# Glaciohound/Chimera-ST

Measured on AMD Instinct MI355X. Metric: train utterances/sec, MuST-C EN-DE s2t_transformer_m, 1/2/4/8 MI355X, higher is better.
Workload: dtype bf16

## Files before the change

### chimera-st_amd/csrc/gemm.hip

```cpp
#include "gemm_common.h"
#include <vector>
#include <stdlib.h>
#include <string.h>
#include <type_traits>

namespace {
using namespace cstg;

template <int BM_, int BN_, int WM_, int WN_, int KV_ = 8>
struct Cfg {
  static constexpr int BM = BM_, BN = BN_, WM = WM_, WN = WN_, NT = 64 * WM_ * WN_, TM = BM_ / WM_ / 32, TN = BN_ / WN_ / 32;
  static constexpr int KV = KV_;
  static_assert(BM_ <= GEMM_MAX_BM && GEMM_MAX_BM % BM_ == 0, "conv0.hip (cst_conv_row_limits) sizes live frames from GEMM_MAX_BM");
};
using CfgSmall = Cfg<128, 128, 2, 2>;
using CfgSkinny = Cfg<64, 64, 2, 2>;
using CfgNarrowN = Cfg<128, 64, 2, 2>;
using CfgNarrowM = Cfg<64, 128, 2, 2>;
using CfgLarge = Cfg<256, 256, 4, 4>;

template <typename T, bool A_KMAJOR, bool B_KMAJOR, bool SEG, typename C, bool CS = false>
__global__ __launch_bounds__(C::NT) void gemm_kernel(GemmParams p) {
  constexpr int BM = C::BM, BN = C::BN, NTHREADS = C::NT, TM = C::TM, TN = C::TN;
  constexpr int VEC = DT<T>::VEC;
  constexpr int KV = C::KV, BK = KV * VEC;
  constexpr int LDK = BK + VEC;
  constexpr int LDMA = sizeof(T) == 2 ? BM + 32 : BM + VEC;
  constexpr int LDMB = sizeof(T) == 2 ? BN + 32 : BN + VEC;
  constexpr int A_ELEMS = A_KMAJOR ? BM * LDK : BK * LDMA;
  constexpr int B_ELEMS = B_KMAJOR ? BN * LDK : BK * LDMB;
  constexpr int MVA = BM / VEC, MVB = BN / VEC;
  constexpr int NVA = BM * KV / NTHREADS, NVB = BN * KV / NTHREADS;
  extern __shared__ __attribute__((aligned(16))) char smem_raw[];
  T* smem = reinterpret_cast<T*>(smem_raw);
  constexpr int STAGE = A_ELEMS + B_ELEMS;

  const int tid = threadIdx.x, lane = tid & 63, wave = tid >> 6;
  const int wm = wave / C::WN, wn = wave % C::WN;

  const int ntiles = p.tiles_m * p.tiles_n;
  int tm, tn, z;
  if (p.split_order) {
    const int total = ntiles * p.splits, L = (int)blockIdx.x + (int)gridDim.x * (int)blockIdx.z;
    const int q = total / 8, r = total % 8, xcd = L % 8, loc = L / 8;
    const int item = (xcd < r ? xcd * (q + 1) : r * (q + 1) + (xcd - r) * q) + loc;
    z = item / ntiles;
    const int t = item % ntiles;
    tm = t / p.tiles_n;
    tn = t % p.tiles_n;
  } else {
    int id = blockIdx.x;
    {
      const int q = ntiles / 8, r = ntiles % 8, xcd = id % 8, loc = id / 8;
      id = (xcd < r ? xcd * (q + 1) : r * (q + 1) + (xcd - r) * q) + loc;
    }
    constexpr int GROUP_M = 8;
    const int per_group = GROUP_M * p.tiles_n;
    const int grp = id / per_group, rem = id % per_group;
    const int gm0 = grp * GROUP_M;
    const int gsz = (p.tiles_m - gm0 < GROUP_M) ? (p.tiles_m - gm0) : GROUP_M;
    tm = gm0 + rem % gsz;
    tn = rem / gsz;
    z = blockIdx.z;
  }
  const int64_t m0 = (int64_t)tm * BM, n0 = (int64_t)tn * BN;

  const int split = z % p.splits;
  const int64_t bidx = z / p.splits;
  const int64_t b0 = bidx / p.batch1, b1 = bidx % p.batch1;
  const T* A = (const T*)p.A + b0 * p.sa0 + b1 * p.sa1;
  const T* B = (const T*)p.B + b0 * p.sb0 + b1 * p.sb1;
  const int64_t cofs = b0 * p.sc0 + b1 * p.sc1;
  const int64_t bofs = b0 * p.sbias0 + b1 * p.sbias1;

  int ktiles = (int)((p.K + BK - 1) / BK);
  const int kfull = (int)(p.K / BK);
  if (p.k_len) {
    typedef const __attribute__((address_space(4))) int32_t* cptr_t;
    const int kl = ((cptr_t)p.k_len)[b0];
    const int live = kl <= 0 ? 0 : (kl + BK - 1) / BK;
    ktiles = live < ktiles ? live : ktiles;
  }
  const int per = (ktiles + p.splits - 1) / p.splits;
  const int kt0 = split * per;
  const int kt1 = (kt0 + per < ktiles) ? kt0 + per : ktiles;

  u32x4 ra[NVA], rb[NVB];
  const T* pa[NVA];
  const T* pb[NVB];
  int ka[NVA], kb[NVB];
  int aq[NVA], ar[NVA], bq[NVB], br[NVB];
#pragma unroll
  for (int i = 0; i < NVA; ++i) {
    const int v = tid + NTHREADS * i;
    if (A_KMAJOR) {
      int64_t row = m0 + v / KV;
      row = row < p.M ? row : p.M - 1;
      ka[i] = kt0 * BK + (v % KV) * VEC;
      if (SEG && p.a_seg) { aq[i] = ka[i] / (int)p.a_seg; ar[i] = ka[i] % (int)p.a_seg; pa[i] = A + row * p.lda; }
      else { aq[i] = 0; ar[i] = 0; pa[i] = A + row * p.lda + ka[i]; }
    } else {
      int64_t m = m0 + (int64_t)(v % MVA) * VEC;
      m = m < p.M ? m : p.M - VEC;
      ka[i] = kt0 * BK + v / MVA;
      aq[i] = 0; ar[i] = 0;
      pa[i] = A + (int64_t)ka[i] * p.lda + segaddr(m, p.a_seg, p.a_seg_stride);
    }
  }
#pragma unroll
  for (int i = 0; i < NVB; ++i) {
    const int v = tid + NTHREADS * i;
    if (B_KMAJOR) {
      int64_t row = n0 + v / KV;
      row = row < p.N ? row : p.N - 1;
      kb[i] = kt0 * BK + (v % KV) * VEC;
      if (SEG && p.b_seg) { bq[i] = kb[i] / (int)p.b_seg; br[i] = kb[i] % (int)p.b_seg; pb[i] = B + row * p.ldb; }
      else { bq[i] = 0; br[i] = 0; pb[i] = B + row * p.ldb + kb[i]; }
    } else {
      int64_t n = n0 + (int64_t)(v % MVB) * VEC;
      n = n < p.N ? n : p.N - VEC;
      kb[i] = kt0 * BK + v / MVB;
      bq[i] = 0; br[i] = 0;
      pb[i] = B + (int64_t)kb[i] * p.ldb + segaddr(n, p.b_seg, p.b_seg_stride);
    }
  }
  const int64_t step_a = A_KMAJOR ? (int64_t)BK : (int64_t)BK * p.lda;
  const int64_t step_b = B_KMAJOR ? (int64_t)BK : (int64_t)BK * p.ldb;

  auto load_tile = [&](auto tail_tag) {
    constexpr bool TAIL = decltype(tail_tag)::value;
    const u32x4 zero = {0, 0, 0, 0};
#pragma unroll
    for (int i = 0; i < NVA; ++i) {
      const T* qa = pa[i];
      if (SEG && A_KMAJOR && p.a_seg) qa = pa[i] + (int64_t)aq[i] * p.a_seg_stride + ar[i];
      if (TAIL) {
        const bool oka = ka[i] < p.K;
        const u32x4 va = *reinterpret_cast<const u32x4*>(oka ? qa : A);
        ra[i] = oka ? va : zero;
      } else {
        ra[i] = *reinterpret_cast<const u32x4*>(qa);
      }
      ka[i] += BK;
      if (SEG && A_KMAJOR && p.a_seg) { ar[i] += BK; while (ar[i] >= (int)p.a_seg) { ar[i] -= (int)p.a_seg; ++aq[i]; } }
      else pa[i] += step_a;
    }
#pragma unroll
    for (int i = 0; i < NVB; ++i) {
      const T* qb = pb[i];
      if (SEG && B_KMAJOR && p.b_seg) qb = pb[i] + (int64_t)bq[i] * p.b_seg_stride + br[i];
      if (TAIL) {
        const bool okb = kb[i] < p.K;
        const u32x4 vb = *reinterpret_cast<const u32x4*>(okb ? qb : B);
        rb[i] = okb ? vb : zero;
      } else {
        rb[i] = *reinterpret_cast<const u32x4*>(qb);
      }
      kb[i] += BK;
      if (SEG && B_KMAJOR && p.b_seg) { br[i] += BK; while (br[i] >= (int)p.b_seg) { br[i] -= (int)p.b_seg; ++bq[i]; } }
      else pb[i] += step_b;
    }
  };
  auto load_any = [&](int kt) {
    if (kt < kfull) load_tile(std::false_type{});
    else load_tile(std::true_type{});
  };
  static_assert(!CS || (!A_KMAJOR && NTHREADS % MVA == 0), "a thread must stage the same columns of an mn-major A in every vector");
  const bool do_cs = CS && tn == 0;
  float cs[VEC];
#pragma unroll
  for (int e = 0; e < VEC; ++e) cs[e] = 0.0f;
  auto store_tile = [&](int buf) {
#pragma unroll
    for (int i = 0; i < NVA; ++i) {
      const int v = tid + NTHREADS * i;
      T* da = smem + buf * STAGE + (A_KMAJOR ? (v / KV) * LDK + (v % KV) * VEC : (v / MVA) * LDMA + (v % MVA) * VEC);
      *reinterpret_cast<u32x4*>(da) = ra[i];
      if (CS && do_cs) {
        if (sizeof(T) == 2) {
#pragma unroll
          for (int e = 0; e < 4; ++e) {
            cs[2 * e] += __uint_as_float(ra[i][e] << 16);
            cs[2 * e + 1] += __uint_as_float(ra[i][e] & 0xffff0000u);
          }
        } else {
#pragma unroll
          for (int e = 0; e < 4; ++e) cs[e] += __uint_as_float(ra[i][e]);
        }
      }
    }
#pragma unroll
    for (int i = 0; i < NVB; ++i) {
      const int v = tid + NTHREADS * i;
      T* db = smem + buf * STAGE + A_ELEMS + (B_KMAJOR ? (v / KV) * LDK + (v % KV) * VEC : (v / MVB) * LDMB + (v % MVB) * VEC);
      *reinterpret_cast<u32x4*>(db) = rb[i];
    }
  };

  f32x16 acc[TM][TN];
#pragma unroll
  for (int i = 0; i < TM; ++i)
#pragma unroll
    for (int j = 0; j < TN; ++j)
#pragma unroll
      for (int r = 0; r < 16; ++r) acc[i][j][r] = 0.0f;

  constexpr int KLIST_MAX = 1000;
  __shared__ int klist[KLIST_MAX];
  __shared__ int klist_n;
  const bool kskip = !SEG && BK == 64 && p.k_live != nullptr && per <= KLIST_MAX;
  int nk = kt1 > kt0 ? kt1 - kt0 : 0;
  if (kskip) {
    if (wave == 0) {
      int total = 0;
      for (int base = 0; base < ktiles; base += 64) {
        const int kt = base + lane;
        total += __builtin_popcountll(__builtin_amdgcn_ballot_w64(kt < ktiles && p.k_live[kt] == p.k_epoch));
      }
      const int lo = (int)(((int64_t)total * split) / p.splits), hi = (int)(((int64_t)total * (split + 1)) / p.splits);
      int seen = 0, n = 0;
      for (int base = 0; base < ktiles && seen < hi; base += 64) {
        const int kt = base + lane;
        const bool live = kt < ktiles && p.k_live[kt] == p.k_epoch;
        const uint64_t m = __builtin_amdgcn_ballot_w64(live);
        const int idx = seen + __builtin_popcountll(m & ((1ull << lane) - 1ull));
        if (live && idx >= lo && idx < hi) klist[idx - lo] = kt;
        seen += __builtin_popcountll(m);
      }
      n = hi - lo;
      if (lane == 0) klist_n = n;
    }
    __syncthreads();
    nk = klist_n;
  }
  if (p.m_live) {
    typedef const __attribute__((address_space(4))) uint32_t* cptr_t;
    cptr_t ml = (cptr_t)p.m_live;
    const int t0 = (int)(m0 >> 6), t1 = (int)((((m0 + BM < p.M) ? m0 + BM : p.M) + 63) >> 6);
    bool live = false;
    for (int t = t0; t < t1; ++t) live |= ml[t] == p.m_epoch;
    if (!live) nk = 0;
  }
  if (p.m_len) {
    typedef const __attribute__((address_space(4))) int32_t* cptr_t;
    if (m0 >= (int64_t)((cptr_t)p.m_len)[b0]) nk = 0;
  }
  int pos = kt0;
  auto fetch = [&](int kt) {
    const int d = kt - pos;
    if (d) {
#pragma unroll
      for (int i = 0; i < NVA; ++i) { pa[i] += (int64_t)d * step_a; ka[i] += d * BK; }
#pragma unroll
      for (int i = 0; i < NVB; ++i) { pb[i] += (int64_t)d * step_b; kb[i] += d * BK; }
    }
    load_any(kt);
    pos = kt + 1;
  };
  auto tile_at = [&](int it) { return kskip ? klist[it] : kt0 + it; };

  if (nk > 0) {
    fetch(tile_at(0));
    store_tile(0);
  }
  __syncthreads();
  int cur = 0;
  const int lrow = lane & 31, lk = 8 * (lane >> 5);
  constexpr int WROWS = TM * 32, WCOLS = TN * 32;
  for (int it = 0; it < nk; ++it) {
    const bool more = it + 1 < nk;
    if (more) fetch(tile_at(it + 1));
    const T* sa = smem + cur * STAGE;
    const T* sb = sa + A_ELEMS;
#pragma unroll
    for (int kk = 0; kk < BK; kk += 16) {
      Frag<T> fa[TM], fb[TN];
#pragma unroll
      for (int i = 0; i < TM; ++i) {
        if (A_KMAJOR) frag_load_contig(fa[i], sa + (wm * WROWS + i * 32 + lrow) * LDK + kk + lk);
        else frag_load_tr(fa[i], sa, LDMA, wm * WROWS + i * 32, kk + lk, kk + lk + 4, lane);
      }
#pragma unroll
      for (int j = 0; j < TN; ++j) {
        if (B_KMAJOR) frag_load_contig(fb[j], sb + (wn * WCOLS + j * 32 + lrow) * LDK + kk + lk);
        else frag_load_tr(fb[j], sb, LDMB, wn * WCOLS + j * 32, kk + lk, kk + lk + 4, lane);
      }
#pragma unroll
      for (int i = 0; i < TM; ++i)
#pragma unroll
        for (int j = 0; j < TN; ++j) mma16(acc[i][j], fa[i], fb[j]);
    }
    if (more) store_tile(cur ^ 1);
    __syncthreads();
    cur ^= 1;
  }

  if (CS && do_cs) {
    float* red = reinterpret_cast<float*>(smem_raw);
#pragma unroll
    for (int e = 0; e < VEC; ++e) red[(tid / MVA) * BM + (tid % MVA) * VEC + e] = cs[e];
    __syncthreads();
    if (tid < BM && m0 + tid < p.M) {
      float tot = 0.0f;
      for (int r = 0; r < NTHREADS / MVA; ++r) tot += red[r * BM + tid];
      if (p.splits > 1) p.colsum_ws[((int64_t)bidx * p.splits + split) * p.M + m0 + tid] = tot;
      else DT<T>::st((T*)p.colsum + bidx * p.M + m0 + tid, tot);
    }
  }

  constexpr int LDC = BN + 4;
  constexpr int VPR = BN / 8;
  constexpr int NPASS = BM / 64;
  constexpr int ITERS = 64 * VPR / NTHREADS;
  float* stage = reinterpret_cast<float*>(smem_raw);
  float* wsp = p.splits > 1 ? p.ws + ((int64_t)z) * p.M * p.N : nullptr;
  const bool ws_vec = (p.N % 4) == 0;
#pragma unroll
  for (int ps = 0; ps < NPASS; ++ps) {
    __syncthreads();
#pragma unroll
    for (int i = 0; i < TM; ++i) {
      const int trow = wm * WROWS + i * 32;
      if (trow / 64 == ps) {
#pragma unroll
        for (int j = 0; j < TN; ++j)
#pragma unroll
          for (int r = 0; r < 16; ++r)
            stage[(trow - 64 * ps + acc_row(r, lane)) * LDC + wn * WCOLS + j * 32 + lrow] = acc[i][j][r];
      }
    }
    __syncthreads();
#pragma unroll 2
    for (int it = 0; it < ITERS; ++it) {
      const int v = tid + NTHREADS * it;
      const int rl = v / VPR, cl = (v % VPR) * 8;
      const int64_t row = m0 + 64 * ps + rl, col = n0 + cl;
      if (row >= p.M || col >= p.N) continue;
      float x[8];
      {
        const f32x4 a = *reinterpret_cast<const f32x4*>(stage + rl * LDC + cl);
        const f32x4 b = *reinterpret_cast<const f32x4*>(stage + rl * LDC + cl + 4);
        x[0] = a[0]; x[1] = a[1]; x[2] = a[2]; x[3] = a[3]; x[4] = b[0]; x[5] = b[1]; x[6] = b[2]; x[7] = b[3];
      }
      const bool full = col + 8 <= p.N;
      if (wsp) {
        if (full && ws_vec) store8(wsp + row * p.N + col, x);
        else
          for (int e = 0; e < 8 && col + e < p.N; ++e) wsp[row * p.N + col + e] = x[e];
      } else if (full && p.vec_epi) {
        epilogue_store8<T>(p, cofs, bofs, row, col, x);
      } else {
        for (int e = 0; e < 8 && col + e < p.N; ++e) epilogue_store<T>(p, cofs, bofs, row, col + e, x[e]);
      }
    }
  }
}

template <int N>
__device__ __forceinline__ void wait_vmcnt() { asm volatile("s_waitcnt vmcnt(%0)" ::"n"(N) : "memory"); }

template <typename T, bool A_KMAJOR, bool B_KMAJOR, typename C, int NS>
__global__ __launch_bounds__(C::NT) void gemm_glds_kernel(GemmParams p) {
  constexpr int BM = C::BM, BN = C::BN, NTHREADS = C::NT, TM = C::TM, TN = C::TN, NWAVES = C::NT / 64;
  constexpr int ES = sizeof(T), VEC = DT<T>::VEC, BK = 128 / ES;
  constexpr int A_BYTES = A_KMAJOR ? BM * 128 : BK * BM * ES;
  constexpr int B_BYTES = B_KMAJOR ? BN * 128 : BK * BN * ES;
  constexpr int STAGE_BYTES = A_BYTES + B_BYTES;
  constexpr int GA = A_BYTES / 1024 / NWAVES, GB = B_BYTES / 1024 / NWAVES;
  extern __shared__ __attribute__((aligned(16))) char smem_raw[];

  const int tid = threadIdx.x, lane = tid & 63, wave = tid >> 6;
  const int wm = wave / C::WN, wn = wave % C::WN;
  const int ntiles = p.tiles_m * p.tiles_n;
  int id = blockIdx.x;
  {
    const int q = ntiles / 8, r = ntiles % 8, xcd = id % 8, loc = id / 8;
    id = (xcd < r ? xcd * (q + 1) : r * (q + 1) + (xcd - r) * q) + loc;
  }
  constexpr int GROUP_M = 8;
  int tm, tn;
  {
    const int per_group = GROUP_M * p.tiles_n;
    const int grp = id / per_group, rem = id % per_group;
    const int gm0 = grp * GROUP_M;
    const int gsz = (p.tiles_m - gm0 < GROUP_M) ? (p.tiles_m - gm0) : GROUP_M;
    tm = gm0 + rem % gsz;
    tn = rem / gsz;
  }
  const int64_t m0 = (int64_t)tm * BM, n0 = (int64_t)tn * BN;
  const int z = blockIdx.z;
  const int split = z % p.splits;
  const int64_t bidx = z / p.splits;
  const int64_t b0 = bidx / p.batch1, b1 = bidx % p.batch1;
  const T* A = (const T*)p.A + b0 * p.sa0 + b1 * p.sa1;
  const T* B = (const T*)p.B + b0 * p.sb0 + b1 * p.sb1;
  const int64_t cofs = b0 * p.sc0 + b1 * p.sc1;
  const int64_t bofs = b0 * p.sbias0 + b1 * p.sbias1;
  const int ktiles = (int)((p.K + BK - 1) / BK);
  const int kfull = (int)(p.K / BK);
  const int per = (ktiles + p.splits - 1) / p.splits;
  const int kt0 = split * per;
  const int kt1 = (kt0 + per < ktiles) ? kt0 + per : ktiles;
  int nt = kt1 - kt0;
  if (p.m_len) {
    typedef const __attribute__((address_space(4))) int32_t* cptr_t;
    if (m0 >= (int64_t)((cptr_t)p.m_len)[b0]) nt = 0;
  }

  const T* pa[GA];
  const T* pb[GB];
  int ka[GA], kb[GB];
#pragma unroll
  for (int i = 0; i < GA; ++i) {
    const int g = wave + NWAVES * i;
    if (A_KMAJOR) {
      const int r = 8 * g + (lane >> 3), c = (lane & 7) ^ ((r >> 1) & 7);
      int64_t row = m0 + r;
      row = row < p.M ? row : p.M - 1;
      ka[i] = kt0 * BK + c * VEC;
      pa[i] = A + row * p.lda + ka[i];
    } else {
      constexpr int RB = BM * ES, RPG = 1024 / RB > 0 ? 1024 / RB : 1, CPR = RB / 16;
      const int kl = g * RPG + (lane * 16) / RB, pc = ((lane * 16) % RB) / 16;
      const int c = ES == 2 ? (pc ^ (4 * (kl & 3))) : pc;
      int64_t m = m0 + (int64_t)c * VEC;
      m = m < p.M ? m : p.M - VEC;
      ka[i] = kt0 * BK + kl;
      pa[i] = A + (int64_t)ka[i] * p.lda + segaddr(m, p.a_seg, p.a_seg_stride);
      (void)CPR;
    }
  }
#pragma unroll
  for (int i = 0; i < GB; ++i) {
    const int g = wave + NWAVES * i;
    if (B_KMAJOR) {
      const int r = 8 * g + (lane >> 3), c = (lane & 7) ^ ((r >> 1) & 7);
      int64_t row = n0 + r;
      row = row < p.N ? row : p.N - 1;
      kb[i] = kt0 * BK + c * VEC;
      pb[i] = B + row * p.ldb + kb[i];
    } else {
      constexpr int RB = BN * ES, RPG = 1024 / RB > 0 ? 1024 / RB : 1;
      const int kl = g * RPG + (lane * 16) / RB, pc = ((lane * 16) % RB) / 16;
      const int c = ES == 2 ? (pc ^ (4 * (kl & 3))) : pc;
      int64_t n = n0 + (int64_t)c * VEC;
      n = n < p.N ? n : p.N - VEC;
      kb[i] = kt0 * BK + kl;
      pb[i] = B + (int64_t)kb[i] * p.ldb + segaddr(n, p.b_seg, p.b_seg_stride);
    }
  }
  const int64_t step_a = A_KMAJOR ? (int64_t)BK : (int64_t)BK * p.lda;
  const int64_t step_b = B_KMAJOR ? (int64_t)BK : (int64_t)BK * p.ldb;

  auto issue = [&](int kt, int stage) {
    char* sbase = smem_raw + stage * STAGE_BYTES;
    if (kt < kfull) {
#pragma unroll
      for (int i = 0; i < GA; ++i) {
        __builtin_amdgcn_global_load_lds((const __attribute__((address_space(1))) void*)pa[i],
                                         (__attribute__((address_space(3))) void*)(sbase + (wave + NWAVES * i) * 1024), 16, 0, 0);
        pa[i] += step_a;
        ka[i] += BK;
      }
#pragma unroll
      for (int i = 0; i < GB; ++i) {
        __builtin_amdgcn_global_load_lds((const __attribute__((address_space(1))) void*)pb[i],
                                         (__attribute__((address_space(3))) void*)(sbase + A_BYTES + (wave + NWAVES * i) * 1024), 16, 0, 0);
        pb[i] += step_b;
        kb[i] += BK;
      }
    } else {
      const u32x4 zero = {0, 0, 0, 0};
#pragma unroll
      for (int i = 0; i < GA; ++i) {
        const bool ok = ka[i] < p.K;
        const u32x4 v = *reinterpret_cast<const u32x4*>(ok ? pa[i] : A);
        *reinterpret_cast<u32x4*>(sbase + (wave + NWAVES * i) * 1024 + lane * 16) = ok ? v : zero;
        pa[i] += step_a;
        ka[i] += BK;
      }
#pragma unroll
      for (int i = 0; i < GB; ++i) {
        const bool ok = kb[i] < p.K;
        const u32x4 v = *reinterpret_cast<const u32x4*>(ok ? pb[i] : B);
        *reinterpret_cast<u32x4*>(sbase + A_BYTES + (wave + NWAVES * i) * 1024 + lane * 16) = ok ? v : zero;
        pb[i] += step_b;
        kb[i] += BK;
      }
    }
  };

  f32x16 acc[TM][TN];
#pragma unroll
  for (int i = 0; i < TM; ++i)
#pragma unroll
    for (int j = 0; j < TN; ++j)
#pragma unroll
      for (int r = 0; r < 16; ++r) acc[i][j][r] = 0.0f;

  const int lrow = lane & 31, hi = lane >> 5;
  constexpr int WROWS = TM * 32, WCOLS = TN * 32;
  constexpr int G = GA + GB;

#pragma unroll
  for (int s = 0; s < NS - 1; ++s)
    if (s < nt) issue(kt0 + s, s);

  constexpr bool PIN = NTHREADS == 256 && TM == 4 && NS == 2 && A_KMAJOR && B_KMAJOR && sizeof(T) == 2;
  if constexpr (PIN) {
    auto issue_one = [&](int d, char* sbase) {
      if (d < GA) {
        __builtin_amdgcn_global_load_lds((const __attribute__((address_space(1))) void*)pa[d],
                                         (__attribute__((address_space(3))) void*)(sbase + (wave + NWAVES * d) * 1024), 16, 0, 0);
        pa[d] += step_a;
        ka[d] += BK;
      } else {
        const int e = d - GA;
        __builtin_amdgcn_global_load_lds((const __attribute__((address_space(1))) void*)pb[e],
                                         (__attribute__((address_space(3))) void*)(sbase + A_BYTES + (wave + NWAVES * e) * 1024), 16, 0, 0);
        pb[e] += step_b;
        kb[e] += BK;
      }
    };
    constexpr int NSLOT = TM * TN / 2, NFR = TM + TN;
    for (int it = 0; it < nt; ++it) {
      wait_vmcnt<0>();
      __builtin_amdgcn_s_barrier();
      const bool more = it + 1 < nt;
      const bool dma_ok = more && (kt0 + it + 1) < kfull;
      if (more && !dma_ok) issue(kt0 + it + 1, (it + 1) & 1);
      const char* sbase = smem_raw + (it & 1) * STAGE_BYTES;
      char* nbase = smem_raw + ((it + 1) & 1) * STAGE_BYTES;
      const T* sa = reinterpret_cast<const T*>(sbase);
      const T* sb = reinterpret_cast<const T*>(sbase + A_BYTES);
      Frag<T> fa[2][TM], fb[2][TN];
      auto read_one = [&](int f, int kk, int buf) {
        if (f < TM) frag_load_kswz(fa[buf][f], sa, wm * WROWS + f * 32 + lrow, kk * 16 + 8 * hi);
        else frag_load_kswz(fb[buf][f - TM], sb, wn * WCOLS + (f - TM) * 32 + lrow, kk * 16 + 8 * hi);
      };
#pragma unroll
      for (int f = 0; f < NFR; ++f) read_one(f, 0, 0);
      __builtin_amdgcn_sched_barrier(0);
#pragma unroll
      for (int kk = 0; kk < 4; ++kk) {
#pragma unroll
        for (int sl = 0; sl < NSLOT; ++sl) {
#pragma unroll
          for (int u = 0; u < 2; ++u) {
            const int m = 2 * sl + u, i = m / TN, j = m % TN;
            mma16(acc[i][j], fb[kk & 1][j], fa[kk & 1][i]);
          }
          if (kk < 3) {
            if (sl < NFR) read_one(sl, kk + 1, (kk + 1) & 1);
            if (sl == 0 && NFR > NSLOT) {
#pragma unroll
              for (int f = NSLOT; f < NFR; ++f) read_one(f, kk + 1, (kk + 1) & 1);
            }
          }
          if (kk * NSLOT + sl < G && dma_ok) issue_one(kk * NSLOT + sl, nbase);
          __builtin_amdgcn_sched_barrier(0);
        }
      }
    }
  } else
  for (int it = 0; it < nt; ++it) {
    const int issued = (it + NS - 1 < nt) ? it + NS - 1 : nt;
    if (NS > 2 && issued - it - 1 == NS - 2) wait_vmcnt<(NS - 2) * G>();
    else wait_vmcnt<0>();
    __builtin_amdgcn_s_barrier();
    if (it + NS - 1 < nt) issue(kt0 + it + NS - 1, (it + NS - 1) % NS);
    const char* sbase = smem_raw + (it % NS) * STAGE_BYTES;
    const T* sa = reinterpret_cast<const T*>(sbase);
    const T* sb = reinterpret_cast<const T*>(sbase + A_BYTES);
#pragma unroll
    for (int kk = 0; kk < BK; kk += 16) {
      Frag<T> fa[TM], fb[TN];
#pragma unroll
      for (int i = 0; i < TM; ++i) {
        if (A_KMAJOR) {
          const int r = wm * WROWS + i * 32 + lrow;
          frag_load_kswz(fa[i], sa, r, kk + 8 * hi);
        } else {
          frag_load_tr_swz(fa[i], sa, BM, wm * WROWS + i * 32, kk + 8 * hi, lane);
        }
      }
#pragma unroll
      for (int j = 0; j < TN; ++j) {
        if (B_KMAJOR) {
          const int r = wn * WCOLS + j * 32 + lrow;
          frag_load_kswz(fb[j], sb, r, kk + 8 * hi);
        } else {
          frag_load_tr_swz(fb[j], sb, BN, wn * WCOLS + j * 32, kk + 8 * hi, lane);
        }
      }
#pragma unroll
      for (int i = 0; i < TM; ++i)
#pragma unroll
        for (int j = 0; j < TN; ++j) mma16(acc[i][j], fa[i], fb[j]);
    }
  }

  float* wsp = p.splits > 1 ? p.ws + ((int64_t)z) * p.M * p.N : nullptr;
  const bool ws_vec = (p.N % 4) == 0;
  if constexpr (PIN) {
    constexpr int LDW = WCOLS + 4, VPRW = WCOLS / 8, RITER = 32 * VPRW / 64;
    static_assert(4 * 32 * LDW * 4 <= NS * STAGE_BYTES && (32 * VPRW) % 64 == 0, "the four waves' images live in the stage buffers");
    __syncthreads();
    float* img = reinterpret_cast<float*>(smem_raw) + wave * (32 * LDW);
#pragma unroll
    for (int i = 0; i < TM; ++i) {
#pragma unroll
      for (int j = 0; j < TN; ++j)
#pragma unroll
        for (int q = 0; q < 4; ++q) {
          const f32x4 v = {acc[i][j][4 * q], acc[i][j][4 * q + 1], acc[i][j][4 * q + 2], acc[i][j][4 * q + 3]};
          *reinterpret_cast<f32x4*>(img + lrow * LDW + j * 32 + 8 * q + 4 * hi) = v;
        }
#pragma unroll 2
      for (int tv = 0; tv < RITER; ++tv) {
        const int v = tv * 64 + lane;
        const int rl = v / VPRW, cl = (v % VPRW) * 8;
        const int64_t row = m0 + wm * WROWS + i * 32 + rl, col = n0 + wn * WCOLS + cl;
        if (row >= p.M || col >= p.N) continue;
        float x[8];
        {
          const f32x4 a = *reinterpret_cast<const f32x4*>(img + rl * LDW + cl);
          const f32x4 b = *reinterpret_cast<const f32x4*>(img + rl * LDW + cl + 4);
          x[0] = a[0]; x[1] = a[1]; x[2] = a[2]; x[3] = a[3]; x[4] = b[0]; x[5] = b[1]; x[6] = b[2]; x[7] = b[3];
        }
        const bool full = col + 8 <= p.N;
        if (wsp) {
          if (full && ws_vec) store8(wsp + row * p.N + col, x);
          else
            for (int e = 0; e < 8 && col + e < p.N; ++e) wsp[row * p.N + col + e] = x[e];
        } else if (full && p.vec_epi) {
          epilogue_store8<T>(p, cofs, bofs, row, col, x);
        } else {
          for (int e = 0; e < 8 && col + e < p.N; ++e) epilogue_store<T>(p, cofs, bofs, row, col + e, x[e]);
        }
      }
    }
    return;
  }
  constexpr int LDC = BN + 4;
  constexpr int VPR = BN / 8;
  constexpr int NPASS = BM / 64;
  constexpr int ITERS = 64 * VPR / NTHREADS;
  float* stage = reinterpret_cast<float*>(smem_raw);
#pragma unroll
  for (int ps = 0; ps < NPASS; ++ps) {
    __syncthreads();
#pragma unroll
    for (int i = 0; i < TM; ++i) {
      const int trow = wm * WROWS + i * 32;
      if (trow / 64 == ps) {
#pragma unroll
        for (int j = 0; j < TN; ++j)
#pragma unroll
          for (int r = 0; r < 16; ++r)
            stage[(trow - 64 * ps + acc_row(r, lane)) * LDC + wn * WCOLS + j * 32 + lrow] = acc[i][j][r];
      }
    }
    __syncthreads();
#pragma unroll 2
    for (int itv = 0; itv < ITERS; ++itv) {
      const int v = tid + NTHREADS * itv;
      const int rl = v / VPR, cl = (v % VPR) * 8;
      const int64_t row = m0 + 64 * ps + rl, col = n0 + cl;
      if (row >= p.M || col >= p.N) continue;
      float x[8];
      {
        const f32x4 a = *reinterpret_cast<const f32x4*>(stage + rl * LDC + cl);
        const f32x4 b = *reinterpret_cast<const f32x4*>(stage + rl * LDC + cl + 4);
        x[0] = a[0]; x[1] = a[1]; x[2] = a[2]; x[3] = a[3]; x[4] = b[0]; x[5] = b[1]; x[6] = b[2]; x[7] = b[3];
      }
      const bool full = col + 8 <= p.N;
      if (wsp) {
        if (full && ws_vec) store8(wsp + row * p.N + col, x);
        else
          for (int e = 0; e < 8 && col + e < p.N; ++e) wsp[row * p.N + col + e] = x[e];
      } else if (full && p.vec_epi) {
        epilogue_store8<T>(p, cofs, bofs, row, col, x);
      } else {
        for (int e = 0; e < 8 && col + e < p.N; ++e) epilogue_store<T>(p, cofs, bofs, row, col + e, x[e]);
      }
    }
  }
}

template <typename T>
__global__ void splitk_reduce_kernel(GemmParams p) {
  const int64_t total = p.M * p.N;
  const int64_t bidx = blockIdx.y;
  const int64_t b0 = bidx / p.batch1, b1 = bidx % p.batch1;
  const int64_t cofs = b0 * p.sc0 + b1 * p.sc1;
  const int64_t bofs = b0 * p.sbias0 + b1 * p.sbias1;
  const float* ws = p.ws + bidx * p.splits * total;
  if (p.colsum) {
    for (int64_t m = (int64_t)blockIdx.x * blockDim.x + threadIdx.x; m < p.M; m += (int64_t)gridDim.x * blockDim.x) {
      float v = 0.0f;
      for (int s = 0; s < p.splits; ++s) v += p.colsum_ws[(bidx * p.splits + s) * p.M + m];
      DT<T>::st((T*)p.colsum + bidx * p.M + m, v);
    }
  }
  if (p.vec_epi && (p.N % 8) == 0) {
    const int64_t total8 = total >> 3;
    for (int64_t i8 = (int64_t)blockIdx.x * blockDim.x + threadIdx.x; i8 < total8; i8 += (int64_t)gridDim.x * blockDim.x) {
      const float* src = ws + i8 * 8;
      float v[8] = {0.0f, 0.0f, 0.0f, 0.0f, 0.0f, 0.0f, 0.0f, 0.0f};
      int sp = 0;
      for (; sp + 4 <= p.splits; sp += 4) {
        f32x4 a[4][2];
#pragma unroll
        for (int u = 0; u < 4; ++u) {
          a[u][0] = *reinterpret_cast<const f32x4*>(src + (int64_t)(sp + u) * total);
          a[u][1] = *reinterpret_cast<const f32x4*>(src + (int64_t)(sp + u) * total + 4);
        }
#pragma unroll
        for (int u = 0; u < 4; ++u)
#pragma unroll
          for (int e = 0; e < 4; ++e) { v[e] += a[u][0][e]; v[4 + e] += a[u][1][e]; }
      }
      for (; sp < p.splits; ++sp) {
        const f32x4 a0 = *reinterpret_cast<const f32x4*>(src + (int64_t)sp * total), a1 = *reinterpret_cast<const f32x4*>(src + (int64_t)sp * total + 4);
#pragma unroll
        for (int e = 0; e < 4; ++e) { v[e] += a0[e]; v[4 + e] += a1[e]; }
      }
      const int64_t i = i8 * 8, row = i / p.N;
      epilogue_store8<T>(p, cofs, bofs, row, i - row * p.N, v);
    }
    return;
  }
  for (int64_t i = (int64_t)blockIdx.x * blockDim.x + threadIdx.x; i < total; i += (int64_t)gridDim.x * blockDim.x) {
    float v = 0.0f;
    for (int s = 0; s < p.splits; ++s) v += ws[s * total + i];
    epilogue_store<T>(p, cofs, bofs, i / p.N, i % p.N, v);
  }
}

template <typename T, bool AK, bool BK_, bool SEG, typename C>
int launch(GemmParams p, int64_t M, int64_t N, int64_t nbatch, hipStream_t s) {
  constexpr int VEC = DT<T>::VEC;
  constexpr int BKc = C::KV * VEC, LDK = BKc + VEC;
  constexpr int LDMA = sizeof(T) == 2 ? C::BM + 32 : C::BM + VEC, LDMB = sizeof(T) == 2 ? C::BN + 32 : C::BN + VEC;
  constexpr int A_ELEMS = AK ? C::BM * LDK : BKc * LDMA;
  constexpr int B_ELEMS = BK_ ? C::BN * LDK : BKc * LDMB;
  size_t lds = 2 * (size_t)(A_ELEMS + B_ELEMS) * sizeof(T);
  const size_t stage_bytes = (size_t)64 * (C::BN + 4) * sizeof(float);
  if (lds < stage_bytes) lds = stage_bytes;
  static bool attr_set = false;
  if (!attr_set) {
    (void)hipFuncSetAttribute(reinterpret_cast<const void*>(&gemm_kernel<T, AK, BK_, SEG, C>), hipFuncAttributeMaxDynamicSharedMemorySize, 160 * 1024 - 4096);
    attr_set = true;
  }
  p.tiles_m = (int)cst_ceil_div(M, C::BM);
  p.tiles_n = (int)cst_ceil_div(N, C::BN);
  p.split_order = (p.splits > 1 && nbatch == 1) ? 1 : 0;
  dim3 grid(p.tiles_m * p.tiles_n, 1, (unsigned)(nbatch * p.splits));
  if constexpr (!AK && !BK_ && !SEG && C::NT <= 256) {
    if (p.colsum) {
      static bool attr_cs = false;
      if (!attr_cs) {
        (void)hipFuncSetAttribute(reinterpret_cast<const void*>(&gemm_kernel<T, AK, BK_, SEG, C, true>), hipFuncAttributeMaxDynamicSharedMemorySize, 160 * 1024 - 4096);
        attr_cs = true;
      }
      hipLaunchKernelGGL((gemm_kernel<T, AK, BK_, SEG, C, true>), grid, dim3(C::NT), lds, s, p);
      return cst_check_launch("cst_gemm");
    }
  }
  if (p.colsum) { cst_set_error("cst_gemm: internal: column sums requested from a configuration that does not build them"); return CST_ERR_UNSUPPORTED; }
  hipLaunchKernelGGL((gemm_kernel<T, AK, BK_, SEG, C>), grid, dim3(C::NT), lds, s, p);
  return cst_check_launch("cst_gemm");
}

template <typename T, bool AK, bool BK_, typename C, int NS>
int launch_glds(GemmParams p, int64_t M, int64_t N, int64_t nbatch, hipStream_t s) {
  constexpr int ES = sizeof(T), BKc = 128 / ES;
  constexpr int A_BYTES = AK ? C::BM * 128 : BKc * C::BM * ES, B_BYTES = BK_ ? C::BN * 128 : BKc * C::BN * ES;
  size_t lds = (size_t)NS * (A_BYTES + B_BYTES);
  const size_t stage_bytes = (size_t)64 * (C::BN + 4) * sizeof(float);
  if (lds < stage_bytes) lds = stage_bytes;
  static bool attr_set = false;
  if (!attr_set) {
    (void)hipFuncSetAttribute(reinterpret_cast<const void*>(&gemm_glds_kernel<T, AK, BK_, C, NS>), hipFuncAttributeMaxDynamicSharedMemorySize, 160 * 1024);
    attr_set = true;
  }
  p.tiles_m = (int)cst_ceil_div(M, C::BM);
  p.tiles_n = (int)cst_ceil_div(N, C::BN);
  dim3 grid(p.tiles_m * p.tiles_n, 1, (unsigned)(nbatch * p.splits));
  hipLaunchKernelGGL((gemm_glds_kernel<T, AK, BK_, C, NS>), grid, dim3(C::NT), lds, s, p);
  return cst_check_launch("cst_gemm");
}


struct GemmSwitches {
  bool no_klive;
  int group_m;
  bool no_narrow;
  bool no_4w;
  bool experiment;
  const char* force_cfg;
};

GemmSwitches gemm_switches() {
  static const GemmSwitches once = [] {
    GemmSwitches w;
    w.no_klive = getenv("CST_GEMM_NO_KLIVE") != nullptr;
    const char* gm = getenv("CST_GEMM8P_GROUP_M");
    w.group_m = gm && atoi(gm) > 0 ? atoi(gm) : 4;
    w.no_narrow = getenv("CST_GEMM_NO_NARROW") != nullptr;
    w.no_4w = getenv("CST_GEMM_NO_4W") != nullptr;
    w.experiment = getenv("CST_GEMM_EXPERIMENT") != nullptr;
    w.force_cfg = nullptr;
    return w;
  }();
  GemmSwitches w = once;
  if (w.experiment) {
    const char* f = getenv("CST_GEMM_FORCE_CFG");
    w.force_cfg = f && *f ? f : nullptr;
  }
  return w;
}

enum class Family { Reg, Dma, Persistent8, FourWave };
enum class Tile { Small, Large, Skinny, NarrowN, NarrowM, Big4, Big4N, Unknown };
enum class Colsum { None, Fused, Separate };
using CfgBig4 = Cfg<256, 256, 2, 2>;
using CfgBig4N = Cfg<256, 192, 2, 2>;

struct GemmRoute {
  Family family;
  Tile tile;
  bool bf16, ak, bk;
  bool seg;
  int stages;
  int splits;
  Colsum colsum;
};

struct TileDims { int bm, bn, nt; };
template <typename C> constexpr TileDims dims_of() { return {C::BM, C::BN, C::NT}; }
constexpr TileDims kTileDims[] = {dims_of<CfgSmall>(),   dims_of<CfgLarge>(), dims_of<CfgSkinny>(), dims_of<CfgNarrowN>(),
                                  dims_of<CfgNarrowM>(), dims_of<CfgBig4>(),  dims_of<CfgBig4N>(),  {0, 0, 0}};

bool use_large(const cst_gemm_desc* d, bool seg, int splits) {
  if (seg) return false;
  const int64_t tiles = cst_ceil_div(d->M, 256) * cst_ceil_div(d->N, 256) * d->batch0 * d->batch1 * splits;
  return d->M >= 256 && d->N >= 256 && tiles >= 200;
}

int choose_splits(const cst_gemm_desc* d) {
  if (d->split_k > 1) return d->split_k;
  if (d->split_k == 0 || d->split_k == 1) return 1;
  const int bk = d->dtype == CST_BF16 ? 64 : 32;
  const int64_t ktiles = cst_ceil_div(d->K, bk);
  const int64_t nb = d->batch0 * d->batch1;
  if (d->M >= 256 && d->N >= 256) {
    const int64_t tl = cst_ceil_div(d->M, 256) * cst_ceil_div(d->N, 256) * nb;
    if (tl >= 200) return 1;
    int64_t s = 256 / tl;
    if (s > ktiles / 16) s = ktiles / 16;
    if (s > 32) s = 32;
    if (s >= 1 && tl * s >= 200) return (int)s;
  }
  const int64_t tiles = cst_ceil_div(d->M, 128) * cst_ceil_div(d->N, 128) * nb;
  if (tiles >= 256 || ktiles < 16) return 1;
  const int64_t cap = ktiles / 8 < 32 ? ktiles / 8 : 32;
  int64_t s1 = 256 / tiles, s2 = 512 / tiles;
  if (s1 > cap) s1 = cap;
  if (s2 > cap) s2 = cap;
  if (s1 < 1) s1 = 1;
  if (s2 < 1) s2 = 1;
  const int64_t s = (2.0 / (double)s2 < 0.9 / (double)s1) ? s2 : s1;
  return (int)s;
}

struct Forced { const char* name; bool kk; Family family; Tile tile; int stages; };
const Forced kForced[] = {
    {"small", false, Family::Reg, Tile::Small, 0},     {"narrowm", false, Family::Reg, Tile::NarrowM, 0},
    {"narrown", false, Family::Reg, Tile::NarrowN, 0}, {"skinny", false, Family::Reg, Tile::Skinny, 0},
    {"large", false, Family::Reg, Tile::Large, 0},     {"big4r", false, Family::Reg, Tile::Big4, 0},
    {"skinny4", true, Family::Dma, Tile::Skinny, 4},   {"skinny2", true, Family::Dma, Tile::Skinny, 2},
    {"small2", true, Family::Dma, Tile::Small, 2},     {"small3", true, Family::Dma, Tile::Small, 3},
    {"big4", true, Family::Dma, Tile::Big4, 2},        {"big4n", true, Family::Dma, Tile::Big4N, 2},
    {"big4r", true, Family::Reg, Tile::Big4, 0},       {"large", true, Family::Reg, Tile::Large, 0},
    {"8p", true, Family::Persistent8, Tile::Large, 0}, {"4w", true, Family::FourWave, Tile::Big4N, 0},
};

GemmRoute gemm_route(const cst_gemm_desc* d, const GemmParams& p, const GemmSwitches& sw) {
  GemmRoute r;
  r.bf16 = d->dtype == CST_BF16;
  r.ak = d->a_kmajor != 0;
  r.bk = d->b_kmajor != 0;
  r.seg = (r.ak && d->a_seg) || (r.bk && d->b_seg);
  r.stages = 2;
  r.splits = choose_splits(d);
  const bool kk = r.ak && r.bk, mm = !r.ak && !r.bk;
  const bool large = use_large(d, r.seg, r.splits);
  const int64_t nbatch = d->batch0 * d->batch1;
  r.colsum = !d->colsum ? Colsum::None : (mm && !d->a_seg && !d->b_seg && !large) ? Colsum::Fused : Colsum::Separate;
  auto take = [&r](Family f, Tile t, int stages = 2) { r.family = f; r.tile = t; r.stages = stages; return r; };

  if (!sw.no_narrow && !r.seg && !large && kk && d->N <= 64 && d->M > 256) return take(Family::Dma, Tile::NarrowN);
  if (!sw.no_narrow && !r.seg && !large && mm && d->M <= 64 && d->N > 256) return take(Family::Reg, Tile::NarrowM);

  GemmParams q = p;
  q.splits = r.splits;
  const bool unsplit1 = !r.seg && nbatch == 1 && r.splits == 1;
  if (sw.force_cfg && r.bf16 && !r.seg && nbatch == 1 && (mm || (kk && r.splits == 1))) {
    for (const Forced& f : kForced) {
      if (f.kk != kk || strcmp(f.name, sw.force_cfg) != 0) continue;
      if (f.family == Family::Persistent8 && !cst_gemm8p_supported(q, r.ak, r.bk, nbatch)) break;
      if (f.family == Family::FourWave && !cst_gemm4w_supported(q, r.ak, r.bk, nbatch)) break;
      return take(f.family, f.tile, f.stages);
    }
    return take(Family::Reg, Tile::Unknown);
  }

  const bool mid8p = kk && unsplit1 && d->M >= 256 && d->N >= 256 && cst_ceil_div(d->M, 256) * cst_ceil_div(d->N, 256) >= 150;
  if (kk && unsplit1 && (d->M <= 256 || (!large && !mid8p && cst_ceil_div(d->M, 128) * cst_ceil_div(d->N, 128) < 256))) {
    const bool two_stage = d->M > 256 && cst_ceil_div(d->M, 64) * cst_ceil_div(d->N, 64) > 512;
    return take(Family::Dma, Tile::Skinny, two_stage ? 2 : 4);
  }
  if (r.bf16 && !r.seg && !d->colsum) {
    if (!sw.no_4w && cst_gemm4w_supported(q, r.ak, r.bk, nbatch)) return take(Family::FourWave, Tile::Big4N);
    if (r.ak && (!d->dact || (!d->resid && !d->aux_out)) && (large || mid8p) && cst_gemm8p_supported(q, r.ak, r.bk, nbatch))
      return take(Family::Persistent8, Tile::Large);
  }
  const Tile t = large ? Tile::Large : Tile::Small;
  if (r.seg) return take(Family::Reg, Tile::Small);
  return take(kk && !d->colsum ? Family::Dma : Family::Reg, t);
}

void route_text(const GemmRoute& r, char* out, int64_t n) {
  const TileDims t = kTileDims[(int)r.tile];
  const char* dt = r.bf16 ? "bf16" : "f32";
  const char a = r.ak ? 'k' : 'm', b = r.bk ? 'k' : 'm';
  switch (r.family) {
    case Family::Reg:
      snprintf(out, (size_t)n, "reg %s %c%c%s %dx%d nt%d%s split%d", dt, a, b, r.seg ? " seg" : "", t.bm, t.bn, t.nt,
               r.colsum == Colsum::Fused ? " colsum" : "", r.splits);
      break;
    case Family::Dma: snprintf(out, (size_t)n, "glds %s %c%c %dx%d nt%d ns%d split%d", dt, a, b, t.bm, t.bn, t.nt, r.stages, r.splits); break;
    case Family::Persistent8: snprintf(out, (size_t)n, "8p %c%c", a, b); break;
    case Family::FourWave: snprintf(out, (size_t)n, "4w"); break;
  }
}

}

extern "C" int64_t cst_colsum_workspace(int64_t rows, int64_t cols);
extern "C" int cst_colsum_typed(const void* x, int64_t ldx, void* out, void* workspace, int64_t rows, int64_t cols, int dtype, int out_dtype, cst_stream stream);
extern "C" int cst_colsum_typed_live(const void* x, int64_t ldx, void* out, void* workspace, int64_t rows, int64_t cols, int dtype, int out_dtype,
                                     const uint32_t* row_live, uint32_t epoch, cst_stream stream);

namespace {

int validate(const cst_gemm_desc* d) {
  CST_REQUIRE(d && d->A && d->B && d->C, "cst_gemm: null operand");
  CST_REQUIRE(d->dtype == CST_F32 || d->dtype == CST_BF16, "cst_gemm: bad dtype %d", d->dtype);
  CST_REQUIRE(d->c_dtype == d->dtype || d->c_dtype == CST_F32, "cst_gemm: c_dtype must be dtype or f32");
  CST_REQUIRE(d->M > 0 && d->N > 0 && d->K > 0, "cst_gemm: empty problem M=%lld N=%lld K=%lld", (long long)d->M,
              (long long)d->N, (long long)d->K);
  const int vec = d->dtype == CST_BF16 ? 8 : 4;
  if (d->a_kmajor) CST_REQUIRE(d->K % vec == 0 && d->lda % vec == 0, "cst_gemm: k-major A needs K,lda %% %d == 0 (K=%lld lda=%lld)", vec, (long long)d->K, (long long)d->lda);
  else CST_REQUIRE(d->M % vec == 0 && d->lda % vec == 0, "cst_gemm: mn-major A needs M,lda %% %d == 0 (M=%lld lda=%lld)", vec, (long long)d->M, (long long)d->lda);
  if (d->b_kmajor) CST_REQUIRE(d->K % vec == 0 && d->ldb % vec == 0, "cst_gemm: k-major B needs K,ldb %% %d == 0 (K=%lld ldb=%lld)", vec, (long long)d->K, (long long)d->ldb);
  else CST_REQUIRE(d->N % vec == 0 && d->ldb % vec == 0, "cst_gemm: mn-major B needs N,ldb %% %d == 0 (N=%lld ldb=%lld)", vec, (long long)d->N, (long long)d->ldb);
  CST_REQUIRE(d->a_seg % vec == 0 && d->b_seg % vec == 0 && d->a_seg_stride % vec == 0 && d->b_seg_stride % vec == 0,
              "cst_gemm: segment sizes must be multiples of %d", vec);
  CST_REQUIRE(((uintptr_t)d->A % 16 == 0) && ((uintptr_t)d->B % 16 == 0), "cst_gemm: A/B must be 16-byte aligned");
  CST_REQUIRE(d->sa0 % vec == 0 && d->sa1 % vec == 0 && d->sb0 % vec == 0 && d->sb1 % vec == 0, "cst_gemm: batch strides of A/B must be multiples of %d", vec);
  CST_REQUIRE(d->batch0 >= 1 && d->batch1 >= 1, "cst_gemm: batch counts must be >= 1");
  CST_REQUIRE(!d->dact || d->aux_in, "cst_gemm: dact needs aux_in");
  CST_REQUIRE(d->drop_p >= 0.0f && d->drop_p < 1.0f, "cst_gemm: drop_p must be in [0, 1)");
  CST_REQUIRE(d->drop_p == 0.0f || d->batch0 * d->batch1 == 1, "cst_gemm: fused dropout needs an unbatched problem");
  CST_REQUIRE(!d->colsum || (!d->a_kmajor && !d->a_seg), "cst_gemm: colsum needs an mn-major, unsegmented A");
  return CST_OK;
}

GemmParams fill_params(const cst_gemm_desc* d, const GemmSwitches& sw) {
  GemmParams p;
  p.M = d->M; p.N = d->N; p.K = d->K;
  p.A = d->A; p.lda = d->lda; p.a_seg = d->a_seg; p.a_seg_stride = d->a_seg_stride;
  p.B = d->B; p.ldb = d->ldb; p.b_seg = d->b_seg; p.b_seg_stride = d->b_seg_stride;
  p.C = d->C; p.ldc = d->ldc;
  p.bias = d->bias; p.bias_mode = d->bias ? d->bias_mode : CST_BIAS_NONE; p.sbias0 = d->sbias0; p.sbias1 = d->sbias1;
  p.act = d->act;
  p.aux_out = d->aux_out; p.ld_aux_out = d->ld_aux_out;
  p.dact = d->dact; p.aux_in = d->aux_in; p.ld_aux_in = d->ld_aux_in;
  p.resid = d->resid; p.ld_resid = d->ld_resid;
  p.alpha = d->alpha;
  p.drop_thr = d->drop_p > 0.0f ? cst_drop_thr16(d->drop_p) : 0u;
  p.drop_key = d->drop_key;
  p.drop_scale = d->drop_p > 0.0f ? 1.0f / (1.0f - d->drop_p) : 1.0f;
  p.drop_row0 = 0;
  p.batch1 = d->batch1;
  p.sa0 = d->sa0; p.sa1 = d->sa1; p.sb0 = d->sb0; p.sb1 = d->sb1; p.sc0 = d->sc0; p.sc1 = d->sc1;
  p.c_f32 = (d->c_dtype == CST_F32 && d->dtype != CST_F32) ? 1 : 0;
  {
    auto al16 = [](const void* q) { return q == nullptr || ((uintptr_t)q % 16) == 0; };
    bool ok = d->ldc % 8 == 0 && d->sc0 % 8 == 0 && d->sc1 % 8 == 0 && al16(d->C) && al16(d->bias) && al16(d->aux_out) && al16(d->aux_in) && al16(d->resid);
    if (d->bias && d->bias_mode == CST_BIAS_COL) ok = ok && d->sbias0 % 8 == 0 && d->sbias1 % 8 == 0;
    if (d->aux_out) ok = ok && d->ld_aux_out % 8 == 0;
    if (d->aux_in) ok = ok && d->ld_aux_in % 8 == 0;
    if (d->resid) ok = ok && d->ld_resid % 8 == 0;
    if (d->drop_p > 0.0f) ok = ok && (d->N % 2 == 0);
    p.vec_epi = ok ? 1 : 0;
  }
  p.tiles_m = p.tiles_n = 0;
  p.split_order = 0;
  p.sched = nullptr;
  p.gperm_full = 0;
  p.mrot = 0;
  p.k_live = sw.no_klive ? nullptr : d->k_live;
  p.k_epoch = d->k_epoch;
  p.m_live = sw.no_klive ? nullptr : d->m_live;
  p.m_epoch = d->m_epoch;
  p.k_len = sw.no_klive ? nullptr : d->k_len;
  p.m_len = sw.no_klive ? nullptr : d->m_len;
  p.group_m = sw.group_m;
  p.splits = 1;
  p.ws = nullptr;
  p.colsum = nullptr;
  p.colsum_ws = nullptr;
  return p;
}

int64_t route_workspace(const cst_gemm_desc* d, const GemmRoute& r) {
  const int64_t s = r.splits, nb = d->batch0 * d->batch1;
  int64_t bytes = s > 1 ? s * d->M * d->N * nb * (int64_t)sizeof(float) : 0;
  if (r.colsum == Colsum::Fused) bytes += s > 1 ? s * d->M * nb * (int64_t)sizeof(float) : 0;
  else if (r.colsum == Colsum::Separate) bytes += cst_colsum_workspace(d->K, d->M);
  return bytes;
}

int take_route(const cst_gemm_desc* d, const GemmSwitches& sw, GemmParams& p, GemmRoute& r) {
  r = gemm_route(d, p, sw);
  const int64_t nbatch = d->batch0 * d->batch1;
  CST_REQUIRE(r.colsum != Colsum::Separate || (nbatch == 1 && d->M % 8 == 0 && d->lda % 8 == 0),
              "cst_gemm: colsum of this configuration runs as a separate column sum: unbatched, M and lda multiples of 8");
  CST_REQUIRE(cst_ceil_div(d->M, 128) * cst_ceil_div(d->N, 128) < (1ll << 31) && nbatch * r.splits < 65536, "cst_gemm: grid too large");
  p.splits = r.splits;
  p.colsum = r.colsum == Colsum::Fused ? d->colsum : nullptr;
#ifdef CST_TRACE
  if (p.splits == 1 && d->workspace) p.ws = (float*)d->workspace;
#endif
  const int64_t need = route_workspace(d, r);
  if (need > 0 && (!d->workspace || d->workspace_bytes < need)) {
    if (r.splits > 1) cst_set_error("cst_gemm: split_k=%d needs %lld workspace bytes, got %lld", r.splits, (long long)need, (long long)d->workspace_bytes);
    else cst_set_error("cst_gemm: colsum needs %lld workspace bytes, got %lld", (long long)need, (long long)d->workspace_bytes);
    return CST_ERR_WORKSPACE;
  }
  if (r.splits > 1) {
    p.ws = (float*)d->workspace;
    p.colsum_ws = p.ws + (int64_t)r.splits * d->M * d->N * nbatch;
  }
  return CST_OK;
}

template <typename W>
bool read_back(hipStream_t s, const W* dev, int64_t n, std::vector<W>& host) {
  host.resize((size_t)n);
  return hipStreamSynchronize(s) == hipSuccess && hipMemcpy(host.data(), dev, sizeof(W) * n, hipMemcpyDeviceToHost) == hipSuccess;
}

struct Work { double flops, bytes; };
Work credited_work(const cst_gemm_desc* d, const GemmParams& p, hipStream_t s) {
  double frac = 1.0;
  if (cst_prof_is_on()) {
    std::vector<uint32_t> st;
    std::vector<int32_t> len;
    const int64_t mtiles = cst_ceil_div(d->M, 256);
    if (p.k_live && read_back(s, p.k_live, cst_ceil_div(d->K, 64), st)) {
      int64_t live = 0;
      for (uint32_t v : st) live += v == p.k_epoch;
      frac *= (double)live / (double)st.size();
    }
    if (p.k_len && read_back(s, p.k_len, d->batch0, len)) {
      double sum = 0.0;
      for (int32_t v : len) sum += (double)(v < 0 ? 0 : (v < d->K ? v : d->K));
      frac *= sum / ((double)d->batch0 * (double)d->K);
    }
    if (p.m_len && read_back(s, p.m_len, d->batch0, len)) {
      double live = 0.0;
      for (int32_t v : len) {
        const int64_t t = v <= 0 ? 0 : cst_ceil_div((int64_t)v, 256);
        live += (double)(t < mtiles ? t : mtiles);
      }
      frac *= live / ((double)d->batch0 * (double)mtiles);
    }
    if (p.m_live && read_back(s, p.m_live, cst_ceil_div(d->M, 64), st)) {
      const int64_t nt = (int64_t)st.size();
      int64_t live = 0;
      for (int64_t t = 0; t < mtiles; ++t) {
        bool l = false;
        for (int64_t i = 4 * t; i < 4 * t + 4 && i < nt; ++i) l |= st[i] == p.m_epoch;
        live += l;
      }
      frac *= (double)live / (double)mtiles;
    }
  }
  const double nbatch = (double)(d->batch0 * d->batch1), esz = (double)cst_dtype_size(d->dtype);
  return {2.0 * (double)d->M * (double)d->N * (double)d->K * nbatch * frac,
          ((double)d->M * d->K + (double)d->N * d->K) * esz * nbatch * frac + (double)d->M * d->N * cst_dtype_size(d->c_dtype) * nbatch};
}

int unlaunchable(const GemmRoute& r, const GemmSwitches& sw) {
  if (r.tile == Tile::Unknown) {
    cst_set_error("cst_gemm: unknown CST_GEMM_FORCE_CFG %s", sw.force_cfg ? sw.force_cfg : "");
    return CST_ERR_BAD_ARG;
  }
  if (r.family == Family::Reg && r.colsum == Colsum::Fused && kTileDims[(int)r.tile].nt > 256) {
    cst_set_error("cst_gemm: internal: column sums requested from a configuration that does not build them");
    return CST_ERR_UNSUPPORTED;
  }
  return CST_OK;
}

template <typename T, bool SEG, typename C>
int launch_reg(const GemmRoute& r, const GemmParams& p, int64_t nbatch, hipStream_t s) {
  return r.ak ? (r.bk ? launch<T, true, true, SEG, C>(p, p.M, p.N, nbatch, s) : launch<T, true, false, SEG, C>(p, p.M, p.N, nbatch, s))
              : (r.bk ? launch<T, false, true, SEG, C>(p, p.M, p.N, nbatch, s) : launch<T, false, false, SEG, C>(p, p.M, p.N, nbatch, s));
}

constexpr int arm(Family f, Tile t, int stages = 0) { return ((int)f << 8) | ((int)t << 4) | stages; }

template <typename T>
int launch_route(const GemmRoute& r, const GemmParams& p, int64_t nbatch, hipStream_t s, const GemmSwitches& sw) {
  constexpr bool HOOK = std::is_same<T, bf16_t>::value;
  const int64_t M = p.M, N = p.N;
  switch (arm(r.family, r.tile, r.family == Family::Dma ? r.stages : 0)) {
    case arm(Family::Persistent8, Tile::Large): return cst_gemm8p_launch(p, r.ak, r.bk, nbatch, s);
    case arm(Family::FourWave, Tile::Big4N): return cst_gemm4w_launch(p, s);
    case arm(Family::Reg, Tile::Small): return r.seg ? launch_reg<T, true, CfgSmall>(r, p, nbatch, s) : launch_reg<T, false, CfgSmall>(r, p, nbatch, s);
    case arm(Family::Reg, Tile::Large): return launch_reg<T, false, CfgLarge>(r, p, nbatch, s);
    case arm(Family::Reg, Tile::NarrowM): return launch<T, false, false, false, CfgNarrowM>(p, M, N, nbatch, s);
    case arm(Family::Dma, Tile::Small, 2): return launch_glds<T, true, true, CfgSmall, 2>(p, M, N, nbatch, s);
    case arm(Family::Dma, Tile::Large, 2): return launch_glds<T, true, true, CfgLarge, 2>(p, M, N, nbatch, s);
    case arm(Family::Dma, Tile::NarrowN, 2): return launch_glds<T, true, true, CfgNarrowN, 2>(p, M, N, nbatch, s);
    case arm(Family::Dma, Tile::Skinny, 2): return launch_glds<T, true, true, CfgSkinny, 2>(p, M, N, nbatch, s);
    case arm(Family::Dma, Tile::Skinny, 4): return launch_glds<T, true, true, CfgSkinny, 4>(p, M, N, nbatch, s);
    case arm(Family::Reg, Tile::NarrowN): if constexpr (HOOK) return launch<T, false, false, false, CfgNarrowN>(p, M, N, nbatch, s); break;
    case arm(Family::Reg, Tile::Skinny): if constexpr (HOOK) return launch<T, false, false, false, CfgSkinny>(p, M, N, nbatch, s); break;
    case arm(Family::Reg, Tile::Big4):
      if constexpr (HOOK) return r.ak ? launch<T, true, true, false, CfgBig4>(p, M, N, nbatch, s) : launch<T, false, false, false, CfgBig4>(p, M, N, nbatch, s);
      break;
    case arm(Family::Dma, Tile::Small, 3): if constexpr (HOOK) return launch_glds<T, true, true, CfgSmall, 3>(p, M, N, nbatch, s); break;
    case arm(Family::Dma, Tile::Big4, 2): if constexpr (HOOK) return launch_glds<T, true, true, CfgBig4, 2>(p, M, N, nbatch, s); break;
    case arm(Family::Dma, Tile::Big4N, 2): if constexpr (HOOK) return launch_glds<T, true, true, CfgBig4N, 2>(p, M, N, nbatch, s); break;
    default: break;
  }
  const int rc = unlaunchable(r, sw);
  if (rc == CST_OK) cst_set_error("cst_gemm: internal: a route without a launch arm");
  return rc == CST_OK ? CST_ERR_UNSUPPORTED : rc;
}

int finish(const cst_gemm_desc* d, const GemmRoute& r, const GemmParams& p, cst_stream stream) {
  const int64_t nbatch = d->batch0 * d->batch1;
  if (p.splits > 1 && d->defer_reduce) {
    CST_REQUIRE((nbatch == 1 || !d->colsum) && d->alpha == 1.0f && !d->bias && !d->act && !d->dact && !d->aux_out && !d->resid && d->drop_p == 0.0f && d->ldc == d->N &&
                    d->N % 8 == 0 && r.colsum != Colsum::Separate,
                "cst_gemm: defer_reduce needs a plain epilogue and a dense C (batched: no colsum; the slabs are [batch][split][M][N])");
    return CST_OK;
  }
  int rc = CST_OK;
  if (p.splits > 1) {
    const int64_t total = d->M * d->N;
    const int64_t work = (p.vec_epi && d->N % 8 == 0) ? total / 8 : total;
    int blocks = (int)(cst_ceil_div(work, 256) < 2048 ? cst_ceil_div(work, 256) : 2048);
    dim3 grid(blocks, (unsigned)nbatch);
    if (d->dtype == CST_BF16) hipLaunchKernelGGL(splitk_reduce_kernel<bf16_t>, grid, dim3(256), 0, (hipStream_t)stream, p);
    else hipLaunchKernelGGL(splitk_reduce_kernel<float>, grid, dim3(256), 0, (hipStream_t)stream, p);
    rc = cst_check_launch("cst_gemm split-k reduce");
  }
  if (rc == CST_OK && r.colsum == Colsum::Separate) {
    void* cws = (char*)d->workspace + (p.splits > 1 ? (int64_t)p.splits * d->M * d->N * (int64_t)sizeof(float) : 0);
    rc = p.k_live ? cst_colsum_typed_live(d->A, d->lda, d->colsum, cws, d->K, d->M, d->dtype, d->dtype, p.k_live, p.k_epoch, stream)
                  : cst_colsum_typed(d->A, d->lda, d->colsum, cws, d->K, d->M, d->dtype, d->dtype, stream);
  }
  return rc;
}

int gemm_one(const cst_gemm_desc* d, cst_stream stream) {
  int rc = validate(d);
  if (rc != CST_OK) return rc;
  const GemmSwitches sw = gemm_switches();
  GemmParams p = fill_params(d, sw);
  GemmRoute r;
  if ((rc = take_route(d, sw, p, r)) != CST_OK) return rc;
  hipStream_t s = (hipStream_t)stream;
  const int64_t nbatch = d->batch0 * d->batch1;
  const Work w = credited_work(d, p, s);
  CstProfScope prof(CST_K_GEMM, s, w.flops, w.bytes);
  rc = r.bf16 ? launch_route<bf16_t>(r, p, nbatch, s, sw) : launch_route<float>(r, p, nbatch, s, sw);
  if (cst_prof_is_on())
    prof.tag("M=%lld N=%lld K=%lld b=%lld a%c b%c split=%d%s%s%s%s%s%s%s", (long long)d->M, (long long)d->N, (long long)d->K, (long long)nbatch, r.ak ? 'k' : 'm',
             r.bk ? 'k' : 'm', p.splits, d->bias ? " bias" : "", d->act ? " act" : "", d->aux_out ? " aux_out" : "", d->dact ? " dact" : "",
             d->resid ? " resid" : "", d->drop_p > 0 ? " drop" : "", (d->k_live || d->m_live || d->k_len || d->m_len) ? " live" : "");
  return rc != CST_OK ? rc : finish(d, r, p, stream);
}

GemmRoute query_route(const cst_gemm_desc* d) {
  const GemmSwitches sw = gemm_switches();
  return gemm_route(d, fill_params(d, sw), sw);
}

}

extern "C" int cst_gemm_splits(const cst_gemm_desc* d) { return d ? query_route(d).splits : 0; }

extern "C" int cst_gemm_colsum_is_fused(const cst_gemm_desc* d) { return d && query_route(d).colsum == Colsum::Fused ? 1 : 0; }

extern "C" int64_t cst_gemm_workspace(const cst_gemm_desc* d) { return route_workspace(d, query_route(d)); }

extern "C" int cst_gemm_route(const cst_gemm_desc* d, char* out, int64_t out_bytes) {
  if (out && out_bytes > 0) out[0] = 0;
  int rc = validate(d);
  if (rc != CST_OK) return rc;
  CST_REQUIRE(out && out_bytes > 0, "cst_gemm_route: no room for the text");
  const GemmSwitches sw = gemm_switches();
  GemmParams p = fill_params(d, sw);
  GemmRoute r;
  if ((rc = take_route(d, sw, p, r)) != CST_OK) return rc;
  if ((rc = unlaunchable(r, sw)) != CST_OK) return rc;
  route_text(r, out, out_bytes);
  return CST_OK;
}

extern "C" int cst_gemm(const cst_gemm_desc* d, cst_stream stream) { return gemm_one(d, stream); }
```

### chimera-st_amd/csrc/gemm_common.h

```cpp
#pragma once
#include "cst_common.h"

namespace cstg {

constexpr int GEMM_MAX_BM = 256;

struct GemmParams {
  int64_t M, N, K;
  const void* A; int64_t lda, a_seg, a_seg_stride;
  const void* B; int64_t ldb, b_seg, b_seg_stride;
  void* C; int64_t ldc;
  const void* bias; int bias_mode; int64_t sbias0, sbias1;
  int act;
  void* aux_out; int64_t ld_aux_out;
  int dact;
  const void* aux_in; int64_t ld_aux_in;
  const void* resid; int64_t ld_resid;
  float alpha;
  uint32_t drop_thr, drop_key; float drop_scale;
  int64_t drop_row0;
  int64_t batch1;
  int64_t sa0, sa1, sb0, sb1, sc0, sc1;
  int splits;
  float* ws;
  int c_f32;
  int vec_epi;
  int tiles_m, tiles_n;
  int nz;
  int half_from, nitems;
  int group_m;
  unsigned long long magic_ntiles, magic_per_group;
  int per_group, group_shift;
  int gperm_full, gperm_q, gperm_r;
  int mrot;
  unsigned long long magic_gq, magic_gq1;
  int split_order;
  int* sched;
  const uint32_t* m_live; uint32_t m_epoch;
  const int32_t* k_len;
  const int32_t* m_len;
  const uint32_t* k_live; uint32_t k_epoch;
  void* colsum;
  float* colsum_ws;
};

__device__ __forceinline__ int64_t segaddr(int64_t c, int64_t seg, int64_t seg_stride) {
  return seg ? (c / seg) * seg_stride + (c % seg) : c;
}

template <typename T>
__device__ __forceinline__ void epilogue_store(const GemmParams& p, int64_t cofs, int64_t bofs, int64_t row, int64_t col, float v) {
  v *= p.alpha;
  if (p.bias_mode == CST_BIAS_COL) v += DT<T>::ld((const T*)p.bias + bofs + col);
  else if (p.bias_mode == CST_BIAS_ROW) v += DT<T>::ld((const T*)p.bias + bofs + row);
  if (p.aux_out) DT<T>::st((T*)p.aux_out + cofs + row * p.ld_aux_out + col, v);
  v = act_t<T>(v, p.act);
  if (p.drop_thr) v *= cst_drop1(p.drop_key, (uint64_t)((row + p.drop_row0) * p.N + col), p.drop_thr, p.drop_scale);
  if (p.dact) v *= dact_t<T>(DT<T>::ld((const T*)p.aux_in + cofs + row * p.ld_aux_in + col), p.dact);
  if (p.resid) v += DT<T>::ld((const T*)p.resid + cofs + row * p.ld_resid + col);
  if (p.c_f32) ((float*)p.C)[cofs + row * p.ldc + col] = v;
  else DT<T>::st((T*)p.C + cofs + row * p.ldc + col, v);
}

template <typename T>
__device__ __forceinline__ void epilogue_store8(const GemmParams& p, int64_t cofs, int64_t bofs, int64_t row, int64_t col, float (&v)[8]) {
#pragma unroll
  for (int e = 0; e < 8; ++e) v[e] *= p.alpha;
  if (p.bias_mode == CST_BIAS_COL) {
    float b[8];
    load8((const T*)p.bias + bofs + col, b);
#pragma unroll
    for (int e = 0; e < 8; ++e) v[e] += b[e];
  } else if (p.bias_mode == CST_BIAS_ROW) {
    const float b = DT<T>::ld((const T*)p.bias + bofs + row);
#pragma unroll
    for (int e = 0; e < 8; ++e) v[e] += b;
  }
  if (p.aux_out) store8((T*)p.aux_out + cofs + row * p.ld_aux_out + col, v);
  if (p.act == CST_ACT_RELU) {
#pragma unroll
    for (int e = 0; e < 8; ++e) v[e] = fmaxf(v[e], 0.0f);
  } else if (p.act == CST_ACT_GELU) {
#pragma unroll
    for (int e = 0; e < 8; ++e) v[e] = gelu_t<T>(v[e]);
  }
  if (p.drop_thr) cst_drop8(v, p.drop_key, (uint64_t)((row + p.drop_row0) * p.N + col), p.drop_thr, p.drop_scale);
  if (p.dact) {
    float z[8];
    load8((const T*)p.aux_in + cofs + row * p.ld_aux_in + col, z);
#pragma unroll
    for (int e = 0; e < 8; ++e) v[e] *= dact_t<T>(z[e], p.dact);
  }
  if (p.resid) {
    float r[8];
    load8((const T*)p.resid + cofs + row * p.ld_resid + col, r);
#pragma unroll
    for (int e = 0; e < 8; ++e) v[e] += r[e];
  }
  if (p.c_f32) store8((float*)p.C + cofs + row * p.ldc + col, v);
  else store8((T*)p.C + cofs + row * p.ldc + col, v);
}

}

int cst_gemm8p_launch(cstg::GemmParams p, bool a_kmajor, bool b_kmajor, int64_t nbatch, hipStream_t s);
bool cst_gemm8p_supported(const cstg::GemmParams& p, bool a_kmajor, bool b_kmajor, int64_t nbatch);
int cst_gemm4w_launch(cstg::GemmParams p, hipStream_t s);
bool cst_gemm4w_supported(const cstg::GemmParams& p, bool a_kmajor, bool b_kmajor, int64_t nbatch);
```

### chimera-st_amd/functional.py

```python
import os as _os
import weakref as _weakref

import torch

from . import kernels as K
from . import lib as L

_ACT = {None: L.ACT_NONE, "none": L.ACT_NONE, "relu": L.ACT_RELU, "gelu": L.ACT_GELU}


def _flat2d(x):
    return x.reshape(-1, x.shape[-1]).contiguous()


def _vec(dtype):
    return 8 if dtype == torch.bfloat16 else 4


def _with_tiles(t, tiles):
    if t.is_contiguous():
        t._cst_live_tiles = (tiles[0], tiles[1], t.data_ptr(), t.numel(), t.shape[-1], t._version)
        if t._base is not None:
            t._base._cst_live_tiles = t._cst_live_tiles
    return t
# ... 500 lines not shown
        B, T = qkv.shape[0], qkv.shape[1]
        o = torch.empty(B, T, C, dtype=qkv.dtype, device=qkv.device)
        lse = torch.empty((seq[0].numel() - 1) if seq is not None else B, H, int(seq[1]) if seq is not None else T, dtype=torch.float32, device=qkv.device)
        d = K.attn_desc(q, k, v, o, lse, H, D, kpm, causal, scale, "bt", "bt", drop_p, drop_key, kvl, seq)
        K.attn_fwd_desc(d)
        ctx.save_for_backward(qkv, o, lse, kpm, kvl, seq[0] if seq is not None else None)
        ctx.cfg = (H, D, C, causal, scale, drop_p, drop_key, int(seq[1]) if seq is not None else None)
        return o

    @staticmethod
    def backward(ctx, do):
        qkv, o, lse, kpm, kvl, seq_off = ctx.saved_tensors
        H, D, C, causal, scale, drop_p, drop_key, seq_max = ctx.cfg
        seq = (seq_off, seq_max) if seq_off is not None else None
        live = _tiles_of(do, qkv.shape[0] * qkv.shape[1]) if ctx.pad_tiles is not None else None
        if not do.is_contiguous():
            do = do.contiguous()
        dqkv = torch.empty_like(qkv)
        K.attn_bwd(do, qkv[..., :C], qkv[..., C:2 * C], qkv[..., 2 * C:], o, lse, H, D, kpm, causal, scale, "bt", "bt", drop_p, drop_key, kvl, seq,
                   grads=(dqkv[..., :C], dqkv[..., C:2 * C], dqkv[..., 2 * C:]))
        if live is not None:
            stamps = torch.where(ctx.pad_tiles, live[0], torch.full_like(live[0], live[1] if live[1] < 2 ** 31 else live[1] - 2 ** 32))
            dqkv = _with_tiles(dqkv, (stamps, live[1]))
        return dqkv, None, None, None, None, None, None, None, None, None


def attention_packed(qkv, num_heads, key_padding_mask=None, causal=False, scale=None, dropout_p=0.0, seq=None):
    C = qkv.shape[-1] // 3
    if scale is None:
        scale = (C // num_heads) ** -0.5
    assert qkv.is_contiguous()
    if seq is not None:
        assert key_padding_mask is None and qkv.shape[0] == 1 and qkv.shape[1] == seq.rows
        return _AttnPackedFn.apply(qkv, None, seq.kv_len, num_heads, bool(causal), float(scale), *_drop_args(dropout_p), None, (seq.offsets, seq.longest))
    key_padding_mask, kv_len = _mask_and_len(key_padding_mask)
    pad_tiles = _pad_tiles(key_padding_mask) if (key_padding_mask is not None and qkv.requires_grad) else None
    return _AttnPackedFn.apply(qkv, key_padding_mask, kv_len, num_heads, bool(causal), float(scale), *_drop_args(dropout_p), pad_tiles)


class _StackedRowsFn(torch.autograd.Function):

    @staticmethod
    def forward(ctx, *ts):
        a = ts[0]
        ctx.rows, ctx.n = a.shape[0], len(ts)
        return torch.as_strided(a, (len(ts) * a.shape[0],) + tuple(a.shape[1:]), a.stride(), a.storage_offset())

    @staticmethod
    def backward(ctx, g):
        r = ctx.rows
        return tuple(g[i * r:(i + 1) * r] for i in range(ctx.n))


def stacked_rows(*ts):
    a = ts[0]
    n = a.numel() * a.element_size()
    if (not _os.environ.get("CST_NO_QKV_VIEW") and all(t.shape == a.shape and t.is_contiguous() for t in ts)
            and all(ts[i].data_ptr() + n == ts[i + 1].data_ptr() for i in range(len(ts) - 1))
            and a.untyped_storage().data_ptr() == ts[-1].untyped_storage().data_ptr()):
        K.STATS["qkv_view"] = K.STATS.get("qkv_view", 0) + 1
        out = _StackedRowsFn.apply(*ts)
        out._cst_parts = tuple(t.detach() for t in ts)
        out._cst_parts_params = tuple(ts)
        return out
    return torch.cat(ts, 0)


class PackedRows:

    def __init__(self, offsets, kv_len, rows, longest, B, T, host_lens=None):
        self.offsets, self.kv_len, self.rows, self.longest, self.B, self.T = offsets, kv_len, rows, longest, B, T
        self.host_lens = host_lens
        self.kept_host = None


def plan_packed_rows(padding_mask, margin):
    B, T = padding_mask.shape
    lens = (~padding_mask).sum(dim=1).to(torch.int32)
    n = torch.clamp(lens + (margin + 1), max=T)
    off = torch.zeros(B + 1, dtype=torch.int32, device=padding_mask.device)
    off[1:] = torch.cumsum(n, 0)
    host = torch.cat((off[-1:], n.max().view(1), lens)).tolist()
    plan = PackedRows(off.contiguous(), lens.contiguous(), int(host[0]), int(host[1]), B, T, [int(v) for v in host[2:]])
    plan.kept_host = [min(T, v + margin + 1) for v in plan.host_lens]
    return plan


def plan_from_lengths(lens_dev, host_lens, T):
    B = lens_dev.numel()
    n = torch.clamp(lens_dev.to(torch.int32), max=T)
    off = torch.zeros(B + 1, dtype=torch.int32, device=lens_dev.device)
    off[1:] = torch.cumsum(n, 0)
    hl = [min(int(v), T) for v in host_lens]
    return PackedRows(off.contiguous(), n.contiguous(), sum(hl), max(hl), B, T, hl)


class _PackRowsFn(torch.autograd.Function):

    @staticmethod
    def forward(ctx, x, seq):
        ctx.seq = seq
        return K.rows_pack(x.contiguous(), seq.offsets, seq.rows, tail_sum=False).unsqueeze(0)

    @staticmethod
    def backward(ctx, dy):
        s = ctx.seq
        dy2 = dy.reshape(s.rows, dy.shape[-1])
        return K.rows_unpack(dy2.contiguous(), s.offsets, s.B, s.T, tail_broadcast=False), None


class _UnpackRowsFn(torch.autograd.Function):

    @staticmethod
    def forward(ctx, y, seq, broadcast):
        ctx.seq, ctx.broadcast = seq, broadcast
        y2 = y.reshape(seq.rows, y.shape[-1])
        return K.rows_unpack(y2.contiguous(), seq.offsets, seq.B, seq.T, tail_broadcast=broadcast)

    @staticmethod
    def backward(ctx, dx):
        s = ctx.seq
        return K.rows_pack(dx.contiguous(), s.offsets, s.rows, tail_sum=ctx.broadcast).unsqueeze(0), None, None


def pack_rows(x, seq):
    return _PackRowsFn.apply(x, seq)


def unpack_rows(y, seq, broadcast=True):
    return _UnpackRowsFn.apply(y, seq, bool(broadcast))


def _conv0_args(wav, w, write_limit, grad_limit):
    C, _, k = w.shape
    if _os.environ.get("CST_NO_MLEN") or _os.environ.get("CST_GEMM_NO_KLIVE"):
        write_limit = grad_limit = None
    return wav.float().contiguous(), w.reshape(C, k).contiguous(), k, write_limit, grad_limit


class _Conv0Fn(torch.autograd.Function):
    @staticmethod
    def forward(ctx, wav, w, gamma, beta, stride, eps, write_limit, grad_limit):
        wav, w2, k, write_limit, grad_limit = _conv0_args(wav, w, write_limit, grad_limit)
        y, mean, rstd, gram = K.conv0_fwd(wav, w2, gamma, beta, k, stride, eps, frame_limit=write_limit)
        ctx.save_for_backward(wav, w2, gamma, beta, mean, rstd, gram)
        ctx.k, ctx.stride, ctx.grad_limit = k, stride, grad_limit
        return y

    @staticmethod
    def backward(ctx, dy):
        wav, w2, gamma, beta, mean, rstd, gram = ctx.saved_tensors
        dw, dg, db = K.conv0_bwd(dy.contiguous(), wav, w2, gamma, beta, mean, rstd, gram, ctx.k, ctx.stride, frame_limit=ctx.grad_limit)
        return None, dw.view(w2.shape[0], 1, ctx.k).to(w2.dtype), dg.to(gamma.dtype), db.to(gamma.dtype), None, None, None, None


def conv0_gn_gelu(wav, weight, gn_weight, gn_bias, stride, eps=1e-5, write_limit=None, grad_limit=None):
    return _Conv0Fn.apply(wav, weight, gn_weight, gn_bias, stride, eps, write_limit, grad_limit)


class _Conv0LnFn(torch.autograd.Function):
    @staticmethod
    def forward(ctx, wav, w, bias, gamma, beta, stride, eps, write_limit, grad_limit):
        wav, w2, k, write_limit, grad_limit = _conv0_args(wav, w, write_limit, grad_limit)
        y, mean, rstd = K.conv0_ln_fwd(wav, w2, bias, gamma, beta, k, stride, eps, frame_limit=write_limit)
        ctx.save_for_backward(wav, w2, bias, gamma, beta, mean, rstd)
        ctx.k, ctx.stride, ctx.grad_limit = k, stride, grad_limit
        return y

    @staticmethod
    def backward(ctx, dy):
        wav, w2, bias, gamma, beta, mean, rstd = ctx.saved_tensors
        dw, dbi, dg, db = K.conv0_ln_bwd(dy.contiguous(), wav, w2, bias, gamma, beta, mean, rstd, ctx.k, ctx.stride, frame_limit=ctx.grad_limit)
        return (None, dw.view(w2.shape[0], 1, ctx.k).to(w2.dtype), dbi.to(bias.dtype), dg.to(gamma.dtype), db.to(gamma.dtype),
                None, None, None, None)


def conv0_ln_gelu(wav, weight, bias, ln_weight, ln_bias, stride, eps=1e-5, write_limit=None, grad_limit=None):
    return _Conv0LnFn.apply(wav, weight, bias, ln_weight, ln_bias, stride, eps, write_limit, grad_limit)


class _LnGeluFn(torch.autograd.Function):

    @staticmethod
    def forward(ctx, u, gamma, beta, conv_bias, eps, row_limit):
        if _os.environ.get("CST_NO_MLEN"):
            row_limit = None
        u = u.contiguous()
        y, mean, rstd = K.ln_gelu_fwd(u, gamma, beta, eps, row_limit)
        ctx.save_for_backward(u, gamma, beta, mean, rstd)
        ctx.row_limit = row_limit
        ctx.bias_dtype = conv_bias.dtype if conv_bias is not None else None
        return y

    @staticmethod
    def backward(ctx, dy):
        u, gamma, beta, mean, rstd = ctx.saved_tensors
        want_bias = ctx.bias_dtype is not None and ctx.needs_input_grad[3]
        du, dg, db, dc = K.ln_gelu_bwd(dy.contiguous(), u, gamma, beta, mean, rstd, ctx.row_limit,
                                       want_colsum=want_bias, padded=True)
        return du, dg.to(gamma.dtype), db.to(gamma.dtype), (dc.to(ctx.bias_dtype) if want_bias else None), None, None


def ln_gelu(u, ln_weight, ln_bias, conv_bias=None, eps=1e-5, row_limit=None):
    return _LnGeluFn.apply(u, ln_weight, ln_bias, conv_bias, eps, row_limit)


def _padded_base(t, L, C):
    if t.dim() == 3 and t.stride(2) == 1 and t.stride(1) == C and t.stride(0) == (L + 2) * C and t.storage_offset() >= C:
        return torch.as_strided(t, (t.shape[0], L + 2, C), t.stride(), t.storage_offset() - C)
    return None


class _Conv1dCLFn(torch.autograd.Function):

    @staticmethod
    def forward(ctx, x, w_cl, bias, k, stride, pad, act, prev_z, grad_is_dz, nz_out=None, nz_in=None, unread_ok=False):
        if _os.environ.get("CST_NO_MLEN"):
            nz_in = None
            fwd_len = None
        else:
            fwd_len = nz_out if (bias is None or unread_ok) else None
        ctx.nz_out = nz_out
        ctx.nz_in = nz_in
        B, Lin, Cin = x.shape
        Cout = w_cl.shape[0]
        if pad:
            xp = torch.empty(B, Lin + 2 * pad, Cin, dtype=x.dtype, device=x.device)
            xp[:, :pad].zero_()
            xp[:, pad + Lin:].zero_()
            xp[:, pad:pad + Lin] = x
        elif x.stride(2) == 1 and x.stride(1) == Cin:
            xp = x
        else:
            xp = x.contiguous()
        Lp = Lin + 2 * pad
        Lout = (Lp - k) // stride + 1
        padded_out = bool(grad_is_dz) and act != L.ACT_NONE
        rows = Lout + 2 if padded_out else Lout
        y_full = torch.empty(B, rows, Cout, dtype=x.dtype, device=x.device)
        z_full = torch.empty_like(y_full) if act != L.ACT_NONE else None
        coff = Cout if padded_out else 0
        K.gemm(xp, w_cl, y_full, Lout, Cout, k * Cin, a_kmajor=1, b_kmajor=1, lda=stride * Cin, ldb=k * Cin, ldc=Cout, bias=bias,
               act=act, aux_out=z_full, ld_aux_out=Cout, batch0=B, sa=(xp.stride(0), 0), sc=(rows * Cout, 0), split_k=1,
               a_off=0, c_off=coff, m_len=fwd_len)
        y = y_full[:, 1:1 + Lout] if padded_out else y_full
        z = (z_full[:, 1:1 + Lout] if padded_out else z_full) if z_full is not None else None
        ctx.save_for_backward(xp, w_cl, z, prev_z)
        ctx.cfg = (B, Lin, Cin, Cout, k, stride, pad, Lout, act, bias is not None, grad_is_dz)
        ctx.set_materialize_grads(False)
        if act != L.ACT_NONE:
            ctx.mark_non_differentiable(z)
            return y, z
        return y, None

    @staticmethod
    def backward(ctx, dy, _dz_unused):
        xp, w_cl, z, prev_z = ctx.saved_tensors
        B, Lin, Cin, Cout, k, stride, pad, Lout, act, has_bias, grad_is_dz = ctx.cfg
        fast = pad == 0 and k <= stride + 1
        dzp = _padded_base(dy, Lout, Cout) if (act == L.ACT_NONE or grad_is_dz) else None
        if dzp is None:
            dyc = dy.contiguous()
            dzc = K.act_bwd(dyc, z.contiguous(), act) if (act != L.ACT_NONE and not grad_is_dz) else dyc
            if fast:
                dzp = torch.empty(B, Lout + 2, Cout, dtype=dy.dtype, device=dy.device)
                dzp[:, 0].zero_()
                dzp[:, Lout + 1].zero_()
                dzp[:, 1:1 + Lout] = dzc
            dz_rows, dz_bs, dz_off = dzc, Lout * Cout, 0
        else:
            dz_rows, dz_bs, dz_off = dzp, (Lout + 2) * Cout, Cout
        dx = dw = db = None
        if ctx.needs_input_grad[0]:
            if fast:
                dx_padded = prev_z is not None and _padded_base(prev_z, Lin, Cin) is not None
                rows = Lin + 2 if dx_padded else Lin
                dx_full = torch.empty(B, rows, Cin, dtype=dy.dtype, device=dy.device)
                if dx_padded:
                    dx_full[:, 0].zero_()
                    dx_full[:, Lin + 1].zero_()
                pz = prev_z if prev_z is None or dx_padded else prev_z.contiguous()
                pz_base = _padded_base(prev_z, Lin, Cin) if dx_padded else pz
                w3 = w_cl.view(Cout, k, Cin)
                for r in range(stride):
                    taps = list(range(r, k, stride))
                    n = len(taps)
                    U = (Lin - r + stride - 1) // stride
                    if n == 0 or U <= 0:
                        continue
                    wr = w3[:, r::stride, :].flip(1).permute(2, 1, 0).reshape(Cin, n * Cout).contiguous()
                    ml = ctx.nz_in[r] if ctx.nz_in is not None else None
                    K.gemm(dzp, wr, dx_full, U, Cin, n * Cout, a_kmajor=1, b_kmajor=1, lda=Cout, ldb=n * Cout, ldc=stride * Cin,
                           batch0=B, sa=((Lout + 2) * Cout, 0), sc=(rows * Cin, 0), a_off=(2 - n) * Cout,
                           c_off=(Cin if dx_padded else 0) + r * Cin, dact=L.ACT_GELU if prev_z is not None else L.ACT_NONE,
                           aux_in=pz_base, ld_aux_in=stride * Cin, split_k=1, m_len=ml)
                dx = dx_full[:, 1:1 + Lin] if dx_padded else dx_full
            else:
                dz2 = dz_rows.reshape(B * Lout, Cout) if dzp is None else dzp[:, 1:1 + Lout].reshape(B * Lout, Cout)
                dcol = torch.empty(B * Lout, k * Cin, dtype=dy.dtype, device=dy.device)
                K.gemm(dz2, w_cl, dcol, B * Lout, k * Cin, Cout, a_kmajor=1, b_kmajor=0, lda=Cout, ldb=k * Cin, ldc=k * Cin, split_k=1)
                pzc = prev_z if prev_z is None else prev_z.contiguous()
                dx = K.col2im1d(dcol, pzc, B, Lin, Lout, Cin, k, stride, pad, L.ACT_GELU if prev_z is not None else 0)
        if ctx.needs_input_grad[1]:
            part = torch.empty(B, Cout, k * Cin, dtype=torch.float32, device=dy.device)
            wgs = B * ((Cout + 255) // 256) * ((k * Cin + 255) // 256)
            rem = wgs % 256
            sk = 2 if (wgs >= 256 and 0 < rem < 192 and Lout >= 2048) else 1
            dw = torch.empty(Cout, k * Cin, dtype=w_cl.dtype, device=dy.device)
            K.gemm(dz_rows, xp, part, Cout, k * Cin, Lout, a_kmajor=0, b_kmajor=0, lda=Cout, ldb=stride * Cin, ldc=k * Cin, batch0=B,
                   sa=(dz_bs, 0), sb=(xp.stride(0), 0), sc=(Cout * k * Cin, 0), a_off=dz_off, split_k=sk, k_len=ctx.nz_out, reduce_to=dw)
        if has_bias and ctx.needs_input_grad[2]:
            db = K.colsum(dz_rows.reshape(B * Lout, Cout) if dzp is None else dzp[:, 1:1 + Lout].reshape(B * Lout, Cout), w_cl.dtype)
        return dx, dw, db, None, None, None, None, None, None, None, None, None


def conv1d_cl(x, weight, bias, stride, pad=0, act=None, prev_z=None, grad_is_dz=False, nz_out=None, nz_in=None, unread_ok=False):
    Cout, Cin, k = weight.shape
    w_cl = weight.permute(0, 2, 1).reshape(Cout, k * Cin)
    if not w_cl.is_contiguous():
        w_cl = w_cl.contiguous()
    return _Conv1dCLFn.apply(x, w_cl, bias, k, stride, pad, _ACT[act], prev_z, bool(grad_is_dz), nz_out, nz_in, bool(unread_ok))


_POSCONV_DW_SPLIT = int(_os.environ.get("CST_POSCONV_DW_SPLIT", 1))
_POSCONV_WINDOW_CG, _POSCONV_WINDOW_KMAX = 48, 128


class _PosConvFn(torch.autograd.Function):

    @staticmethod
    def forward(ctx, x, weight, bias, groups, lens=None, grad_rows=None, grad_rows_host=None):
        B, T, C = x.shape
        k = weight.shape[2]
        cg = C // groups
        padl = k // 2
        Tp = T + k - 1 + (1 if k % 2 == 0 else 0)
        ml = None if lens is None else torch.clamp(lens.to(torch.int32) + padl, max=T).contiguous()
        window = (x.dtype == torch.bfloat16 and weight.dtype == x.dtype and cg == _POSCONV_WINDOW_CG and k <= _POSCONV_WINDOW_KMAX
                  and (bias is None or bias.dtype == x.dtype) and not _os.environ.get("CST_POSCONV_GEMM"))
        ctx.window = window
        if window:
            xc = x.contiguous()
            wg = weight.view(groups, cg, cg, k).permute(0, 1, 3, 2).contiguous()
            y, z = K.posconv_fwd(xc, wg, bias, groups, ml)
            ctx.save_for_backward(xc, weight, z)
            ctx.cfg = (B, T, C, k, groups, cg, padl, Tp)
            ctx.grad_rows, ctx.grad_rows_host = grad_rows, grad_rows_host
            return y
        xg = torch.empty(groups, B, Tp, cg, dtype=x.dtype, device=x.device)
        xg[:, :, :padl].zero_()
        xg[:, :, padl + T:].zero_()
        xg[:, :, padl:padl + T] = x.view(B, T, groups, cg).permute(2, 0, 1, 3)
        wg = weight.view(groups, cg, cg, k).permute(0, 1, 3, 2).contiguous()
        y = torch.empty(B, T, C, dtype=x.dtype, device=x.device)
        z = torch.empty_like(y)
        xc = x.contiguous()
        K.gemm(xg, wg, y, T, cg, k * cg, a_kmajor=1, b_kmajor=1, lda=cg, ldb=k * cg, ldc=C, batch0=B, batch1=groups,
               sa=(Tp * cg, B * Tp * cg), sb=(0, cg * k * cg), sc=(T * C, cg), bias=bias, sbias=(0, cg), act=L.ACT_GELU,
               aux_out=z, ld_aux_out=C, resid=xc, ld_resid=C, split_k=1, m_len=ml)
        ctx.save_for_backward(xg, weight, z)
        ctx.cfg = (B, T, C, k, groups, cg, padl, Tp)
        ctx.grad_rows, ctx.grad_rows_host = grad_rows, grad_rows_host
        return y

    @staticmethod
    def backward(ctx, dy):
        xg, weight, z = ctx.saved_tensors
        B, T, C, k, groups, cg, padl, Tp = ctx.cfg
        dy = dy.contiguous()
        dz = K.act_bwd(dy, z, L.ACT_GELU)
        dx = dw = db = None
        window = ctx.window and (_POSCONV_DW_SPLIT == 1 or not ctx.needs_input_grad[1])
        if ctx.window and not window:
            xc = xg
            xg = torch.zeros(groups, B, Tp, cg, dtype=xc.dtype, device=xc.device)
            xg[:, :, padl:padl + T] = xc.view(B, T, groups, cg).permute(2, 0, 1, 3)
        lp = k - 1 - padl
        dzg = None
        if (ctx.needs_input_grad[0] or ctx.needs_input_grad[1]) and not window:
            dzg = torch.empty(groups, B, Tp, cg, dtype=dy.dtype, device=dy.device)
            dzg[:, :, :lp].zero_()
            dzg[:, :, lp + T:].zero_()
            dzg[:, :, lp:lp + T] = dz.view(B, T, groups, cg).permute(2, 0, 1, 3)
        if ctx.needs_input_grad[0]:
            wflip = weight.view(groups, cg, cg, k).flip(3).permute(0, 2, 3, 1).contiguous()
            gr = ctx.grad_rows
            ml = None if gr is None else torch.clamp(gr.to(torch.int32) + lp, max=T).contiguous()
            if window:
                dx = K.posconv_dx(dz, wflip, dy, groups, ml)
            else:
                dx = torch.empty(B, T, C, dtype=dy.dtype, device=dy.device)
                K.gemm(dzg, wflip, dx, T, cg, k * cg, a_kmajor=1, b_kmajor=1, lda=cg, ldb=k * cg, ldc=C, batch0=B, batch1=groups,
                       sa=(Tp * cg, B * Tp * cg), sb=(0, cg * k * cg), sc=(T * C, cg), resid=dy, ld_resid=C, split_k=1, m_len=ml)
        if ctx.needs_input_grad[1]:
            Kr = B * Tp - (k - 1)
            if ctx.needs_input_grad[2] and not _os.environ.get("CST_NO_GEMM_COLSUM"):
                db = torch.empty(C, dtype=dy.dtype, device=dy.device)
            live = None
            if ctx.grad_rows is not None and not _os.environ.get("CST_GEMM_NO_KLIVE"):
                if ctx.grad_rows_host is not None:
                    import numpy as np
                    n = np.asarray(ctx.grad_rows_host, dtype=np.int64)
                    ks = np.arange((Kr + 63) // 64, dtype=np.int64) * 64
                    b0 = ks // Tp
                    t0 = ks - b0 * Tp
                    nxt = np.minimum(b0 + 1, B - 1)
                    st = ((t0 < n[b0]) | ((t0 + 64 > Tp) & (b0 + 1 < B) & (n[nxt] > 0))).astype(np.int32)
                    stamps = torch.from_numpy(st).pin_memory().to(dy.device, non_blocking=True)
                else:
                    n = ctx.grad_rows.to(torch.int64)
                    ks = torch.arange((Kr + 63) // 64, device=dy.device, dtype=torch.int64) * 64
                    b0 = torch.div(ks, Tp, rounding_mode="floor")
                    t0 = ks - b0 * Tp
                    nxt = torch.clamp(b0 + 1, max=B - 1)
                    stamps = ((t0 < n[b0]) | ((t0 + 64 > Tp) & (b0 + 1 < B) & (n[nxt] > 0))).to(torch.int32)
                live = (stamps, 1)
            if window:
                dw = K.posconv_dw(dz, xg, groups, k, db, live)
            else:
                dwg = torch.empty(groups, cg, k * cg, dtype=torch.float32, device=dy.device)
                K.gemm(dzg, xg, dwg, cg, k * cg, Kr, a_kmajor=0, b_kmajor=0, lda=cg, ldb=cg, ldc=k * cg, batch0=1, batch1=groups,
                       sa=(0, B * Tp * cg), sb=(0, B * Tp * cg), sc=(0, cg * k * cg), a_off=lp * cg, split_k=_POSCONV_DW_SPLIT, colsum=db,
                       k_live=live)
                dw = dwg.view(groups, cg, k, cg).permute(0, 1, 3, 2).reshape(C, cg, k).to(weight.dtype)
                if db is not None:
                    db = db.to(weight.dtype)
        if ctx.needs_input_grad[2] and db is None:
            db = K.colsum(dz.view(B * T, C), weight.dtype)
        return dx, dw, db, None, None, None, None


class _WeightNormFn(torch.autograd.Function):

    @staticmethod
    def forward(ctx, v, g):
        vc, gc = v.contiguous(), g.reshape(-1).contiguous()
        w, norm = K.weight_norm_fwd(vc, gc)
        ctx.save_for_backward(vc, gc, norm)
        ctx.gshape = g.shape
        return w

    @staticmethod
    def backward(ctx, dw):
        vc, gc, norm = ctx.saved_tensors
        dv, dg = K.weight_norm_bwd(vc, gc, dw.contiguous(), norm)
        return dv, dg.view(ctx.gshape)


def weight_norm_last_dim(v, g):
    return _WeightNormFn.apply(v, g)


def pos_conv_gelu_residual(x, weight, bias, groups, lens=None, grad_rows=None, grad_rows_host=None):
    return _PosConvFn.apply(x, weight, bias, groups, lens, grad_rows, grad_rows_host)


class _GluFn(torch.autograd.Function):
    @staticmethod
    def forward(ctx, z):
        z2 = _flat2d(z)
        ctx.save_for_backward(z2)
        ctx.shape = z.shape
        return K.glu_fwd(z2).view(*z.shape[:-1], z.shape[-1] // 2)

    @staticmethod
    def backward(ctx, dy):
        (z2,) = ctx.saved_tensors
        return K.glu_bwd(_flat2d(dy), z2).view(ctx.shape)


def glu(z):
    return _GluFn.apply(z)


class _MaskRowsFn(torch.autograd.Function):
    @staticmethod
    def forward(ctx, x, mask):
        m = mask.reshape(-1).to(torch.uint8).contiguous()
        ctx.save_for_backward(m)
        ctx.shape = x.shape
        return K.mask_rows(_flat2d(x), m).view(x.shape)

    @staticmethod
    def backward(ctx, dy):
        (m,) = ctx.saved_tensors
        return K.mask_rows(_flat2d(dy), m).view(ctx.shape), None


def mask_rows(x, mask):
    return _MaskRowsFn.apply(x, mask)


class _DropoutFn(torch.autograd.Function):

    @staticmethod
    def forward(ctx, x, p, key):
        ctx.p, ctx.key = p, key
        xc = x.contiguous()
        return K.dropout(xc, p, key).view(x.shape)

    @staticmethod
    def backward(ctx, dy):
        dc = dy.contiguous()
        return K.dropout(dc, ctx.p, ctx.key).view(dy.shape), None, None


def dropout(x, p, key=None):
    if p <= 0.0:
        return x
    from . import rng
    return _DropoutFn.apply(x, float(p), rng.next_key() if key is None else key)


class _EmbedPosFn(torch.autograd.Function):

    @staticmethod
    def forward(ctx, tokens, pad_mask, embed, x, pos_table, scale, pad_idx, p, key):
        out = K.embed_pos_fwd(tokens, pad_mask, embed, x, pos_table, scale, pad_idx, p, key)
        ctx.save_for_backward(tokens)
        ctx.cfg = (scale, pad_idx, p, key, embed.shape[0] if embed is not None else 0, embed.dtype if embed is not None else None)
        return out

    @staticmethod
    def backward(ctx, dy):
        (tokens,) = ctx.saved_tensors
        scale, pad_idx, p, key, V, gdt = ctx.cfg
        dy = dy.contiguous()
        if V:
            dE = K.embed_bwd(dy, tokens, V, scale, pad_idx, p, key, gdt) if ctx.needs_input_grad[2] else None
            return None, None, dE, None, None, None, None, None, None
        dx = K.dropout_scale(dy, scale, p, key) if ctx.needs_input_grad[3] else None
        return None, None, None, dx, None, None, None, None, None


def embed_positions(tokens=None, pad_mask=None, embed=None, x=None, pos_table=None, scale=1.0, pad_idx=1, dropout_p=0.0):
    if pad_mask is not None:
        pad_mask = pad_mask.to(torch.uint8).contiguous()
    if tokens is not None:
        tokens = tokens.contiguous()
    if x is not None and not x.is_contiguous():
        x = x.contiguous()
    return _EmbedPosFn.apply(tokens, pad_mask, embed, x, pos_table, float(scale), int(pad_idx), *_drop_args(dropout_p))


class _LsCeFn(torch.autograd.Function):
    @staticmethod
    def forward(ctx, logits, target, eps, pad):
        l2 = _flat2d(logits)
        t = target.reshape(-1).contiguous()
        out2, lse = K.ls_ce_fwd(l2, t, eps, pad)
        ctx.save_for_backward(l2, t, lse)
        ctx.cfg = (eps, pad, logits.shape)
        ctx.mark_non_differentiable(out2)
        return out2[0].clone(), out2

    @staticmethod
    def backward(ctx, dloss, _):
        l2, t, lse = ctx.saved_tensors
        eps, pad, shape = ctx.cfg
        g = dloss.reshape(1).float().contiguous()
        return K.ls_ce_bwd(l2, t, lse, g, eps, pad).view(shape), None, None, None


def label_smoothed_nll_loss(logits, target, eps, pad):
    loss, out2 = _LsCeFn.apply(logits, target, float(eps), int(pad))
    return loss, out2[1]


class _CtcFn(torch.autograd.Function):
    @staticmethod
    def forward(ctx, logits, targets, target_len, input_len, blank, zero_infinity):
        loss, nll, saved = K.ctc_fwd(logits, targets, target_len, input_len, blank, zero_infinity, need_grad=ctx.needs_input_grad[0])
        ctx.save_for_backward(*[t for t in saved if t is not None])
        ctx.cfg = (blank, zero_infinity)
        ctx.mark_non_differentiable(nll)
        return loss[0].clone(), nll

    @staticmethod
    def backward(ctx, dloss, _):
        blank, zero_infinity = ctx.cfg
        g = dloss.reshape(1).float().contiguous()
        return K.ctc_bwd(ctx.saved_tensors, g, blank, zero_infinity), None, None, None, None, None


def ctc_loss(logits, targets, target_len, input_len, blank=0, zero_infinity=False):
    return _CtcFn.apply(logits, targets, target_len, input_len, int(blank), bool(zero_infinity))


def ctc_greedy(logits, input_len, blank=0):
    return K.ctc_greedy(logits, input_len, int(blank))


class _InfoNceFn(torch.autograd.Function):
    @staticmethod
    def forward(ctx, x, y, idx, inv_temp):
        loss, nll, counters, saved, _ = K.infonce_fwd(x, y, idx, inv_temp)
        ctx.save_for_backward(*saved)
        ctx.inv_temp = inv_temp
        ctx.mark_non_differentiable(nll, counters)
        return loss[0].clone(), nll, counters

    @staticmethod
    def backward(ctx, dloss, _nll, _counters):
        g = dloss.reshape(1).float().contiguous()
        dx, dy = K.infonce_bwd(ctx.saved_tensors, g, ctx.inv_temp, need_dy=ctx.needs_input_grad[1])
        return (dx if ctx.needs_input_grad[0] else None), dy, None, None


def infonce_loss(x, y, neg_idx, logit_temp):
    return _InfoNceFn.apply(x, y, neg_idx, 1.0 / float(logit_temp))


def sample_negatives(B, M, num_negatives, cross_sample_negatives=0, key=None, device="cuda"):
# ... 98 lines not shown
```

### chimera-st_amd/kernels.py

```python
import ctypes
import os

import torch

from . import lib as L

_ws = {}
STATS = {}


def workspace(nbytes: int, device) -> torch.Tensor:
    key = (device.index, L.stream_ptr().value)
    t = _ws.get(key)
    if t is None or t.numel() < nbytes:
        t = torch.empty(max(nbytes, 1 << 20), dtype=torch.uint8, device=device)
        _ws[key] = t
    return t


class _Deferred:

    MAX_BYTES = 32 << 20

    def __init__(self):
        self.on, self.items, self.keep, self.flushes = 0, [], [], 0
        self.main = None
        self.side = None
        self.side_used = False
        self.poison = False

    def push(self, src_ptr, dst, stride, Lr, P, keep, order=0):
        if self.poison:
            dst.fill_(float("nan"))
        if self.side_used and torch.is_tensor(keep) and torch.cuda.current_stream() != self.main:
            keep.record_stream(self.main)
        self.items.append((src_ptr, dst.data_ptr(), stride, Lr, P, L.dtype_code(dst.dtype), order))
        self.keep.append((keep, dst.detach()))

    def join(self):
        if self.side_used:
            torch.cuda.current_stream().wait_stream(self.side)
            self.side_used = False

    def flush(self):
        self.join()
        if self.items:
            reduce_multi(self.items)
            self.flushes += 1
            self.items, self.keep = [], []


DEFER = _Deferred()


def reduce_multi(items):
    lib = L.load()
    for at in range(0, len(items), 64):
        chunk = items[at:at + 64]
        arr = (L.ReduceItem * len(chunk))()
        for a, (src, dst, stride, Lr, P, dt, order) in zip(arr, chunk):
            a.src, a.dst, a.stride, a.L, a.P, a.dst_dtype, a.order = src, dst, stride, Lr, P, dt, order
        L.check(lib.cst_reduce_multi(arr, len(chunk), L.stream_ptr()), "cst_reduce_multi")


class deferred_reductions:

    def __init__(self, enabled=True):
        self.enabled = bool(enabled) and not os.environ.get("CST_NO_DEFER")

    def __enter__(self):
        if self.enabled:
            DEFER.on += 1
            DEFER.main = torch.cuda.current_stream()
            DEFER.poison = bool(os.environ.get("CST_DEFER_POISON"))
        return self

    def __exit__(self, *exc):
        if self.enabled:
            DEFER.on -= 1
            if DEFER.on == 0:
                DEFER.flush()
        return False


def side_gemm(big, reads, *args, **kw):
    if big or not DEFER.on or DEFER.main is None or not os.environ.get("CST_SIDE_STREAM") or torch.cuda.current_stream() != DEFER.main:
        return gemm(*args, **kw)
    if DEFER.side is None:
        DEFER.side = torch.cuda.Stream()
    side = DEFER.side
    side.wait_stream(DEFER.main)
    DEFER.side_used = True
    with torch.cuda.stream(side):
        out = gemm(*args, **kw)
    for t in reads:
        if t is not None:
            t.record_stream(side)
    STATS["side_gemm"] = STATS.get("side_gemm", 0) + 1
    return out


def _2d(t):
    assert t.dim() == 2 and t.stride(1) == 1, "expected a row-major 2-D tensor, got %s / %s" % (tuple(t.shape), t.stride())
    return t


def _stamps(live, extent, stat):
    if live is None:
        return None, 0
    assert live[0].numel() * 64 >= extent and live[0].dtype == torch.int32
    STATS[stat] = STATS.get(stat, 0) + 1
    return live[0].data_ptr(), live[1]


def _per_batch(v, batch0, stat):
    if v is None:
        return None
    assert v.dtype == torch.int32 and v.numel() == batch0 and v.is_contiguous()
    STATS[stat] = STATS.get(stat, 0) + 1
    return v.data_ptr()


def gemm(A, B, C, M, N, K, *, a_kmajor, b_kmajor, lda, ldb, ldc, bias=None, bias_mode=L.BIAS_COL, act=L.ACT_NONE,
         aux_out=None, ld_aux_out=0, dact=L.ACT_NONE, aux_in=None, ld_aux_in=0, resid=None, ld_resid=0, alpha=1.0,
         batch0=1, batch1=1, sa=(0, 0), sb=(0, 0), sc=(0, 0), sbias=(0, 0), a_seg=0, a_seg_stride=0, b_seg=0,
         b_seg_stride=0, split_k=-1, a_off=0, b_off=0, c_off=0, drop_p=0.0, drop_key=0, k_live=None, m_live=None, k_len=None, m_len=None,
         ws=None, colsum=None, defer=False, reduce_to=None):
    lib = L.load()
    d = L.GemmDesc()
    d.dtype = L.dtype_code(A.dtype)
    assert B.dtype == A.dtype, "A/B dtype mismatch"
    d.c_dtype = L.dtype_code(C.dtype)
    d.a_kmajor, d.b_kmajor = int(a_kmajor), int(b_kmajor)
    d.M, d.N, d.K = M, N, K
    es = A.element_size()
    d.A = A.data_ptr() + a_off * es
    d.lda, d.a_seg, d.a_seg_stride = lda, a_seg, a_seg_stride
    d.B = B.data_ptr() + b_off * es
    d.ldb, d.b_seg, d.b_seg_stride = ldb, b_seg, b_seg_stride
    d.C = C.data_ptr() + c_off * C.element_size()
    d.ldc = ldc
    if bias is not None:
        assert bias.dtype == A.dtype
        d.bias, d.bias_mode = bias.data_ptr(), bias_mode
    else:
        d.bias, d.bias_mode = None, L.BIAS_NONE
    d.sbias0, d.sbias1 = sbias
    d.act = act
    d.aux_out = None if aux_out is None else aux_out.data_ptr() + c_off * es
    d.ld_aux_out = ld_aux_out
    d.dact = dact
    d.aux_in = None if aux_in is None else aux_in.data_ptr() + c_off * es
    d.ld_aux_in = ld_aux_in
    d.resid = None if resid is None else resid.data_ptr() + c_off * es
    d.ld_resid = ld_resid
    d.alpha = alpha
    d.drop_p, d.drop_key = float(drop_p), int(drop_key) & 0xFFFFFFFF
    d.batch0, d.batch1 = batch0, batch1
    d.sa0, d.sa1 = sa
    d.sb0, d.sb1 = sb
    d.sc0, d.sc1 = sc
    d.split_k = split_k
    d.k_live, d.k_epoch = _stamps(k_live, K, "gemm_k_live")
    d.m_live, d.m_epoch = _stamps(m_live, M, "gemm_m_live")
    d.k_len = _per_batch(k_len, batch0, "gemm_k_len")
    d.m_len = _per_batch(m_len, batch0, "gemm_m_len")
    if colsum is not None:
        assert not a_kmajor and colsum.dtype == A.dtype and colsum.is_contiguous() and colsum.numel() == M * batch0 * batch1
        d.colsum = colsum.data_ptr()
    else:
        d.colsum = None
    d.defer_reduce = 0
    splits = 1
    need = lib.cst_gemm_workspace(ctypes.byref(d))
    nb = batch0 * batch1
    deferred = False
    if need > 0 and (reduce_to is not None or (defer and DEFER.on and nb == 1 and need <= DEFER.MAX_BYTES and ldc == N and N % 8 == 0)):
        splits = lib.cst_gemm_splits(ctypes.byref(d))
        if splits > 1:
            assert ws is None and bias is None and act == L.ACT_NONE and dact == L.ACT_NONE and resid is None and aux_out is None and alpha == 1.0
            ws = torch.empty(need, dtype=torch.uint8, device=A.device)
            d.defer_reduce = 1
            deferred = True
    if need > 0:
        if ws is None:
            ws = workspace(need, A.device)
        assert ws.dtype == torch.uint8 and ws.numel() >= need, "split-K scratch too small: %d < %d" % (ws.numel(), need)
        d.workspace, d.workspace_bytes = ws.data_ptr(), ws.numel()
    else:
        d.workspace, d.workspace_bytes = None, 0
    L.check(lib.cst_gemm(ctypes.byref(d), L.stream_ptr()), "cst_gemm")
    if reduce_to is not None:
        assert C.dtype == torch.float32 and sc == (M * N, 0) and ldc == N and reduce_to.numel() == M * N and reduce_to.is_contiguous() and colsum is None
        item = ((ws.data_ptr(), reduce_to, M * N, M * N, nb * splits, ws) if deferred else (C.data_ptr(), reduce_to, M * N, M * N, nb, C))
        if defer and DEFER.on:
            DEFER.push(*item)
        else:
            reduce_multi([(item[0], item[1].data_ptr(), item[2], item[3], item[4], L.dtype_code(reduce_to.dtype), 0)])
    elif deferred:
        DEFER.push(ws.data_ptr(), C, M * N, M * N, splits, ws)
        if colsum is not None:
            DEFER.push(ws.data_ptr() + 4 * splits * M * N, colsum, M, M, splits, ws)
    return C


_DW_FUSED = {}


def dw_colsum_is_fused(n_out, k_in, tokens, dtype):
    key = (n_out, k_in, tokens, dtype)
    r = _DW_FUSED.get(key)
    if r is None:
        d = L.GemmDesc()
        d.dtype = d.c_dtype = L.dtype_code(dtype)
        d.a_kmajor = d.b_kmajor = 0
        d.M, d.N, d.K = n_out, k_in, tokens
        d.batch0 = d.batch1 = 1
        d.split_k = -1
        d.colsum = 1
        r = _DW_FUSED[key] = bool(L.load().cst_gemm_colsum_is_fused(ctypes.byref(d)))
        if len(_DW_FUSED) > 4096:
            _DW_FUSED.clear()
    return r


def layernorm_fwd(x, res, gamma, beta, eps, want_sum=False):
    x = _2d(x)
    rows, cols = x.shape
    y = torch.empty_like(x)
    s = torch.empty_like(x) if (want_sum and res is not None) else None
    mean = torch.empty(rows, dtype=torch.float32, device=x.device)
    rstd = torch.empty(rows, dtype=torch.float32, device=x.device)
    L.check(L.load().cst_layernorm_fwd(L.ptr(x), L.ptr(res), L.ptr(gamma), L.ptr(beta), L.ptr(y), L.ptr(s), L.ptr(mean),
                                       L.ptr(rstd), rows, cols, eps, L.dtype_code(x.dtype), L.stream_ptr()), "cst_layernorm_fwd")
    return y, s, mean, rstd


_EPOCH = [0x3C6EF372]


def next_epoch():
    _EPOCH[0] = (_EPOCH[0] % 0xFFFFFFFE) + 1
    return _EPOCH[0]


def _two_stage(wbytes, outs, defer, launch):
    deferred = bool(defer) and DEFER.on > 0
    dev = outs[0].device
    ws = torch.empty(wbytes, dtype=torch.uint8, device=dev) if deferred else workspace(wbytes, dev)
    launch(ws, *[None if deferred else L.ptr(o) for o in outs])
    if deferred:
        n, cols = len(outs), outs[0].numel()
        for i, o in enumerate(outs):
            DEFER.push(ws.data_ptr() + 4 * cols * i, o, n * cols, cols, wbytes // (4 * n * cols), ws, order=1)


def layernorm_bwd(dy, s, gamma, mean, rstd, dres=None, grad_dtype=torch.float32, want_tiles=False, defer=False):
    dy, s = _2d(dy), _2d(s)
    rows, cols = s.shape
    lib = L.load()
    dx = torch.empty_like(s)
    dg = torch.empty(cols, dtype=grad_dtype, device=s.device)
    db = torch.empty(cols, dtype=grad_dtype, device=s.device)
    stamps, epoch = (torch.empty((rows + 63) // 64, dtype=torch.int32, device=s.device), next_epoch()) if want_tiles else (None, 0)

    def launch(ws, pg, pb):
        if want_tiles:
            L.check(lib.cst_layernorm_bwd_tiles(L.ptr(dy), L.ptr(s), L.ptr(gamma), L.ptr(mean), L.ptr(rstd), L.ptr(dres), L.ptr(dx), pg,
                                                pb, L.ptr(ws), rows, cols, L.dtype_code(s.dtype), L.dtype_code(grad_dtype),
                                                L.ptr(stamps), epoch, L.stream_ptr()), "cst_layernorm_bwd_tiles")
        else:
            L.check(lib.cst_layernorm_bwd(L.ptr(dy), L.ptr(s), L.ptr(gamma), L.ptr(mean), L.ptr(rstd), L.ptr(dres), L.ptr(dx), pg,
                                          pb, L.ptr(ws), rows, cols, L.dtype_code(s.dtype), L.dtype_code(grad_dtype), L.stream_ptr()),
                    "cst_layernorm_bwd")

    _two_stage(lib.cst_layernorm_bwd_workspace(rows, cols), (dg, db), defer, launch)
    return (dx, dg, db, (stamps, epoch)) if want_tiles else (dx, dg, db)


def _bhtd_strides(t, layout):
    assert t.stride(-1) == 1
    if layout == "bt":
        return t.stride(0), None, t.stride(1)
    return t.stride(1), None, t.stride(0)


def attn_desc(q, k, v, o, lse, H, D, kpm, causal, scale, layout_q="bt", layout_kv="bt", drop_p=0.0, drop_key=0, kv_len=None, seq=None):
    d = L.AttnDesc()
    d.dtype = L.dtype_code(q.dtype)
    if layout_q == "bt":
        B, Tq = q.shape[0], q.shape[1]
    else:
        Tq, B = q.shape[0], q.shape[1]
    Tk = k.shape[1] if layout_kv == "bt" else k.shape[0]
    if seq is not None:
        assert layout_q == "bt" and layout_kv == "bt" and B == 1 and kpm is None
        assert seq[0].dtype == torch.int32 and seq[0].is_contiguous()
        B, Tq, Tk = seq[0].numel() - 1, int(seq[1]), int(seq[1])
        d.seq_offsets = seq[0].data_ptr()
        STATS["attn_packed"] = STATS.get("attn_packed", 0) + 1
    else:
        d.seq_offsets = None
    d.B, d.H, d.Tq, d.Tk, d.D = B, H, Tq, Tk, D

    def st(t, lay):
        sb, _, stt = _bhtd_strides(t, lay)
        return sb, D, stt

    d.Q = q.data_ptr(); d.q_sb, d.q_sh, d.q_st = st(q, layout_q)
    d.K = k.data_ptr(); d.k_sb, d.k_sh, d.k_st = st(k, layout_kv)
    d.V = v.data_ptr(); d.v_sb, d.v_sh, d.v_st = st(v, layout_kv)
    d.O = o.data_ptr(); d.o_sb, d.o_sh, d.o_st = st(o, layout_q)
    d.lse = lse.data_ptr()
    if kpm is not None:
        assert kpm.dtype == torch.uint8 and kpm.stride(1) == 1 and kpm.shape == (B, Tk)
        d.key_padding_mask, d.kpm_stride = kpm.data_ptr(), kpm.stride(0)
        bits = kpm_bits(kpm)
        d.kpm_bits = bits.data_ptr()
        d._kpm_bits_owner = bits
    else:
        d.key_padding_mask, d.kpm_stride = None, 0
        d.kpm_bits = None
    d.bwd_ws = None
    d.causal, d.scale = int(causal), scale
    if q.dtype == torch.bfloat16 and D == 64 and not causal and not os.environ.get("CST_ATTN_GENERIC"):
        STATS["attn_fast"] = STATS.get("attn_fast", 0) + 1
    d.drop_p, d.drop_key = float(drop_p), int(drop_key) & 0xFFFFFFFF
    if kv_len is not None:
        assert (kpm is not None or seq is not None) and kv_len.dtype == torch.int32 and kv_len.numel() == B and kv_len.is_contiguous()
        d.kv_len = kv_len.data_ptr()
        STATS["attn_kv_len"] = STATS.get("attn_kv_len", 0) + 1
    else:
        d.kv_len = None
    return d


_KPM_BITS = []
_BIT_WEIGHTS = {}


def kpm_bits(kpm):
    key = (kpm.data_ptr(), tuple(kpm.shape), kpm._version)
    for ptr, shape, ver, _, bits in _KPM_BITS:
        if (ptr, shape, ver) == key:
            return bits
    B, Tk = kpm.shape
    nw = (Tk + 63) // 64
    m = kpm != 0
    if nw * 64 != Tk:
        m = torch.cat([m, torch.ones(B, nw * 64 - Tk, dtype=torch.bool, device=kpm.device)], 1)
    w = _BIT_WEIGHTS.get(kpm.device)
    if w is None:
        w = _BIT_WEIGHTS[kpm.device] = torch.ones(64, dtype=torch.int64, device=kpm.device) << torch.arange(64, dtype=torch.int64, device=kpm.device)
    bits = (m.view(B, nw, 64).to(torch.int64) * w).sum(-1).contiguous()
    _KPM_BITS.append(key + (kpm, bits))
    if len(_KPM_BITS) > 8:
        _KPM_BITS.pop(0)
    return bits


def attn_fwd(q, k, v, H, D, kpm, causal, scale, layout_q="bt", layout_kv="bt", drop_p=0.0, drop_key=0, kv_len=None):
    o = torch.empty_like(q)
    if layout_q == "bt":
        B, Tq = q.shape[0], q.shape[1]
    else:
        Tq, B = q.shape[0], q.shape[1]
    lse = torch.empty(B, H, Tq, dtype=torch.float32, device=q.device)
    d = attn_desc(q, k, v, o, lse, H, D, kpm, causal, scale, layout_q, layout_kv, drop_p, drop_key, kv_len)
    L.check(L.load().cst_attn_fwd(ctypes.byref(d), L.stream_ptr()), "cst_attn_fwd")
    return o, lse


def attn_fwd_desc(d):
    L.check(L.load().cst_attn_fwd(ctypes.byref(d), L.stream_ptr()), "cst_attn_fwd")


def attn_bwd_desc(d):
    L.check(L.load().cst_attn_bwd(ctypes.byref(d), L.stream_ptr()), "cst_attn_bwd")


def attn_bwd_fill(d, do, dq, dk, dv, delta, D, layout_q="bt", layout_kv="bt"):
    def st(t, lay):
        sb, _, stt = _bhtd_strides(t, lay)
        return sb, D, stt

    d.dO = do.data_ptr(); d.do_sb, d.do_sh, d.do_st = st(do, layout_q)
    d.dQ = dq.data_ptr(); d.dq_sb, d.dq_sh, d.dq_st = st(dq, layout_q)
    d.dK = dk.data_ptr(); d.dk_sb, d.dk_sh, d.dk_st = st(dk, layout_kv)
    d.dV = dv.data_ptr(); d.dv_sb, d.dv_sh, d.dv_st = st(dv, layout_kv)
    d.delta = delta.data_ptr()
    flags = torch.empty(int(d.B) * int(d.H) * ((int(d.Tq) + 63) // 64), dtype=torch.uint8, device=do.device)
    d.q_flags = flags.data_ptr()
    STATS["attn_q_flags"] = STATS.get("attn_q_flags", 0) + 1
    d._q_flags_owner = flags
    ws = torch.empty(int(L.load().cst_attn_bwd_workspace(ctypes.byref(d))) // 4, dtype=torch.float32, device=do.device)
    d.bwd_ws = ws.data_ptr()
    d._bwd_ws_owner = ws


def attn_bwd(do, q, k, v, o, lse, H, D, kpm, causal, scale, layout_q="bt", layout_kv="bt", drop_p=0.0, drop_key=0, kv_len=None, seq=None,
             grads=None):
    dq, dk, dv = grads if grads is not None else (torch.empty_like(q), torch.empty_like(k), torch.empty_like(v))
    delta = torch.empty_like(lse)
    d = attn_desc(q, k, v, o, lse, H, D, kpm, causal, scale, layout_q, layout_kv, drop_p, drop_key, kv_len, seq)
    attn_bwd_fill(d, do, dq, dk, dv, delta, D, layout_q, layout_kv)
    attn_bwd_desc(d)
    return dq, dk, dv


def conv0_fwd(wav, w, gamma, beta, k, stride, eps=1e-5, frame_limit=None):
    assert wav.dtype == torch.float32 and wav.is_contiguous()
    B, S = wav.shape
    C = w.shape[0]
    Lo = (S - k) // stride + 1
    y = torch.empty(B, Lo, C, dtype=w.dtype, device=wav.device)
    mean = torch.empty(B, C, dtype=torch.float32, device=wav.device)
    rstd = torch.empty(B, C, dtype=torch.float32, device=wav.device)
    gram = torch.empty(B, k * k + k, dtype=torch.float32, device=wav.device)
    lib = L.load()
    ws = workspace(lib.cst_conv0_fwd_workspace(B, S, k, stride), wav.device)
    L.check(lib.cst_conv0_gn_gelu_fwd(L.ptr(wav), L.ptr(w), L.ptr(gamma), L.ptr(beta), L.ptr(y), L.ptr(mean), L.ptr(rstd),
                                      L.ptr(gram), L.ptr(ws), _lim(frame_limit, B), B, S, C, k, stride, eps, L.dtype_code(w.dtype),
                                      L.stream_ptr()), "cst_conv0_gn_gelu_fwd")
    return y, mean, rstd, gram


def _lim(frame_limit, B):
    if frame_limit is None:
        return None
    assert frame_limit.dtype == torch.int32 and frame_limit.numel() == B and frame_limit.is_contiguous()
    STATS["conv0_frame_limit"] = STATS.get("conv0_frame_limit", 0) + 1
    return L.ptr(frame_limit)


def conv0_bwd(dy, wav, w, gamma, beta, mean, rstd, gram, k, stride, frame_limit=None):
    B, S = wav.shape
    C = w.shape[0]
    lib = L.load()
    dw = torch.empty(C, k, dtype=torch.float32, device=wav.device)
    dg = torch.empty(C, dtype=torch.float32, device=wav.device)
    db = torch.empty(C, dtype=torch.float32, device=wav.device)
    ws = workspace(lib.cst_conv0_bwd_workspace(B, S, C, k, stride), wav.device)
    L.check(lib.cst_conv0_gn_gelu_bwd(L.ptr(dy), L.ptr(wav), L.ptr(w), L.ptr(gamma), L.ptr(beta), L.ptr(mean), L.ptr(rstd),
                                      L.ptr(gram), L.ptr(dw), L.ptr(dg), L.ptr(db), L.ptr(ws), _lim(frame_limit, B), B, S, C, k, stride,
                                      L.dtype_code(w.dtype), L.stream_ptr()), "cst_conv0_gn_gelu_bwd")
    return dw, dg, db


def conv0_ln_fwd(wav, w, bias, gamma, beta, k, stride, eps=1e-5, frame_limit=None):
    assert wav.dtype == torch.float32 and wav.is_contiguous()
    B, S = wav.shape
    C = w.shape[0]
    Lo = (S - k) // stride + 1
    y = torch.empty(B, Lo, C, dtype=w.dtype, device=wav.device)
    mean = torch.empty(B, Lo, dtype=torch.float32, device=wav.device)
    rstd = torch.empty(B, Lo, dtype=torch.float32, device=wav.device)
    L.check(L.load().cst_conv0_ln_gelu_fwd(L.ptr(wav), L.ptr(w), L.ptr(bias), L.ptr(gamma), L.ptr(beta), L.ptr(y), L.ptr(mean),
                                           L.ptr(rstd), _lim(frame_limit, B), B, S, C, k, stride, eps, L.dtype_code(w.dtype),
                                           L.stream_ptr()), "cst_conv0_ln_gelu_fwd")
    return y, mean, rstd


def conv0_ln_bwd(dy, wav, w, bias, gamma, beta, mean, rstd, k, stride, frame_limit=None):
    B, S = wav.shape
    C = w.shape[0]
    lib = L.load()
    dw = torch.empty(C, k, dtype=torch.float32, device=wav.device)
    dbi, dg, db = (torch.empty(C, dtype=torch.float32, device=wav.device) for _ in range(3))
    ws = workspace(lib.cst_conv0_ln_bwd_workspace(B, S, C, k, stride), wav.device)
    L.check(lib.cst_conv0_ln_gelu_bwd(L.ptr(dy), L.ptr(wav), L.ptr(w), L.ptr(bias), L.ptr(gamma), L.ptr(beta), L.ptr(mean),
                                      L.ptr(rstd), L.ptr(dw), L.ptr(dbi), L.ptr(dg), L.ptr(db), L.ptr(ws), _lim(frame_limit, B), B, S,
                                      C, k, stride, L.dtype_code(w.dtype), L.stream_ptr()), "cst_conv0_ln_gelu_bwd")
    return dw, dbi, dg, db


def _row_lim(row_limit, B):
    if row_limit is None:
        return None
    assert row_limit.dtype == torch.int32 and row_limit.numel() == B and row_limit.is_contiguous()
    return L.ptr(row_limit)


def ln_gelu_fwd(u, gamma, beta, eps=1e-5, row_limit=None):
    assert u.dim() == 3 and u.is_contiguous()
    B, Lr, C = u.shape
    y = torch.empty_like(u)
    mean = torch.empty(B, Lr, dtype=torch.float32, device=u.device)
    rstd = torch.empty(B, Lr, dtype=torch.float32, device=u.device)
    L.check(L.load().cst_ln_gelu_fwd(L.ptr(u), L.ptr(gamma), L.ptr(beta), L.ptr(y), L.ptr(mean), L.ptr(rstd), _row_lim(row_limit, B),
                                     B, Lr, C, eps, L.dtype_code(u.dtype), L.stream_ptr()), "cst_ln_gelu_fwd")
    return y, mean, rstd


def ln_gelu_bwd(dy, u, gamma, beta, mean, rstd, row_limit=None, want_colsum=False, padded=False):
    assert dy.is_contiguous() and u.is_contiguous()
    B, Lr, C = u.shape
    lib = L.load()
    if padded:
        full = torch.empty(B, Lr + 2, C, dtype=u.dtype, device=u.device)
        full[:, 0].zero_()
        full[:, Lr + 1].zero_()
# ... 567 lines not shown
```

### chimera-st_amd/lib.py

```python
import ctypes
import os

import torch

_HERE = os.path.dirname(os.path.abspath(__file__))
LIB_PATH = os.path.join(_HERE, "libcst_hip.so")
ABI_VERSION = 13

F32, BF16 = 0, 1
ACT_NONE, ACT_RELU, ACT_GELU = 0, 1, 2
BIAS_NONE, BIAS_COL, BIAS_ROW = 0, 1, 2
K_GEMM, K_ATTN_FWD, K_ATTN_BWD, K_LAYERNORM, K_CONV0, K_ELEMENTWISE, K_LOSS, K_OPTIM = range(8)
KERNEL_CLASSES = ["gemm", "attn_fwd", "attn_bwd", "layernorm", "conv0", "elementwise", "loss", "optim"]

c_i64, c_int, c_f, c_p = ctypes.c_int64, ctypes.c_int, ctypes.c_float, ctypes.c_void_p


class GemmDesc(ctypes.Structure):
    _fields_ = [
        ("dtype", c_int), ("c_dtype", c_int), ("a_kmajor", c_int), ("b_kmajor", c_int),
        ("M", c_i64), ("N", c_i64), ("K", c_i64),
        ("A", c_p), ("lda", c_i64), ("a_seg", c_i64), ("a_seg_stride", c_i64),
        ("B", c_p), ("ldb", c_i64), ("b_seg", c_i64), ("b_seg_stride", c_i64),
        ("C", c_p), ("ldc", c_i64),
        ("bias", c_p), ("bias_mode", c_int), ("sbias0", c_i64), ("sbias1", c_i64),
        ("act", c_int),
        ("aux_out", c_p), ("ld_aux_out", c_i64),
        ("dact", c_int),
        ("aux_in", c_p), ("ld_aux_in", c_i64),
        ("resid", c_p), ("ld_resid", c_i64),
        ("alpha", c_f),
        ("drop_p", c_f), ("drop_key", ctypes.c_uint32),
        ("batch0", c_i64), ("batch1", c_i64),
        ("sa0", c_i64), ("sa1", c_i64), ("sb0", c_i64), ("sb1", c_i64), ("sc0", c_i64), ("sc1", c_i64),
        ("split_k", c_int),
        ("workspace", c_p), ("workspace_bytes", c_i64),
        ("k_live", c_p), ("k_epoch", ctypes.c_uint32),
        ("m_live", c_p), ("m_epoch", ctypes.c_uint32),
        ("k_len", c_p),
        ("m_len", c_p),
        ("colsum", c_p),
        ("defer_reduce", c_int),
    ]


class ReduceItem(ctypes.Structure):
    _fields_ = [("src", c_p), ("dst", c_p), ("stride", c_i64), ("L", c_i64), ("P", ctypes.c_int32), ("dst_dtype", ctypes.c_int32),
                ("block0", ctypes.c_int32), ("order", ctypes.c_int32)]


class AttnDesc(ctypes.Structure):
    _fields_ = [
        ("dtype", c_int),
        ("B", c_i64), ("H", c_i64), ("Tq", c_i64), ("Tk", c_i64), ("D", c_i64),
        ("Q", c_p), ("q_sb", c_i64), ("q_sh", c_i64), ("q_st", c_i64),
        ("K", c_p), ("k_sb", c_i64), ("k_sh", c_i64), ("k_st", c_i64),
        ("V", c_p), ("v_sb", c_i64), ("v_sh", c_i64), ("v_st", c_i64),
        ("O", c_p), ("o_sb", c_i64), ("o_sh", c_i64), ("o_st", c_i64),
        ("lse", c_p),
        ("key_padding_mask", c_p), ("kpm_stride", c_i64),
        ("causal", c_int), ("scale", c_f),
        ("drop_p", c_f), ("drop_key", ctypes.c_uint32),
        ("dO", c_p), ("do_sb", c_i64), ("do_sh", c_i64), ("do_st", c_i64),
        ("dQ", c_p), ("dq_sb", c_i64), ("dq_sh", c_i64), ("dq_st", c_i64),
        ("dK", c_p), ("dk_sb", c_i64), ("dk_sh", c_i64), ("dk_st", c_i64),
        ("dV", c_p), ("dv_sb", c_i64), ("dv_sh", c_i64), ("dv_st", c_i64),
        ("delta", c_p),
        ("kv_len", c_p),
        ("q_flags", c_p),
        ("seq_offsets", c_p),
        ("kpm_bits", c_p),
        ("bwd_ws", c_p),
    ]


class BeamDesc(ctypes.Structure):
    _fields_ = [
        ("dtype", c_int),
        ("bsz", c_i64), ("beam", c_i64), ("vocab", c_i64), ("max_len", c_i64),
        ("pad", c_i64), ("unk", c_i64), ("eos", c_i64), ("min_len", c_i64),
        ("unk_penalty", c_f), ("len_penalty", c_f), ("temperature", c_f),
        ("normalize_scores", c_int),
        ("logits", c_p), ("ld_logits", c_i64),
        ("step", c_p),
        ("tokens", c_p), ("scores", c_p), ("anc", c_p),
        ("cands_to_ignore", c_p), ("finished", c_p), ("nfinal", c_p), ("num_remaining", c_p),
        ("fin_tokens", c_p), ("fin_pos", c_p), ("fin_score", c_p), ("fin_len", c_p),
        ("workspace", c_p),
        ("members", c_i64), ("logits_n", c_p * 7), ("lprobs_out", c_p),
        ("no_repeat_ngram", c_i64), ("prefix_tokens", c_p), ("prefix_len", c_i64),
        ("sampling", c_i64), ("sample_topk", c_i64), ("sample_topp", c_f), ("sample_key", c_p),
        ("diverse_groups", c_i64), ("diverse_strength", c_f), ("diverse_siblings", c_i64), ("sibling_rate", c_f),
        ("fin_anc", c_p),
    ]


class LmFusionDesc(ctypes.Structure):
    _fields_ = [("lm_logits", c_p), ("lm_weight", c_f), ("lprobs_out", c_p)]


class LexDesc(ctypes.Structure):
    _fields_ = [("representation", c_i64), ("constraints", c_p), ("width", c_i64), ("workspace", c_p)]


LEX_TBL_W, LEX_SW, LEX_NEXT_MAX, LEX_WIDTH_MAX = 136, 44, 16, 65


def lex_states(workspace, bsz, beam):
    words = workspace.view(torch.int32)
    return words[bsz * LEX_TBL_W:bsz * LEX_TBL_W + 2 * bsz * beam * LEX_SW].view(2, bsz * beam, LEX_SW)


class FbankDesc(ctypes.Structure):
    _fields_ = [
        ("B", c_i64), ("S", c_i64), ("T", c_i64),
        ("wave", c_p), ("n_samples", c_p), ("out", c_p), ("n_frames", c_p),
        ("utterance_cmvn", c_int), ("norm_means", c_int), ("norm_vars", c_int),
        ("global_mean", c_p), ("global_std", c_p),
        ("global_first", c_int),
        ("specaugment", c_int),
        ("n_fmask", c_int), ("n_tmask", c_int),
        ("fmask", c_p), ("tmask", c_p),
        ("mask_mean", c_int), ("mask_value", c_f),
        ("workspace", c_p), ("workspace_bytes", c_i64),
    ]


SYMBOLS = [
    ("cst_last_error", ctypes.c_char_p, []),
    ("cst_version", c_int, []),
    ("cst_device_arch_ok", c_int, []),
    ("cst_prof_enable", None, [c_int]),
    ("cst_prof_query", c_i64, [c_int, ctypes.POINTER(ctypes.c_double), ctypes.POINTER(ctypes.c_double), ctypes.POINTER(ctypes.c_double)]),
    ("cst_layernorm_fwd", c_int, [c_p, c_p, c_p, c_p, c_p, c_p, c_p, c_p, c_i64, c_i64, c_f, c_int, c_p]),
    ("cst_layernorm_bwd_workspace", c_i64, [c_i64, c_i64]),
    ("cst_layernorm_bwd", c_int, [c_p, c_p, c_p, c_p, c_p, c_p, c_p, c_p, c_p, c_p, c_i64, c_i64, c_int, c_int, c_p]),
    ("cst_layernorm_bwd_tiles", c_int, [c_p, c_p, c_p, c_p, c_p, c_p, c_p, c_p, c_p, c_p, c_i64, c_i64, c_int, c_int, c_p, ctypes.c_uint32, c_p]),
    ("cst_gemm_workspace", c_i64, [ctypes.POINTER(GemmDesc)]),
    ("cst_gemm_colsum_is_fused", c_int, [ctypes.POINTER(GemmDesc)]),
    ("cst_gemm_splits", c_int, [ctypes.POINTER(GemmDesc)]),
    ("cst_gemm_route", c_int, [ctypes.POINTER(GemmDesc), ctypes.c_char_p, c_i64]),
    ("cst_reduce_multi", c_int, [ctypes.POINTER(ReduceItem), c_int, c_p]),
    ("cst_gemm", c_int, [ctypes.POINTER(GemmDesc), c_p]),
    ("cst_posconv_fwd", c_int, [c_p, c_p, c_p, c_p, c_p, c_p, c_i64, c_i64, c_i64, c_i64, c_i64, c_p]),
    ("cst_posconv_dx", c_int, [c_p, c_p, c_p, c_p, c_p, c_i64, c_i64, c_i64, c_i64, c_i64, c_p]),
    ("cst_posconv_dw", c_int, [c_p, c_p, c_p, c_p, c_p, ctypes.c_uint32, c_i64, c_i64, c_i64, c_i64, c_i64, c_p]),
    ("cst_prof_dump", c_i64, [c_int, ctypes.c_char_p, c_i64]),
    ("cst_gemm_reserve_cus", c_int, [c_int]),
    ("cst_transpose2d", c_int, [c_p, c_p, c_i64, c_i64, c_int, c_p]),
    ("cst_transpose2d_multi", c_int, [c_p, c_int, c_i64, c_int, c_p]),
    ("cst_weight_norm_workspace", c_i64, [c_i64, c_i64]),
    ("cst_weight_norm_fwd", c_int, [c_p, c_p, c_p, c_p, c_p, c_i64, c_i64, c_int, c_p]),
    ("cst_weight_norm_bwd", c_int, [c_p, c_p, c_p, c_p, c_p, c_p, c_p, c_i64, c_i64, c_int, c_p]),
    ("cst_attn_bwd_workspace", c_i64, [ctypes.POINTER(AttnDesc)]),
    ("cst_attn_fwd", c_int, [ctypes.POINTER(AttnDesc), c_p]),
    ("cst_attn_bwd", c_int, [ctypes.POINTER(AttnDesc), c_p]),
    ("cst_conv0_fwd_workspace", c_i64, [c_i64, c_i64, c_int, c_int]),
    ("cst_conv0_gn_gelu_fwd", c_int, [c_p, c_p, c_p, c_p, c_p, c_p, c_p, c_p, c_p, c_p, c_i64, c_i64, c_i64, c_int, c_int, c_f, c_int, c_p]),
    ("cst_conv0_bwd_workspace", c_i64, [c_i64, c_i64, c_i64, c_int, c_int]),
    ("cst_conv0_gn_gelu_bwd", c_int, [c_p, c_p, c_p, c_p, c_p, c_p, c_p, c_p, c_p, c_p, c_p, c_p, c_p, c_i64, c_i64, c_i64, c_int, c_int, c_int, c_p]),
    ("cst_conv0_ln_gelu_fwd", c_int, [c_p, c_p, c_p, c_p, c_p, c_p, c_p, c_p, c_p, c_i64, c_i64, c_i64, c_int, c_int, c_f, c_int, c_p]),
    ("cst_conv0_ln_bwd_workspace", c_i64, [c_i64, c_i64, c_i64, c_int, c_int]),
    ("cst_conv0_ln_gelu_bwd", c_int, [c_p, c_p, c_p, c_p, c_p, c_p, c_p, c_p, c_p, c_p, c_p, c_p, c_p, c_p, c_i64, c_i64, c_i64, c_int, c_int, c_int, c_p]),
    ("cst_ln_gelu_fwd", c_int, [c_p, c_p, c_p, c_p, c_p, c_p, c_p, c_i64, c_i64, c_i64, c_f, c_int, c_p]),
    ("cst_ln_gelu_bwd_workspace", c_i64, [c_i64, c_i64]),
    ("cst_ln_gelu_bwd", c_int, [c_p, c_p, c_p, c_p, c_p, c_p, c_p, c_i64, c_p, c_p, c_p, c_p, c_p, c_i64, c_i64, c_i64, c_int, c_p]),
    ("cst_glu_fwd", c_int, [c_p, c_p, c_i64, c_i64, c_int, c_p]),
    ("cst_glu_bwd", c_int, [c_p, c_p, c_p, c_i64, c_i64, c_int, c_p]),
    ("cst_act_bwd", c_int, [c_p, c_p, c_p, c_i64, c_int, c_int, c_p]),
    ("cst_act_fwd", c_int, [c_p, c_p, c_i64, c_int, c_int, c_p]),
    ("cst_colsum", c_int, [c_p, c_i64, c_p, c_i64, c_i64, c_int, c_p]),
    ("cst_colsum_workspace", c_i64, [c_i64, c_i64]),
    ("cst_colsum_typed", c_int, [c_p, c_i64, c_p, c_p, c_i64, c_i64, c_int, c_int, c_p]),
    ("cst_colsum_typed_live", c_int, [c_p, c_i64, c_p, c_p, c_i64, c_i64, c_int, c_int, c_p, ctypes.c_uint32, c_p]),
    ("cst_col2im1d", c_int, [c_p, c_p, c_p, c_i64, c_i64, c_i64, c_i64, c_int, c_int, c_int, c_int, c_int, c_p]),
    ("cst_mask_rows", c_int, [c_p, c_p, c_p, c_i64, c_i64, c_int, c_p]),
    ("cst_dropout", c_int, [c_p, c_p, c_i64, c_f, ctypes.c_uint32, c_int, c_p]),
    ("cst_rows_pack", c_int, [c_p, c_p, c_p, c_i64, c_i64, c_i64, c_int, c_int, c_p]),
    ("cst_rows_unpack", c_int, [c_p, c_p, c_p, c_i64, c_i64, c_i64, c_int, c_int, c_p]),
    ("cst_dec_linear", c_int, [c_p, c_p, c_p, c_p, c_p, c_i64, c_i64, c_i64, c_i64, c_i64, c_i64, c_int, c_p, c_i64, c_int, c_p]),
    ("cst_dec_ln_linear", c_int, [c_p, c_p, c_p, c_p, c_f, c_p, c_p, c_i64, c_i64, c_i64, c_i64, c_i64, c_i64, c_int, c_p, c_i64, c_int, c_p]),
    ("cst_dropout_colsum", c_int, [c_p, c_p, c_p, c_p, c_i64, c_i64, c_int, c_int, c_f, ctypes.c_uint32, c_p, ctypes.c_uint32, c_p]),
    ("cst_conv_row_limits", c_int, [c_p, c_p, c_p, c_int, c_i64, c_p, c_i64, c_int, c_p]),
    ("cst_dropout_scale", c_int, [c_p, c_p, c_i64, c_f, c_f, ctypes.c_uint32, c_int, c_p]),
    ("cst_embed_pos_fwd", c_int, [c_p, c_p, c_p, c_p, c_p, c_f, c_i64, c_p, c_i64, c_i64, c_i64, c_i64, c_i64, c_f, ctypes.c_uint32, c_int, c_p]),
    ("cst_embed_bwd", c_int, [c_p, c_p, c_p, c_f, c_i64, c_i64, c_i64, c_i64, c_f, ctypes.c_uint32, c_int, c_int, c_p]),
    ("cst_ls_ce_fwd", c_int, [c_p, c_p, c_p, c_p, c_p, c_i64, c_i64, c_f, c_i64, c_int, c_p]),
    ("cst_ls_ce_bwd", c_int, [c_p, c_p, c_p, c_p, c_p, c_i64, c_i64, c_f, c_i64, c_int, c_p]),
    ("cst_score_tokens", c_int, [c_p, ctypes.POINTER(c_p), c_i64, c_i64, c_p, c_i64, c_p, c_p, c_p, c_i64, c_i64, c_i64, c_int, c_p]),
    ("cst_ctc_fwd", c_int, [c_p, c_i64, c_i64, c_p, c_i64, c_p, c_p, c_i64, c_int, c_p, c_p, c_p, c_p, c_p, c_p, c_i64, c_i64, c_i64, c_int, c_p]),
    ("cst_ctc_bwd", c_int, [c_p, c_i64, c_i64, c_p, c_i64, c_p, c_p, c_i64, c_int, c_p, c_p, c_p, c_p, c_p, c_p, c_i64, c_i64, c_i64, c_i64, c_i64,
                            c_int, c_p]),
    ("cst_ctc_greedy", c_int, [c_p, c_i64, c_i64, c_p, c_i64, c_p, c_p, c_p, c_i64, c_i64, c_i64, c_int, c_p]),
    ("cst_w2v_negatives", c_int, [ctypes.c_uint32, c_i64, c_i64, c_i64, c_i64, c_p, c_p]),
    ("cst_infonce_fwd", c_int, [c_p, c_p, c_p, c_f, c_p, c_p, c_p, c_p, c_p, c_p, c_p, c_p, c_i64, c_i64, c_i64, c_int, c_p]),
    ("cst_infonce_bwd_x", c_int, [c_p, c_p, c_p, c_f, c_p, c_p, c_p, c_p, c_p, c_p, c_i64, c_i64, c_i64, c_int, c_p]),
    ("cst_infonce_bwd_y", c_int, [c_p, c_p, c_p, c_p, c_p, c_p, c_p, c_p, c_i64, c_i64, c_i64, c_int, c_p]),
    ("cst_gumbel_vq_workspace", c_i64, [c_i64, c_i64, c_i64]),
    ("cst_gumbel_vq_fwd", c_int, [c_p, c_p, c_p, ctypes.c_uint32, c_int, c_p, c_p, c_p, c_p, c_p, c_p, c_p, c_i64, c_i64, c_i64, c_i64, c_int, c_p]),
    ("cst_gumbel_vq_bwd", c_int, [c_p, c_p, ctypes.c_uint32, c_f, c_p, c_p, c_p, c_p, c_p, c_i64, c_i64, c_i64, c_int, c_p]),
    ("cst_contrastive_fwd", c_int, [c_p, c_p, c_p, c_p, c_p, c_p, c_p, c_i64, c_i64, c_i64, c_f, c_int, c_p]),
    ("cst_contrastive_bwd", c_int, [c_p, c_p, c_p, c_p, c_p, c_p, c_p, c_p, c_i64, c_i64, c_i64, c_f, c_int, c_p]),
    ("cst_sumsq_workspace", c_i64, []),
    ("cst_sumsq", c_int, [c_p, c_i64, c_p, c_p, c_int, c_p]),
    ("cst_adam_step", c_int, [c_p, c_p, c_p, c_p, c_p, c_i64, c_f, c_f, c_f, c_f, c_f, c_i64, c_p, c_int, c_int, c_p]),
    ("cst_beam_workspace", c_i64, [c_i64, c_i64]),
    ("cst_beam_init", c_int, [ctypes.POINTER(BeamDesc), c_p]),
    ("cst_beam_step", c_int, [ctypes.POINTER(BeamDesc), c_p]),
    ("cst_beam_step_lm", c_int, [ctypes.POINTER(BeamDesc), ctypes.POINTER(LmFusionDesc), c_p]),
    ("cst_lex_workspace", c_i64, [c_i64, c_i64, c_i64]),
    ("cst_lex_init", c_int, [ctypes.POINTER(BeamDesc), ctypes.POINTER(LexDesc), c_p]),
    ("cst_beam_step_lex", c_int, [ctypes.POINTER(BeamDesc), ctypes.POINTER(LmFusionDesc), ctypes.POINTER(LexDesc), c_p]),
    ("cst_dec_embed", c_int, [c_p, c_p, c_p, c_p, c_f, c_i64, c_p, c_i64, c_i64, c_i64, c_i64, c_int, c_p]),
    ("cst_dec_self_attn", c_int, [c_p, c_p, c_p, c_p, c_p, c_p, c_i64, c_i64, c_i64, c_i64, c_f, c_int, c_p]),
    ("cst_batch_by_size", c_i64, [c_p, c_i64, c_i64, c_i64, ctypes.c_int32, c_p]),
    ("cst_wav_info", c_int, [ctypes.c_char_p, c_p, c_p, c_p, c_p]),
    ("cst_wav_read_f32", c_i64, [ctypes.c_char_p, c_i64, c_i64, c_p, c_i64]),
    ("cst_edit_distance", c_i64, [c_p, c_i64, c_p, c_i64]),
    ("cst_dec_cross_attn", c_int, [c_p, c_p, c_p, c_p, c_p, c_p, c_i64, c_i64, c_i64, c_i64, c_i64, c_i64, c_f, c_int, c_p]),
    ("cst_fbank_workspace_bytes", c_i64, [c_i64, c_i64]),
    ("cst_fbank", c_int, [ctypes.POINTER(FbankDesc), c_p]),
    ("cst_dec_ln_q_cross_attn", c_int, [c_p, c_i64, c_p, c_p, c_p, c_f, c_p, c_p, c_p, c_p, c_p, c_i64, c_i64, c_i64, c_i64, c_i64, c_i64, c_f, c_int, c_p]),
    ("cst_attn_avg_probs", c_int, [c_p, c_i64, c_p, c_i64, c_i64, c_i64, c_p, c_p, c_i64, c_p, c_i64, c_i64, c_i64, c_i64, c_i64, c_i64, c_f, c_f,
                                   c_int, c_int, c_p]),
    ("cst_collate_pairs", c_int, [c_p, c_p, c_int, c_p, c_p, c_i64, c_p, c_i64, c_i64, c_i64, c_i64, c_i64, c_int, c_int, c_p, c_p]),
    ("cst_token_block_slices", c_i64, [c_p, c_i64, c_int, c_i64, c_i64, c_p, c_i64]),
    ("cst_token_block_index", c_int, [c_p, c_i64, c_p, c_i64, c_p]),
    ("cst_collate_blocks", c_int, [c_p, c_int, c_p, c_i64, c_p, c_i64, c_i64, c_i64, c_i64, c_p, c_p]),
]

_lib = None


def load():
    global _lib
    if _lib is not None:
        return _lib
    if not os.path.exists(LIB_PATH):
        raise RuntimeError(
            "chimera-st_amd: %s is missing — the HIP extension is the product path and there is no fallback. "
            "Build it with `python -c 'import __graft_entry__ as g; g.build()'` or `make -C chimera-st_amd/csrc`." % LIB_PATH)
    lib = ctypes.CDLL(LIB_PATH)
    for name, res, args in SYMBOLS:
        fn = getattr(lib, name)
        fn.restype = res
        fn.argtypes = args
    built = lib.cst_version()
    if built != ABI_VERSION:
        raise RuntimeError("chimera-st_amd: %s was built for ABI version %d, this package binds version %d (include/cst.h "
                           "CST_ABI_VERSION) — rebuild it with `make -C chimera-st_amd/csrc`." % (LIB_PATH, built, ABI_VERSION))
    _lib = lib
    return lib


def check(rc, what=""):
    if rc != 0:
        msg = load().cst_last_error()
        raise RuntimeError("libcst_hip %s failed (%d): %s" % (what, rc, msg.decode() if msg else "?"))


def dtype_code(t: torch.dtype) -> int:
    if t == torch.float32:
        return F32
    if t == torch.bfloat16:
        return BF16
    raise TypeError("chimera-st_amd kernels compute in float32 or bfloat16 storage, got %s" % t)


_DEV_INDEX = None


def stream_ptr():
    global _DEV_INDEX
    if _DEV_INDEX is None:
        _DEV_INDEX = torch.cuda.current_device()
    return ctypes.c_void_p(torch._C._cuda_getCurrentRawStream(_DEV_INDEX))


def ptr(t):
    if t is None:
        return None
    if not t.is_cuda:
        raise RuntimeError("chimera-st_amd: tensor is not on the GPU — the HIP path has no CPU fallback")
    return ctypes.c_void_p(t.data_ptr())


def prof_enable(on: bool):
    load().cst_prof_enable(1 if on else 0)


def prof_query():
    lib = load()
    out = {}
    for i, name in enumerate(KERNEL_CLASSES):
        ms, fl, by = ctypes.c_double(), ctypes.c_double(), ctypes.c_double()
        n = lib.cst_prof_query(i, ctypes.byref(ms), ctypes.byref(fl), ctypes.byref(by))
        out[name] = dict(launches=int(n), ms=ms.value, flops=fl.value, bytes=by.value)
    return out


def prof_dump(cls):
    lib = load()
    n = lib.cst_prof_dump(cls, None, 0)
    buf = ctypes.create_string_buffer(int(n) + 16)
    lib.cst_prof_dump(cls, buf, len(buf))
    out = []
    for line in buf.value.decode().splitlines():
        ms, fl, by, *tag = line.split(" ", 3)
        out.append((float(ms), float(fl), float(by), tag[0] if tag else ""))
    return out
```

### chimera-st_amd/s2t_transformer.py

```python
import math
from typing import Dict, List, Optional

import os

import torch
import torch.nn as nn

from . import functional as CF
from .fairseq_model import (EncoderOut, FairseqEncoder, FairseqEncoderDecoderModel, FairseqIncrementalDecoder,
                            lengths_to_padding_mask)
from .modules import (Embedding, FairseqDropout, LayerNorm, Linear, PositionalEmbedding, TransformerDecoderLayer,
                      TransformerEncoderLayer, causal_mask, to_batch_major, to_time_major_view)
from .registry import register_model, register_model_architecture


class Conv1dSubsampler(nn.Module):

    def __init__(self, in_channels, mid_channels, out_channels, kernel_sizes=(3, 3)):
        super().__init__()
        self.n_layers = len(kernel_sizes)
        self.conv_layers = nn.ModuleList()
        for i, k in enumerate(kernel_sizes):
            cin = in_channels if i == 0 else mid_channels // 2
            cout = mid_channels if i < self.n_layers - 1 else out_channels * 2
            conv = nn.Module()
            ref = nn.Conv1d(cin, cout, k, stride=2, padding=k // 2)
            conv.weight = nn.Parameter(ref.weight.detach().clone())
            conv.bias = nn.Parameter(ref.bias.detach().clone())
            conv.kernel_size = k
            self.conv_layers.append(conv)

    def input_reach(self):
        r = 0
        for conv in reversed(self.conv_layers):
            r = 2 * r + (conv.kernel_size - 1 - conv.kernel_size // 2)
        return r

    def get_out_seq_lens_tensor(self, in_seq_lens_tensor):
        out = in_seq_lens_tensor.clone()
        for _ in range(self.n_layers):
            out = ((out.float() - 1) / 2 + 1).floor().long()
        return out

    def forward(self, src_tokens, src_lengths, padding_unread=False):
        x = src_tokens
        lens = [src_lengths]
        for _ in range(self.n_layers):
            lens.append(((lens[-1].float() - 1) / 2 + 1).floor().long())
        limits = [None] * self.n_layers
        if padding_unread and not os.environ.get("CST_NO_MLEN"):
            need = lens[-1]
            for i in reversed(range(self.n_layers)):
                limits[i] = need.to(torch.int32).contiguous()
                k = self.conv_layers[i].kernel_size
                need = (need - 1) * 2 + (k - k // 2)
        for i, conv in enumerate(self.conv_layers):
            z, _ = CF.conv1d_cl(x, conv.weight, conv.bias, 2, pad=conv.kernel_size // 2, nz_out=limits[i], unread_ok=limits[i] is not None)
            x = CF.glu(z)
        return to_time_major_view(x), lens[-1]


class TransformerDecoder(FairseqIncrementalDecoder):

    def __init__(self, args, dictionary, embed_tokens, no_encoder_attn=False):
        self.args = args
        super().__init__(dictionary)
        self.register_buffer("version", torch.Tensor([3]))
        self._future_mask = None
        self.dropout_module = FairseqDropout(args.dropout, module_name=self.__class__.__name__)
        self.decoder_layerdrop = getattr(args, "decoder_layerdrop", 0.0)
        assert self.decoder_layerdrop == 0.0
        self.share_input_output_embed = args.share_decoder_input_output_embed
        input_embed_dim = embed_tokens.embedding_dim
        embed_dim = args.decoder_embed_dim
        self.embed_dim = embed_dim
        self.output_embed_dim = getattr(args, "decoder_output_dim", embed_dim)
        assert input_embed_dim == embed_dim and self.output_embed_dim == embed_dim
        self.padding_idx = embed_tokens.padding_idx
        self.max_target_positions = args.max_target_positions
        self.embed_tokens = embed_tokens
        self.embed_scale = 1.0 if getattr(args, "no_scale_embedding", False) else math.sqrt(embed_dim)
        self.project_in_dim = None
        self.embed_positions = (PositionalEmbedding(args.max_target_positions, embed_dim, self.padding_idx,
                                                    learned=getattr(args, "decoder_learned_pos", False))
                                if not getattr(args, "no_token_positional_embeddings", False) else None)
        self.layernorm_embedding = None
        self.cross_self_attention = False
        self.layers = nn.ModuleList([TransformerDecoderLayer(args, no_encoder_attn) for _ in range(args.decoder_layers)])
        self.num_layers = len(self.layers)
        if args.decoder_normalize_before and not getattr(args, "no_decoder_final_norm", False):
            self.layer_norm = LayerNorm(embed_dim)
        else:
            self.layer_norm = None
        self.project_out_dim = None
        self.adaptive_softmax = None
        if self.share_input_output_embed:
            self.output_projection = Linear(self.embed_tokens.weight.shape[1], self.embed_tokens.weight.shape[0], bias=False)
            self.output_projection.weight = self.embed_tokens.weight
        else:
            self.output_projection = Linear(self.output_embed_dim, len(dictionary), bias=False)
            nn.init.normal_(self.output_projection.weight, mean=0, std=self.output_embed_dim ** -0.5)

    def forward(self, prev_output_tokens, encoder_out=None, incremental_state=None, features_only=False,
                full_context_alignment=False, alignment_layer=None, alignment_heads=None, src_lengths=None,
                return_all_hiddens=False, **unused):
        x, extra = self.extract_features(prev_output_tokens, encoder_out=encoder_out, incremental_state=incremental_state,
                                         full_context_alignment=full_context_alignment, alignment_layer=alignment_layer,
                                         alignment_heads=alignment_heads)
        if not features_only:
            x = self.output_layer(x)
        return x, extra

    def extract_features(self, prev_output_tokens, encoder_out=None, incremental_state=None, full_context_alignment=False,
                         alignment_layer=None, alignment_heads=None):
        return self.extract_features_scriptable(prev_output_tokens, encoder_out, incremental_state, full_context_alignment,
                                                alignment_layer, alignment_heads)

    def extract_features_scriptable(self, prev_output_tokens, encoder_out=None, incremental_state=None,
                                    full_context_alignment=False, alignment_layer=None, alignment_heads=None):
        if alignment_heads is not None:
            raise NotImplementedError("alignment_heads: per-head attention weights never leave the fused kernel")
        if alignment_layer is not None and not 0 <= alignment_layer < self.num_layers:
            raise ValueError("alignment_layer %r outside the decoder's %d layers" % (alignment_layer, self.num_layers))
        attn = None
        if incremental_state is None and prev_output_tokens.is_cuda:
            x = CF.embed_positions(tokens=prev_output_tokens, embed=self.embed_tokens.weight,
                                   pos_table=(self.embed_positions.table(prev_output_tokens.size(1), prev_output_tokens.device)
                                              if self.embed_positions is not None else None),
                                   scale=self.embed_scale, pad_idx=self.padding_idx,
                                   dropout_p=self.dropout_module.p if self.training else 0.0)
        else:
            positions = (self.embed_positions(prev_output_tokens, incremental_state=incremental_state)
                         if self.embed_positions is not None else None)
            if incremental_state is not None:
                prev_output_tokens = prev_output_tokens[:, -1:]
                if positions is not None:
                    positions = positions[:, -1:]
            x = self.embed_scale * self.embed_tokens(prev_output_tokens)
            if positions is not None:
                x = x + positions.to(x.dtype)
            x = self.dropout_module(x)
        x = to_time_major_view(x.contiguous())
        if incremental_state is None:
            self_attn_padding_mask = prev_output_tokens.eq(self.padding_idx)
        else:
            self_attn_padding_mask = prev_output_tokens.eq(self.padding_idx) if prev_output_tokens.eq(self.padding_idx).any() else None
        inner_states = [x]
        for idx, layer in enumerate(self.layers):
            if incremental_state is None and not full_context_alignment:
                self_attn_mask = self.buffered_future_mask(x)
            else:
                self_attn_mask = None
            x, layer_attn, _ = layer(x, encoder_out.encoder_out if encoder_out is not None else None,
                                     encoder_out.encoder_padding_mask if encoder_out is not None else None, incremental_state,
                                     self_attn_mask=self_attn_mask, self_attn_padding_mask=self_attn_padding_mask,
                                     need_attn=idx == alignment_layer)
            inner_states.append(x)
            if idx == alignment_layer:
                attn = layer_attn
        if self.layer_norm is not None:
            x = self.layer_norm(x)
        x = x.transpose(0, 1)
        return x, {"attn": [attn], "inner_states": inner_states}

    def output_layer(self, features):
        return self.output_projection(features)

    def max_positions(self):
        if self.embed_positions is None:
            return self.max_target_positions
        return min(self.max_target_positions, self.embed_positions.max_positions)

    def buffered_future_mask(self, tensor):
        dim = tensor.size(0)
        if self._future_mask is None or self._future_mask.device != tensor.device or self._future_mask.size(0) < dim:
            self._future_mask = causal_mask(max(dim, 256), tensor.device)
        m = self._future_mask[:dim, :dim]
        m.cst_kind = "causal"
        return m


class TransformerDecoderScriptable(TransformerDecoder):

    def extract_features(self, prev_output_tokens, encoder_out=None, incremental_state=None, full_context_alignment=False,
                         alignment_layer=None, alignment_heads=None):
        x, extra = self.extract_features_scriptable(prev_output_tokens, encoder_out, incremental_state, full_context_alignment,
                                                    alignment_layer, alignment_heads)
        return x, (None if alignment_layer is None else extra)


def build_embedding(dictionary, embed_dim):
    return Embedding(len(dictionary), embed_dim, dictionary.pad())


def reorder_encoder_out(encoder_out: EncoderOut, new_order):
    return EncoderOut(
        encoder_out=None if encoder_out.encoder_out is None else encoder_out.encoder_out.index_select(1, new_order),
        encoder_padding_mask=None if encoder_out.encoder_padding_mask is None
        else encoder_out.encoder_padding_mask.index_select(0, new_order),
        encoder_embedding=None if encoder_out.encoder_embedding is None
        else encoder_out.encoder_embedding.index_select(0, new_order),
        encoder_states=None, src_tokens=None, src_lengths=None)


@register_model("s2t_transformer")
class S2TTransformerModel(FairseqEncoderDecoderModel):
    single_use_parameters = True

    @staticmethod
    def add_args(parser):
        add_transformer_args(parser)
        parser.add_argument("--conv-kernel-sizes", type=str)
        parser.add_argument("--conv-channels", type=int)
        parser.add_argument("--load-pretrained-encoder-from", type=str, default=None)

    @classmethod
    def build_model(cls, args, task):
        base_architecture(args)
        decoder_embed_tokens = build_embedding(task.target_dictionary, args.decoder_embed_dim)
        encoder = S2TTransformerEncoder(args)
        decoder = TransformerDecoderScriptable(args, task.target_dictionary, decoder_embed_tokens)
        return cls(encoder, decoder)

    def get_normalized_probs(self, net_output, log_probs, sample=None):
        lprobs = self.decoder.get_normalized_probs(net_output, log_probs, sample)
        lprobs.batch_first = True
        return lprobs

    def forward(self, src_tokens, src_lengths, prev_output_tokens, **extra_args):
        encoder_out = self.encoder(src_tokens=src_tokens, src_lengths=src_lengths)
        return self.decoder(prev_output_tokens=prev_output_tokens, encoder_out=encoder_out)


class S2TTransformerEncoder(FairseqEncoder):

    def __init__(self, args):
        super().__init__(None)
        self.dropout_module = FairseqDropout(p=args.dropout, module_name=self.__class__.__name__)
        self.embed_scale = 1.0 if args.no_scale_embedding else math.sqrt(args.encoder_embed_dim)
        self.padding_idx = 1
        self.subsample = Conv1dSubsampler(args.input_feat_per_channel * args.input_channels, args.conv_channels,
                                          args.encoder_embed_dim, [int(k) for k in args.conv_kernel_sizes.split(",")])
        self.embed_positions = PositionalEmbedding(args.max_source_positions, args.encoder_embed_dim, self.padding_idx)
        self.transformer_layers = nn.ModuleList([TransformerEncoderLayer(args) for _ in range(args.encoder_layers)])
        self.layer_norm = LayerNorm(args.encoder_embed_dim) if args.encoder_normalize_before else None

    def forward(self, src_tokens, src_lengths, **extra_args):
        x, input_lengths = self.subsample(src_tokens, src_lengths)
        encoder_padding_mask = lengths_to_padding_mask(input_lengths, max_len=x.size(0))
        x = to_time_major_view(CF.embed_positions(pad_mask=encoder_padding_mask, x=to_batch_major(x),
                                                  pos_table=self.embed_positions.table(encoder_padding_mask.size(1), x.device),
                                                  scale=self.embed_scale, pad_idx=self.padding_idx,
                                                  dropout_p=self.dropout_module.p if self.training else 0.0))
        for layer in self.transformer_layers:
            x = layer(x, encoder_padding_mask)
        if self.layer_norm is not None:
            x = self.layer_norm(x)
        return EncoderOut(encoder_out=x, encoder_padding_mask=encoder_padding_mask, encoder_embedding=None,
                          encoder_states=None, src_tokens=None, src_lengths=None)

    def reorder_encoder_out(self, encoder_out, new_order):
        return reorder_encoder_out(encoder_out, new_order)


def add_transformer_args(parser):
    parser.add_argument("--activation-fn", type=str, default="relu", choices=["relu", "gelu"])
    parser.add_argument("--dropout", type=float, metavar="D")
    parser.add_argument("--attention-dropout", type=float, metavar="D")
    parser.add_argument("--activation-dropout", "--relu-dropout", type=float, metavar="D")
    parser.add_argument("--encoder-embed-dim", type=int, metavar="N")
    parser.add_argument("--encoder-ffn-embed-dim", type=int, metavar="N")
    parser.add_argument("--encoder-layers", type=int, metavar="N")
    parser.add_argument("--encoder-attention-heads", type=int, metavar="N")
    parser.add_argument("--encoder-normalize-before", action="store_true")
    parser.add_argument("--decoder-embed-dim", type=int, metavar="N")
    parser.add_argument("--decoder-ffn-embed-dim", type=int, metavar="N")
    parser.add_argument("--decoder-layers", type=int, metavar="N")
    parser.add_argument("--decoder-attention-heads", type=int, metavar="N")
    parser.add_argument("--decoder-normalize-before", action="store_true")
    parser.add_argument("--share-decoder-input-output-embed", action="store_true")
    parser.add_argument("--layernorm-embedding", action="store_true")
    parser.add_argument("--no-scale-embedding", action="store_true")


@register_model_architecture(model_name="s2t_transformer", arch_name="s2t_transformer")
def base_architecture(args):
    args.conv_kernel_sizes = getattr(args, "conv_kernel_sizes", "5,5")
    args.conv_channels = getattr(args, "conv_channels", 1024)
    args.input_feat_per_channel = getattr(args, "input_feat_per_channel", 80)
    args.input_channels = getattr(args, "input_channels", 1)
    args.max_source_positions = getattr(args, "max_source_positions", 6000)
    args.max_target_positions = getattr(args, "max_target_positions", 1024)
    args.encoder_embed_dim = getattr(args, "encoder_embed_dim", 512)
    args.encoder_ffn_embed_dim = getattr(args, "encoder_ffn_embed_dim", 2048)
    args.encoder_layers = getattr(args, "encoder_layers", 12)
    args.encoder_attention_heads = getattr(args, "encoder_attention_heads", 8)
    args.encoder_normalize_before = getattr(args, "encoder_normalize_before", True)
    args.decoder_embed_dim = getattr(args, "decoder_embed_dim", args.encoder_embed_dim)
    args.decoder_ffn_embed_dim = getattr(args, "decoder_ffn_embed_dim", args.encoder_ffn_embed_dim)
    args.decoder_layers = getattr(args, "decoder_layers", 6)
    args.decoder_attention_heads = getattr(args, "decoder_attention_heads", 8)
    args.decoder_normalize_before = getattr(args, "decoder_normalize_before", True)
    args.decoder_learned_pos = getattr(args, "decoder_learned_pos", False)
    args.dropout = getattr(args, "dropout", 0.1)
    args.attention_dropout = getattr(args, "attention_dropout", args.dropout)
    args.activation_dropout = getattr(args, "activation_dropout", args.dropout)
    args.activation_fn = getattr(args, "activation_fn", "relu")
    args.share_decoder_input_output_embed = getattr(args, "share_decoder_input_output_embed", False)
    args.no_token_positional_embeddings = getattr(args, "no_token_positional_embeddings", False)
    args.decoder_layerdrop = getattr(args, "decoder_layerdrop", 0.0)
    args.decoder_output_dim = getattr(args, "decoder_output_dim", args.decoder_embed_dim)
    args.decoder_input_dim = getattr(args, "decoder_input_dim", args.decoder_embed_dim)
    args.no_scale_embedding = getattr(args, "no_scale_embedding", False)
    args.quant_noise_pq = getattr(args, "quant_noise_pq", 0)


def _preset(name, **kw):
    @register_model_architecture("s2t_transformer", name)
    def fn(args):
        for k, v in kw.items():
            setattr(args, k, getattr(args, k, v))
        base_architecture(args)

    fn.__name__ = name
    return fn


s2t_transformer_s = _preset("s2t_transformer_s", encoder_embed_dim=256, encoder_ffn_embed_dim=256 * 8,
                            encoder_attention_heads=4, decoder_attention_heads=4, dropout=0.1)
s2t_transformer_sp = _preset("s2t_transformer_sp", encoder_layers=16, encoder_embed_dim=256, encoder_ffn_embed_dim=256 * 8,
                             encoder_attention_heads=4, decoder_attention_heads=4, dropout=0.1)
s2t_transformer_m = _preset("s2t_transformer_m", encoder_embed_dim=512, encoder_ffn_embed_dim=512 * 4,
                            encoder_attention_heads=8, decoder_attention_heads=8, dropout=0.15)
s2t_transformer_mp = _preset("s2t_transformer_mp", encoder_layers=16, encoder_embed_dim=512, encoder_ffn_embed_dim=512 * 4,
                             encoder_attention_heads=8, decoder_attention_heads=8, dropout=0.15)
s2t_transformer_l = _preset("s2t_transformer_l", encoder_embed_dim=1024, encoder_ffn_embed_dim=1024 * 4,
                            encoder_attention_heads=16, decoder_attention_heads=16, dropout=0.2)
s2t_transformer_lp = _preset("s2t_transformer_lp", encoder_layers=16, encoder_embed_dim=1024, encoder_ffn_embed_dim=1024 * 4,
                             encoder_attention_heads=16, decoder_attention_heads=16, dropout=0.2)
```

### include/cst.h

```cpp
#ifndef CST_H
#define CST_H

#include <stdint.h>

#ifdef __cplusplus
extern "C" {
#endif

#define CST_ABI_VERSION 13

typedef enum { CST_F32 = 0, CST_BF16 = 1 } cst_dtype;

typedef enum {
  CST_OK = 0,
  CST_ERR_BAD_ARG = -1,
  CST_ERR_LAUNCH = -2,
  CST_ERR_WORKSPACE = -3,
  CST_ERR_UNSUPPORTED = -4
} cst_status;

typedef void* cst_stream;

const char* cst_last_error(void);
int cst_version(void);
int cst_device_arch_ok(void);

typedef enum {
  CST_K_GEMM = 0, CST_K_ATTN_FWD, CST_K_ATTN_BWD, CST_K_LAYERNORM, CST_K_CONV0, CST_K_ELEMENTWISE,
  CST_K_LOSS, CST_K_OPTIM, CST_K_NUM
} cst_kernel_class;
void cst_prof_enable(int on);
int64_t cst_prof_query(int kernel_class, double* total_ms, double* flops, double* bytes);
int64_t cst_prof_dump(int kernel_class, char* buf, int64_t cap);

int cst_layernorm_fwd(const void* x, const void* res, const void* gamma, const void* beta,
                      void* y, void* sum_out, float* mean, float* rstd,
                      int64_t rows, int64_t cols, float eps, int dtype, cst_stream stream);
int64_t cst_layernorm_bwd_workspace(int64_t rows, int64_t cols);
int cst_layernorm_bwd(const void* dy, const void* s, const void* gamma, const float* mean,
                      const float* rstd, const void* dres, void* dx, void* dgamma, void* dbeta,
                      void* workspace, int64_t rows, int64_t cols, int dtype, int grad_dtype, cst_stream stream);
int cst_layernorm_bwd_tiles(const void* dy, const void* s, const void* gamma, const float* mean,
                            const float* rstd, const void* dres, void* dx, void* dgamma, void* dbeta,
                            void* workspace, int64_t rows, int64_t cols, int dtype, int grad_dtype,
                            uint32_t* tile_live, uint32_t epoch, cst_stream stream);

typedef enum { CST_ACT_NONE = 0, CST_ACT_RELU = 1, CST_ACT_GELU = 2 } cst_act;
typedef enum { CST_BIAS_NONE = 0, CST_BIAS_COL = 1, CST_BIAS_ROW = 2 } cst_bias_mode;

typedef struct {
  int dtype;
  int c_dtype;
  int a_kmajor, b_kmajor;
  int64_t M, N, K;
  const void* A; int64_t lda, a_seg, a_seg_stride;
  const void* B; int64_t ldb, b_seg, b_seg_stride;
  void* C; int64_t ldc;
  const void* bias; int bias_mode;
  int64_t sbias0, sbias1;
  int act;
  void* aux_out; int64_t ld_aux_out;
  int dact;
  const void* aux_in; int64_t ld_aux_in;
  const void* resid; int64_t ld_resid;
  float alpha;
  float drop_p; uint32_t drop_key;
  int64_t batch0, batch1;
  int64_t sa0, sa1, sb0, sb1, sc0, sc1;
  int split_k;
  void* workspace; int64_t workspace_bytes;
  const uint32_t* k_live; uint32_t k_epoch;
  const uint32_t* m_live; uint32_t m_epoch;
  const int32_t* k_len;
  const int32_t* m_len;
  void* colsum;
  int defer_reduce;
} cst_gemm_desc;

int64_t cst_gemm_workspace(const cst_gemm_desc* d);
int cst_gemm_colsum_is_fused(const cst_gemm_desc* d);
int cst_gemm_splits(const cst_gemm_desc* d);
int cst_gemm_route(const cst_gemm_desc* d, char* out, int64_t out_bytes);
int cst_gemm_reserve_cus(int n);
int cst_gemm(const cst_gemm_desc* d, cst_stream stream);

int cst_posconv_fwd(const void* x, const void* w, const void* bias, void* y, void* z, const int32_t* m_len, int64_t B, int64_t T,
                    int64_t C, int64_t groups, int64_t k, cst_stream stream);
int cst_posconv_dx(const void* dz, const void* wflip, const void* dy, void* dx, const int32_t* m_len, int64_t B, int64_t T,
                   int64_t C, int64_t groups, int64_t k, cst_stream stream);
int cst_posconv_dw(const void* dz, const void* x, void* dw, void* db, const uint32_t* k_live, uint32_t k_epoch, int64_t B,
                   int64_t T, int64_t C, int64_t groups, int64_t k, cst_stream stream);

typedef struct {
  int dtype;
  int64_t B, H, Tq, Tk, D;
  const void* Q; int64_t q_sb, q_sh, q_st;
  const void* K; int64_t k_sb, k_sh, k_st;
  const void* V; int64_t v_sb, v_sh, v_st;
  void* O; int64_t o_sb, o_sh, o_st;
  float* lse;
  const uint8_t* key_padding_mask; int64_t kpm_stride;
  int causal;
  float scale;
  float drop_p; uint32_t drop_key;
  const void* dO; int64_t do_sb, do_sh, do_st;
  void* dQ; int64_t dq_sb, dq_sh, dq_st;
  void* dK; int64_t dk_sb, dk_sh, dk_st;
  void* dV; int64_t dv_sb, dv_sh, dv_st;
  float* delta;
  const int32_t* kv_len;
  uint8_t* q_flags;
  const int32_t* seq_offsets;
  const uint64_t* kpm_bits;
  void* bwd_ws;
} cst_attn_desc;

int64_t cst_attn_bwd_workspace(const cst_attn_desc* d);
int cst_attn_fwd(const cst_attn_desc* d, cst_stream stream);
int cst_attn_bwd(const cst_attn_desc* d, cst_stream stream);

int cst_conv_row_limits(const int32_t* nz_last, const int32_t* k, const int32_t* stride, int L, int64_t S, int32_t* out, int64_t B,
                        int smax, cst_stream stream);
int64_t cst_conv0_fwd_workspace(int64_t B, int64_t S, int k, int stride);
int cst_conv0_gn_gelu_fwd(const float* wav, const void* w, const void* gamma, const void* beta,
                          void* y, float* mean, float* rstd, float* gram, float* workspace, const int32_t* frame_limit, int64_t B,
                          int64_t S, int64_t C, int k, int stride, float eps, int dtype, cst_stream stream);
int64_t cst_conv0_bwd_workspace(int64_t B, int64_t S, int64_t C, int k, int stride);
int cst_conv0_gn_gelu_bwd(const void* dy, const float* wav, const void* w, const void* gamma,
                          const void* beta, const float* mean, const float* rstd, const float* gram,
                          float* dw, float* dgamma, float* dbeta, float* workspace, const int32_t* frame_limit,
                          int64_t B, int64_t S, int64_t C, int k, int stride, int dtype,
                          cst_stream stream);

int cst_conv0_ln_gelu_fwd(const float* wav, const void* w, const void* bias, const void* gamma, const void* beta, void* y,
                          float* mean, float* rstd, const int32_t* frame_limit, int64_t B, int64_t S, int64_t C, int k,
                          int stride, float eps, int dtype, cst_stream stream);
int64_t cst_conv0_ln_bwd_workspace(int64_t B, int64_t S, int64_t C, int k, int stride);
int cst_conv0_ln_gelu_bwd(const void* dy, const float* wav, const void* w, const void* bias, const void* gamma, const void* beta,
                          const float* mean, const float* rstd, float* dw, float* dbias, float* dgamma, float* dbeta,
                          float* workspace, const int32_t* frame_limit, int64_t B, int64_t S, int64_t C, int k, int stride,
                          int dtype, cst_stream stream);
int cst_ln_gelu_fwd(const void* u, const void* gamma, const void* beta, void* y, float* mean, float* rstd,
                    const int32_t* row_limit, int64_t B, int64_t L, int64_t C, float eps, int dtype, cst_stream stream);
int64_t cst_ln_gelu_bwd_workspace(int64_t rows, int64_t C);
int cst_ln_gelu_bwd(const void* dy, const void* u, const void* gamma, const void* beta, const float* mean, const float* rstd,
                    void* du, int64_t du_batch_stride, float* dgamma, float* dbeta, float* dcolsum, float* workspace,
                    const int32_t* row_limit, int64_t B, int64_t L, int64_t C, int dtype, cst_stream stream);

int cst_glu_fwd(const void* z, void* y, int64_t rows, int64_t C, int dtype, cst_stream stream);
int cst_glu_bwd(const void* dy, const void* z, void* dz, int64_t rows, int64_t C, int dtype, cst_stream stream);
int cst_act_bwd(const void* dy, const void* z, void* dx, int64_t n, int act, int dtype, cst_stream stream);
int cst_act_fwd(const void* x, void* y, int64_t n, int act, int dtype, cst_stream stream);
int cst_colsum(const void* x, int64_t ldx, float* out, int64_t rows, int64_t cols, int dtype, cst_stream stream);
int cst_dropout_colsum(const void* x, void* xd, void* out, void* workspace, int64_t rows, int64_t cols, int dtype, int out_dtype,
                       float p, uint32_t key, const uint32_t* row_live, uint32_t epoch, cst_stream stream);
int64_t cst_colsum_workspace(int64_t rows, int64_t cols);
int cst_colsum_typed(const void* x, int64_t ldx, void* out, void* workspace, int64_t rows, int64_t cols, int dtype, int out_dtype,
                     cst_stream stream);
int cst_colsum_typed_live(const void* x, int64_t ldx, void* out, void* workspace, int64_t rows, int64_t cols, int dtype,
                          int out_dtype, const uint32_t* row_live, uint32_t epoch, cst_stream stream);
int cst_col2im1d(const void* dcol, const void* z, void* dx, int64_t B, int64_t Lin, int64_t Lout,
                 int64_t C, int k, int stride, int pad, int dact, int dtype, cst_stream stream);
int64_t cst_weight_norm_workspace(int64_t R, int64_t C);
int cst_weight_norm_fwd(const void* v, const void* g, void* w, float* norm, void* workspace, int64_t R, int64_t C, int dtype, cst_stream stream);
int cst_weight_norm_bwd(const void* v, const void* g, const void* dw, const float* norm, void* dv, void* dg, void* workspace, int64_t R,
                        int64_t C, int dtype, cst_stream stream);
int cst_transpose2d(const void* src, void* dst, int64_t R, int64_t C, int dtype, cst_stream stream);
typedef struct cst_transpose_item {
  const void* src; void* dst;
  int64_t R, C;
  int64_t tile0;
} cst_transpose_item;
int cst_transpose2d_multi(const cst_transpose_item* items_dev, int n, int64_t total_tiles, int dtype, cst_stream stream);
#define CST_REDUCE_MAX_ITEMS 64
typedef struct cst_reduce_item {
  const float* src; void* dst;
  int64_t stride, L;
  int32_t P, dst_dtype, block0, order;
} cst_reduce_item;
int cst_reduce_multi(const cst_reduce_item* items, int n, cst_stream stream);
int cst_mask_rows(const void* x, const uint8_t* mask, void* y, int64_t rows, int64_t cols, int dtype, cst_stream stream);

int cst_rows_pack(const void* src, const int32_t* seq_off, void* dst, int64_t B, int64_t T, int64_t C, int tail_sum, int dtype,
                  cst_stream stream);
int cst_rows_unpack(const void* src, const int32_t* seq_off, void* dst, int64_t B, int64_t T, int64_t C, int tail_broadcast, int dtype,
                    cst_stream stream);

int cst_dropout(const void* x, void* y, int64_t n, float p, uint32_t key, int dtype, cst_stream stream);
int cst_dropout_scale(const void* x, void* y, int64_t n, float alpha, float p, uint32_t key, int dtype, cst_stream stream);

int cst_embed_pos_fwd(const int64_t* tokens, const uint8_t* pad_mask, const void* embed, const void* x, const float* pos_table,
                      float scale, int64_t pad_idx, void* out, int64_t B, int64_t T, int64_t C, int64_t V, int64_t pos_rows,
                      float drop_p, uint32_t drop_key, int dtype, cst_stream stream);
int cst_embed_bwd(const void* dy, const int64_t* tokens, void* dE, float scale, int64_t pad_idx, int64_t n, int64_t C, int64_t V,
                  float drop_p, uint32_t drop_key, int dtype, int grad_dtype, cst_stream stream);

int cst_ls_ce_fwd(const void* logits, const int64_t* target, float* out2, float* lse, float* row_ws,
                  int64_t rows, int64_t V, float eps, int64_t pad_idx, int dtype, cst_stream stream);
int cst_ls_ce_bwd(const void* logits, const int64_t* target, const float* lse, const float* gscale,
                  void* dlogits, int64_t rows, int64_t V, float eps, int64_t pad_idx, int dtype,
                  cst_stream stream);

int cst_score_tokens(const void* logits, const void* const* logits_n, int64_t members, int64_t ld, const int64_t* target, int64_t pad,
                     float* pos, float* score, int32_t* len, int64_t B, int64_t T, int64_t V, int dtype, cst_stream stream);

int cst_ctc_fwd(const void* logits, int64_t stride_t, int64_t stride_b, const int64_t* targets, int64_t Lmax, const int64_t* target_len,
                const int64_t* input_len, int64_t blank, int zero_infinity, float* nll, float* loss, float* lse, float* emit, float* alpha,
                float* beta, int64_t T, int64_t B, int64_t V, int dtype, cst_stream stream);
int cst_ctc_bwd(const void* logits, int64_t stride_t, int64_t stride_b, const int64_t* targets, int64_t Lmax, const int64_t* target_len,
                const int64_t* input_len, int64_t blank, int zero_infinity, const float* nll, const float* lse, const float* alpha,
                const float* beta, const float* gscale, void* dlogits, int64_t dstride_t, int64_t dstride_b, int64_t T, int64_t B,
                int64_t V, int dtype, cst_stream stream);
int cst_ctc_greedy(const void* logits, int64_t stride_t, int64_t stride_b, const int64_t* input_len, int64_t blank, int32_t* argmax_ws,
                   int32_t* ids, int32_t* counts, int64_t T, int64_t B, int64_t V, int dtype, cst_stream stream);

int cst_w2v_negatives(uint32_t key, int64_t B, int64_t M, int64_t K, int64_t Kx, int32_t* out, cst_stream stream);
int cst_infonce_fwd(const void* x, const void* y, const int32_t* idx, float inv_temp, float* nll, float* loss, int32_t* counters,
                    float* lse, float* nx, float* ny, int32_t* flags, float* logits_dbg, int64_t N, int64_t KP, int64_t D, int dtype,
                    cst_stream stream);
int cst_infonce_bwd_x(const void* x, const void* y, const int32_t* idx, float inv_temp, const float* lse, const float* nx,
                      const float* ny, const float* gscale, void* dx, float* pairs, int64_t N, int64_t KP, int64_t D, int dtype,
                      cst_stream stream);
int cst_infonce_bwd_y(const void* x, const void* y, const int64_t* perm, const int32_t* offs, const float* pairs, const float* nx,
                      const float* ny, void* dy, int64_t N, int64_t KP, int64_t D, int dtype, cst_stream stream);

int64_t cst_gumbel_vq_workspace(int64_t N, int64_t G, int64_t V);
int cst_gumbel_vq_fwd(const void* logits, const void* vars, const float* noise, uint32_t key, int training, void* q, int32_t* idx,
                      void* onehot, float* avg_probs, float* stats, float* exph, void* workspace, int64_t N, int64_t G, int64_t V, int64_t d,
                      int dtype, cst_stream stream);
int cst_gumbel_vq_bwd(const void* logits, const float* noise, uint32_t key, float inv_tau, const void* gy, const float* avg_probs,
                      const float* exph, const float* dppl, void* dl, int64_t N, int64_t G, int64_t V, int dtype, cst_stream stream);

int cst_contrastive_fwd(const void* a, const void* t, float* loss, float* loss_rows, float* sim, float* na, float* nt,
                        int64_t B, int64_t M, int64_t C, float temp, int dtype, cst_stream stream);
int cst_contrastive_bwd(const void* a, const void* t, const float* sim, const float* na, const float* nt,
                        const float* gscale, void* da, void* dt, int64_t B, int64_t M, int64_t C, float temp,
                        int dtype, cst_stream stream);

int64_t cst_sumsq_workspace(void);
int cst_sumsq(const void* x, int64_t n, float* out, float* workspace, int dtype, cst_stream stream);
int cst_adam_step(float* master, float* exp_avg, float* exp_avg_sq, const void* grad, void* model_param,
                  int64_t n, float lr, float beta1, float beta2, float eps, float weight_decay,
                  int64_t step, const float* grad_scale, int grad_dtype, int param_dtype,
                  cst_stream stream);

typedef struct {
  int dtype;
  int64_t bsz, beam, vocab, max_len;
  int64_t pad, unk, eos, min_len;
  float unk_penalty, len_penalty, temperature;
  int normalize_scores;
  const void* logits; int64_t ld_logits;
  int32_t* step;
  int64_t* tokens; float* scores; int32_t* anc;
  uint8_t* cands_to_ignore; uint8_t* finished; int32_t* nfinal; int32_t* num_remaining;
  int64_t* fin_tokens; float* fin_pos; float* fin_score; int32_t* fin_len;
  void* workspace;
  int64_t members;
  const void* logits_n[7];
  float* lprobs_out;
  int64_t no_repeat_ngram;
  const int64_t* prefix_tokens;
  int64_t prefix_len;
  int64_t sampling;
  int64_t sample_topk;
  float sample_topp;
  const uint32_t* sample_key;
  int64_t diverse_groups;
  float diverse_strength;
  int64_t diverse_siblings;
  float sibling_rate;
  int32_t* fin_anc;
} cst_beam_desc;
int64_t cst_beam_workspace(int64_t bsz, int64_t beam);
int cst_beam_init(const cst_beam_desc* d, cst_stream stream);
int cst_beam_step(const cst_beam_desc* d, cst_stream stream);
typedef struct { const void* lm_logits; float lm_weight; float* lprobs_out; } cst_lm_fusion_desc;
int cst_beam_step_lm(const cst_beam_desc* d, const cst_lm_fusion_desc* f, cst_stream stream);
typedef struct {
  int64_t representation;
  const int64_t* constraints;
  int64_t width;
  void* workspace;
} cst_lex_desc;
int64_t cst_lex_workspace(int64_t bsz, int64_t beam, int64_t width);
int cst_lex_init(const cst_beam_desc* d, const cst_lex_desc* x, cst_stream stream);
int cst_beam_step_lex(const cst_beam_desc* d, const cst_lm_fusion_desc* f, const cst_lex_desc* x, cst_stream stream);
int cst_dec_embed(const int64_t* tokens, const int32_t* step, const void* embed, const float* pos_table, float scale,
                  int64_t pad_idx, void* out, int64_t rows, int64_t C, int64_t max_len, int64_t pos_rows, int dtype,
                  cst_stream stream);
int cst_dec_linear(const void* x, const void* W, const void* bias, const void* resid, void* y, int64_t M, int64_t N, int64_t K,
                   int64_t ldx, int64_t ld_resid, int64_t ldy, int act, const int32_t* step, int64_t max_len, int dtype,
                   cst_stream stream);
int cst_dec_ln_linear(const void* x, const void* Wg, const float* sg, const float* sb, float eps, const void* resid, void* y, int64_t M,
                      int64_t N, int64_t K, int64_t ldx, int64_t ld_resid, int64_t ldy, int act, const int32_t* step, int64_t max_len,
                      int dtype, cst_stream stream);
int cst_dec_self_attn(const void* qkv, void* kcache, void* vcache, const int32_t* anc, const int32_t* step, void* out,
                      int64_t rows, int64_t H, int64_t D, int64_t max_len, float scale, int dtype, cst_stream stream);
int cst_dec_cross_attn(const void* q, const void* kx, const void* vx, const uint8_t* key_padding_mask, void* out,
                       const int32_t* step, int64_t max_len, int64_t bsz, int64_t beam, int64_t H, int64_t D, int64_t S, float scale,
                       int dtype, cst_stream stream);
int cst_dec_ln_q_cross_attn(const void* x, int64_t ldx, const void* Wg, const float* sg, const float* sb, float eps, const void* kx, const void* vx,
                            const uint8_t* key_padding_mask, void* out, const int32_t* step, int64_t max_len, int64_t bsz, int64_t beam, int64_t H,
                            int64_t D, int64_t S, float scale, int dtype, cst_stream stream);

int cst_attn_avg_probs(const void* q, int64_t ldq, const void* k, int64_t k_sb, int64_t k_sh, int64_t k_st, const uint8_t* key_padding_mask,
                       float* out, int64_t out_row_stride, const int32_t* step, int64_t max_len, int64_t B, int64_t Tq, int64_t H, int64_t D,
                       int64_t S, float scale, float out_scale, int accumulate, int dtype, cst_stream stream);

typedef struct {
  int64_t B, S, T;
  const float* wave;
  const int64_t* n_samples;
  float* out;
  int64_t* n_frames;
  int utterance_cmvn, norm_means, norm_vars;
  const float* global_mean;
  const float* global_std;
  int global_first;
  int specaugment;
  int n_fmask, n_tmask;
  const int32_t* fmask;
  const int32_t* tmask;
  int mask_mean;
  float mask_value;
  void* workspace;
  int64_t workspace_bytes;
} cst_fbank_desc;
int64_t cst_fbank_workspace_bytes(int64_t B, int64_t T);
int cst_fbank(const cst_fbank_desc* d, cst_stream stream);

int64_t cst_batch_by_size(const int64_t* num_tokens, int64_t n, int64_t max_tokens, int64_t max_sentences, int32_t bsz_mult,
                          int64_t* batch_sizes);
int cst_wav_info(const char* path, int32_t* sample_rate, int32_t* channels, int64_t* frames, int32_t* bits);
int64_t cst_wav_read_f32(const char* path, int64_t start_frame, int64_t nframes, float* out, int64_t capacity_samples);
int64_t cst_edit_distance(const int64_t* a, int64_t na, const int64_t* b, int64_t nb);

typedef enum { CST_TOK_U8 = 0, CST_TOK_U16 = 1, CST_TOK_I32 = 2, CST_TOK_I64 = 3 } cst_tok_dtype;
int cst_collate_pairs(const void* src_stream, const void* tgt_stream, int tok_dtype, const int64_t* src_offsets,
                      const int64_t* tgt_offsets, int64_t n_sentences, const int64_t* idx, int64_t B, int64_t S, int64_t T, int64_t pad,
                      int64_t eos, int left_pad_source, int left_pad_target, int64_t* out, cst_stream stream);

typedef enum { CST_BREAK_NONE = 0, CST_BREAK_COMPLETE = 1, CST_BREAK_COMPLETE_DOC = 2, CST_BREAK_EOS = 3 } cst_break_mode;
int64_t cst_token_block_slices(const int64_t* sizes, int64_t n, int break_mode, int64_t block_size, int64_t document_sep_len,
                               int64_t* slices_out, int64_t capacity);
int cst_token_block_index(const int64_t* sizes, int64_t n, const int64_t* slices, int64_t n_blocks, int64_t* out);
int cst_collate_blocks(const void* stream_tokens, int tok_dtype, const int64_t* blocks, int64_t n_blocks, const int64_t* idx, int64_t B,
                       int64_t T, int64_t pad, int64_t eos, int64_t* out, cst_stream stream);

#ifdef __cplusplus
}
#endif
#endif
```

Before: 507.1.

## Fold batch into K for conv weight-gradient GEMM instead of per-batch partials

Adds a k_fold mode to the register GEMM kernel. The batch dimension is concatenated into the reduction, so each workgroup walks a contiguous range of live K tiles across batches and accumulates straight into one output. The conv1d weight-gradient path now uses it in place of writing B fp32 partial matrices and reducing them. This is meant to remove the large partial buffer and its reduction, and to balance split-K work over only the live tiles. In exchange it adds a per-workgroup prefix scan over batch lengths, plus a workspace reduction when splits exceed one.

```diff
diff --git a/chimera-st_amd/csrc/gemm.hip b/chimera-st_amd/csrc/gemm.hip
--- a/chimera-st_amd/csrc/gemm.hip
+++ b/chimera-st_amd/csrc/gemm.hip
@@ -19,8 +19,9 @@
 using CfgNarrowM = Cfg<64, 128, 2, 2>;
 using CfgLarge = Cfg<256, 256, 4, 4>;
 
-template <typename T, bool A_KMAJOR, bool B_KMAJOR, bool SEG, typename C, bool CS = false>
+template <typename T, bool A_KMAJOR, bool B_KMAJOR, bool SEG, typename C, bool CS = false, bool FOLD = false>
 __global__ __launch_bounds__(C::NT) void gemm_kernel(GemmParams p) {
+  static_assert(!FOLD || (!A_KMAJOR && !B_KMAJOR && !SEG && !CS), "the folded batch is built for the weight-gradient layout only");
   constexpr int BM = C::BM, BN = C::BN, NTHREADS = C::NT, TM = C::TM, TN = C::TN;
   constexpr int VEC = DT<T>::VEC;
   constexpr int KV = C::KV, BK = KV * VEC;
@@ -66,24 +67,58 @@
   const int64_t m0 = (int64_t)tm * BM, n0 = (int64_t)tn * BN;
 
   const int split = z % p.splits;
-  const int64_t bidx = z / p.splits;
-  const int64_t b0 = bidx / p.batch1, b1 = bidx % p.batch1;
+  const int64_t bidx = FOLD ? 0 : z / p.splits;
+  int ktiles = (int)((p.K + BK - 1) / BK);
+  const int kfull = (int)(p.K / BK);
+  auto live_tiles = [&](int64_t b) {
+    typedef const __attribute__((address_space(4))) int32_t* cptr_t;
+    const int kl = ((cptr_t)p.k_len)[b];
+    const int live = kl <= 0 ? 0 : (kl + BK - 1) / BK;
+    return live < ktiles ? live : ktiles;
+  };
+  __shared__ int fold_at[3];
+  int fold_b = 0, fold_t = 0, fold_n = 0;
+  if constexpr (FOLD) {
+    if (wave == 0) {
+      auto count = [&](int b) { return b < p.k_fold ? (p.k_len ? live_tiles(b) : ktiles) : 0; };
+      auto wave_sum = [](int v) {
+#pragma unroll
+        for (int o = 32; o > 0; o >>= 1) v += __shfl_xor(v, o, 64);
+        return v;
+      };
+      int total = 0;
+      for (int base = 0; base < p.k_fold; base += 64) total += wave_sum(count(base + lane));
+      const int lo = (int)(((int64_t)total * split) / p.splits), hi = (int)(((int64_t)total * (split + 1)) / p.splits);
+      if (lane == 0) { fold_at[0] = 0; fold_at[1] = 0; fold_at[2] = hi - lo; }
+      int before = 0;
+      for (int base = 0; base < p.k_fold && before <= lo && hi > lo; base += 64) {
+        const int n = count(base + lane);
+        int incl = n;
+#pragma unroll
+        for (int o = 1; o < 64; o <<= 1) {
+          const int u = __shfl_up(incl, o, 64);
+          if (lane >= o) incl += u;
+        }
+        const int first = before + incl - n;
+        if (n > 0 && first <= lo && lo < first + n) { fold_at[0] = base + lane; fold_at[1] = lo - first; }
+        before += __shfl(incl, 63, 64);
+      }
+    }
+    __syncthreads();
+    fold_b = __builtin_amdgcn_readfirstlane(fold_at[0]);
+    fold_t = __builtin_amdgcn_readfirstlane(fold_at[1]);
+    fold_n = __builtin_amdgcn_readfirstlane(fold_at[2]);
+  }
+  const int64_t b0 = FOLD ? fold_b : bidx / p.batch1, b1 = FOLD ? 0 : bidx % p.batch1;
   const T* A = (const T*)p.A + b0 * p.sa0 + b1 * p.sa1;
   const T* B = (const T*)p.B + b0 * p.sb0 + b1 * p.sb1;
-  const int64_t cofs = b0 * p.sc0 + b1 * p.sc1;
-  const int64_t bofs = b0 * p.sbias0 + b1 * p.sbias1;
-
-  int ktiles = (int)((p.K + BK - 1) / BK);
-  const int kfull = (int)(p.K / BK);
-  if (p.k_len) {
-    typedef const __attribute__((address_space(4))) int32_t* cptr_t;
-    const int kl = ((cptr_t)p.k_len)[b0];
-    const int live = kl <= 0 ? 0 : (kl + BK - 1) / BK;
-    ktiles = live < ktiles ? live : ktiles;
-  }
+  const int64_t cofs = FOLD ? 0 : b0 * p.sc0 + b1 * p.sc1;
+  const int64_t bofs = FOLD ? 0 : b0 * p.sbias0 + b1 * p.sbias1;
+
+  if (!FOLD && p.k_len) ktiles = live_tiles(b0);
   const int per = (ktiles + p.splits - 1) / p.splits;
-  const int kt0 = split * per;
-  const int kt1 = (kt0 + per < ktiles) ? kt0 + per : ktiles;
+  const int kt0 = FOLD ? fold_t : split * per;
+  const int kt1 = FOLD ? kt0 + fold_n : ((kt0 + per < ktiles) ? kt0 + per : ktiles);
 
   u32x4 ra[NVA], rb[NVB];
   const T* pa[NVA];
@@ -208,7 +243,7 @@
   constexpr int KLIST_MAX = 1000;
   __shared__ int klist[KLIST_MAX];
   __shared__ int klist_n;
-  const bool kskip = !SEG && BK == 64 && p.k_live != nullptr && per <= KLIST_MAX;
+  const bool kskip = !FOLD && !SEG && BK == 64 && p.k_live != nullptr && per <= KLIST_MAX;
   int nk = kt1 > kt0 ? kt1 - kt0 : 0;
   if (kskip) {
     if (wave == 0) {
@@ -233,7 +268,7 @@
     __syncthreads();
     nk = klist_n;
   }
-  if (p.m_live) {
+  if (!FOLD && p.m_live) {
     typedef const __attribute__((address_space(4))) uint32_t* cptr_t;
     cptr_t ml = (cptr_t)p.m_live;
     const int t0 = (int)(m0 >> 6), t1 = (int)((((m0 + BM < p.M) ? m0 + BM : p.M) + 63) >> 6);
@@ -241,7 +276,7 @@
     for (int t = t0; t < t1; ++t) live |= ml[t] == p.m_epoch;
     if (!live) nk = 0;
   }
-  if (p.m_len) {
+  if (!FOLD && p.m_len) {
     typedef const __attribute__((address_space(4))) int32_t* cptr_t;
     if (m0 >= (int64_t)((cptr_t)p.m_len)[b0]) nk = 0;
   }
@@ -258,9 +293,29 @@
     pos = kt + 1;
   };
   auto tile_at = [&](int it) { return kskip ? klist[it] : kt0 + it; };
+  int cb = fold_b, pb_at = fold_b, ct = fold_t, cn = 0;
+  if constexpr (FOLD) cn = fold_n > 0 ? (p.k_len ? live_tiles(fold_b) : ktiles) : 0;
+  auto fetch_next = [&]() {
+    while (ct >= cn && cb + 1 < p.k_fold) {
+      ++cb;
+      ct = 0;
+      cn = p.k_len ? live_tiles(cb) : ktiles;
+    }
+    const int db = cb - pb_at;
+    if (db) {
+#pragma unroll
+      for (int i = 0; i < NVA; ++i) pa[i] += (int64_t)db * p.sa0;
+#pragma unroll
+      for (int i = 0; i < NVB; ++i) pb[i] += (int64_t)db * p.sb0;
+      pb_at = cb;
+    }
+    fetch(ct);
+    ++ct;
+  };
 
   if (nk > 0) {
-    fetch(tile_at(0));
+    if constexpr (FOLD) fetch_next();
+    else fetch(tile_at(0));
     store_tile(0);
   }
   __syncthreads();
@@ -269,7 +324,10 @@
   constexpr int WROWS = TM * 32, WCOLS = TN * 32;
   for (int it = 0; it < nk; ++it) {
     const bool more = it + 1 < nk;
-    if (more) fetch(tile_at(it + 1));
+    if (more) {
+      if constexpr (FOLD) fetch_next();
+      else fetch(tile_at(it + 1));
+    }
     const T* sa = smem + cur * STAGE;
     const T* sb = sa + A_ELEMS;
 #pragma unroll
@@ -773,6 +831,26 @@
   return cst_check_launch("cst_gemm");
 }
 
+template <typename T, typename C>
+int launch_fold(GemmParams p, hipStream_t s) {
+  constexpr int VEC = DT<T>::VEC, BKc = C::KV * VEC;
+  constexpr int LDMA = sizeof(T) == 2 ? C::BM + 32 : C::BM + VEC, LDMB = sizeof(T) == 2 ? C::BN + 32 : C::BN + VEC;
+  size_t lds = 2 * (size_t)(BKc * LDMA + BKc * LDMB) * sizeof(T);
+  const size_t stage_bytes = (size_t)64 * (C::BN + 4) * sizeof(float);
+  if (lds < stage_bytes) lds = stage_bytes;
+  static bool attr_set = false;
+  if (!attr_set) {
+    (void)hipFuncSetAttribute(reinterpret_cast<const void*>(&gemm_kernel<T, false, false, false, C, false, true>), hipFuncAttributeMaxDynamicSharedMemorySize, 160 * 1024 - 4096);
+    attr_set = true;
+  }
+  p.tiles_m = (int)cst_ceil_div(p.M, C::BM);
+  p.tiles_n = (int)cst_ceil_div(p.N, C::BN);
+  p.split_order = p.splits > 1 ? 1 : 0;
+  dim3 grid(p.tiles_m * p.tiles_n, 1, (unsigned)p.splits);
+  hipLaunchKernelGGL((gemm_kernel<T, false, false, false, C, false, true>), grid, dim3(C::NT), lds, s, p);
+  return cst_check_launch("cst_gemm");
+}
+
 template <typename T, bool AK, bool BK_, typename C, int NS>
 int launch_glds(GemmParams p, int64_t M, int64_t N, int64_t nbatch, hipStream_t s) {
   constexpr int ES = sizeof(T), BKc = 128 / ES;
@@ -836,6 +914,7 @@
   int stages;
   int splits;
   Colsum colsum;
+  bool fold;
 };
 
 struct TileDims { int bm, bn, nt; };
@@ -875,6 +954,29 @@
   return (int)s;
 }
 
+bool kfold_supported(const cst_gemm_desc* d) {
+  if (d->a_kmajor || d->b_kmajor || d->a_seg || d->b_seg || d->batch0 < 1 || d->batch1 != 1) return false;
+  if (d->bias || d->act || d->dact || d->aux_out || d->resid || d->colsum || d->alpha != 1.0f || d->drop_p != 0.0f) return false;
+  if (d->k_live || d->m_live || d->m_len || d->ldc != d->N || d->N % 8 != 0) return false;
+  return d->K > 0 && d->batch0 * cst_ceil_div(d->K, 32) < (1ll << 31);
+}
+
+bool fold_large(const cst_gemm_desc* d) { return d->M >= 256 && d->N >= 256; }
+
+int fold_splits(const cst_gemm_desc* d) {
+  if (d->split_k > 1) return d->split_k;
+  if (d->split_k == 0 || d->split_k == 1) return 1;
+  const int64_t t = fold_large(d) ? 256 : 128;
+  const int64_t tiles = cst_ceil_div(d->M, t) * cst_ceil_div(d->N, t);
+  const int64_t ktiles = d->batch0 * cst_ceil_div(d->K, d->dtype == CST_BF16 ? 64 : 32);
+  int64_t s = 256 / tiles;
+  if (s > ktiles / 16) s = ktiles / 16;
+  if (s > 64) s = 64;
+  return s < 1 ? 1 : (int)s;
+}
+
+int64_t out_batches(const cst_gemm_desc* d) { return d->k_fold ? 1 : d->batch0 * d->batch1; }
+
 struct Forced { const char* name; bool kk; Family family; Tile tile; int stages; };
 const Forced kForced[] = {
     {"small", false, Family::Reg, Tile::Small, 0},     {"narrowm", false, Family::Reg, Tile::NarrowM, 0},
@@ -894,6 +996,14 @@
   r.bk = d->b_kmajor != 0;
   r.seg = (r.ak && d->a_seg) || (r.bk && d->b_seg);
   r.stages = 2;
+  r.fold = d->k_fold != 0;
+  if (r.fold) {
+    r.family = Family::Reg;
+    r.tile = fold_large(d) ? Tile::Large : Tile::Small;
+    r.splits = fold_splits(d);
+    r.colsum = Colsum::None;
+    return r;
+  }
   r.splits = choose_splits(d);
   const bool kk = r.ak && r.bk, mm = !r.ak && !r.bk;
   const bool large = use_large(d, r.seg, r.splits);
@@ -938,7 +1048,7 @@
   const char a = r.ak ? 'k' : 'm', b = r.bk ? 'k' : 'm';
   switch (r.family) {
     case Family::Reg:
-      snprintf(out, (size_t)n, "reg %s %c%c%s %dx%d nt%d%s split%d", dt, a, b, r.seg ? " seg" : "", t.bm, t.bn, t.nt,
+      snprintf(out, (size_t)n, "reg %s %c%c%s %dx%d nt%d%s split%d", dt, a, b, r.seg ? " seg" : (r.fold ? " kfold" : ""), t.bm, t.bn, t.nt,
                r.colsum == Colsum::Fused ? " colsum" : "", r.splits);
       break;
     case Family::Dma: snprintf(out, (size_t)n, "glds %s %c%c %dx%d nt%d ns%d split%d", dt, a, b, t.bm, t.bn, t.nt, r.stages, r.splits); break;
@@ -976,6 +1086,10 @@
   CST_REQUIRE(d->drop_p >= 0.0f && d->drop_p < 1.0f, "cst_gemm: drop_p must be in [0, 1)");
   CST_REQUIRE(d->drop_p == 0.0f || d->batch0 * d->batch1 == 1, "cst_gemm: fused dropout needs an unbatched problem");
   CST_REQUIRE(!d->colsum || (!d->a_kmajor && !d->a_seg), "cst_gemm: colsum needs an mn-major, unsegmented A");
+  if (d->k_fold && !kfold_supported(d)) {
+    cst_set_error("cst_gemm: k_fold does not cover this descriptor (see cst_gemm_kfold_supported)");
+    return CST_ERR_UNSUPPORTED;
+  }
   return CST_OK;
 }
 
@@ -1019,6 +1133,7 @@
   p.m_epoch = d->m_epoch;
   p.k_len = sw.no_klive ? nullptr : d->k_len;
   p.m_len = sw.no_klive ? nullptr : d->m_len;
+  p.k_fold = d->k_fold ? (int)d->batch0 : 0;
   p.group_m = sw.group_m;
   p.splits = 1;
   p.ws = nullptr;
@@ -1028,7 +1143,7 @@
 }
 
 int64_t route_workspace(const cst_gemm_desc* d, const GemmRoute& r) {
-  const int64_t s = r.splits, nb = d->batch0 * d->batch1;
+  const int64_t s = r.splits, nb = out_batches(d);
   int64_t bytes = s > 1 ? s * d->M * d->N * nb * (int64_t)sizeof(float) : 0;
   if (r.colsum == Colsum::Fused) bytes += s > 1 ? s * d->M * nb * (int64_t)sizeof(float) : 0;
   else if (r.colsum == Colsum::Separate) bytes += cst_colsum_workspace(d->K, d->M);
@@ -1037,7 +1152,7 @@
 
 int take_route(const cst_gemm_desc* d, const GemmSwitches& sw, GemmParams& p, GemmRoute& r) {
   r = gemm_route(d, p, sw);
-  const int64_t nbatch = d->batch0 * d->batch1;
+  const int64_t nbatch = out_batches(d);
   CST_REQUIRE(r.colsum != Colsum::Separate || (nbatch == 1 && d->M % 8 == 0 && d->lda % 8 == 0),
               "cst_gemm: colsum of this configuration runs as a separate column sum: unbatched, M and lda multiples of 8");
   CST_REQUIRE(cst_ceil_div(d->M, 128) * cst_ceil_div(d->N, 128) < (1ll << 31) && nbatch * r.splits < 65536, "cst_gemm: grid too large");
@@ -1102,6 +1217,10 @@
     }
   }
   const double nbatch = (double)(d->batch0 * d->batch1), esz = (double)cst_dtype_size(d->dtype);
+  if (d->k_fold)
+    return {2.0 * (double)d->M * (double)d->N * (double)d->K * nbatch * frac,
+            ((double)d->M * d->K + (double)d->N * d->K) * esz * nbatch * frac +
+                (double)d->M * d->N * (p.splits > 1 ? 4.0 * p.splits : (double)cst_dtype_size(d->c_dtype))};
   return {2.0 * (double)d->M * (double)d->N * (double)d->K * nbatch * frac,
           ((double)d->M * d->K + (double)d->N * d->K) * esz * nbatch * frac + (double)d->M * d->N * cst_dtype_size(d->c_dtype) * nbatch};
 }
@@ -1130,6 +1249,7 @@
 int launch_route(const GemmRoute& r, const GemmParams& p, int64_t nbatch, hipStream_t s, const GemmSwitches& sw) {
   constexpr bool HOOK = std::is_same<T, bf16_t>::value;
   const int64_t M = p.M, N = p.N;
+  if (r.fold) return r.tile == Tile::Large ? launch_fold<T, CfgLarge>(p, s) : launch_fold<T, CfgSmall>(p, s);
   switch (arm(r.family, r.tile, r.family == Family::Dma ? r.stages : 0)) {
     case arm(Family::Persistent8, Tile::Large): return cst_gemm8p_launch(p, r.ak, r.bk, nbatch, s);
     case arm(Family::FourWave, Tile::Big4N): return cst_gemm4w_launch(p, s);
@@ -1157,7 +1277,7 @@
 }
 
 int finish(const cst_gemm_desc* d, const GemmRoute& r, const GemmParams& p, cst_stream stream) {
-  const int64_t nbatch = d->batch0 * d->batch1;
+  const int64_t nbatch = out_batches(d);
   if (p.splits > 1 && d->defer_reduce) {
     CST_REQUIRE((nbatch == 1 || !d->colsum) && d->alpha == 1.0f && !d->bias && !d->act && !d->dact && !d->aux_out && !d->resid && d->drop_p == 0.0f && d->ldc == d->N &&
                     d->N % 8 == 0 && r.colsum != Colsum::Separate,
@@ -1190,14 +1310,14 @@
   GemmRoute r;
   if ((rc = take_route(d, sw, p, r)) != CST_OK) return rc;
   hipStream_t s = (hipStream_t)stream;
-  const int64_t nbatch = d->batch0 * d->batch1;
+  const int64_t nbatch = out_batches(d);
   const Work w = credited_work(d, p, s);
   CstProfScope prof(CST_K_GEMM, s, w.flops, w.bytes);
   rc = r.bf16 ? launch_route<bf16_t>(r, p, nbatch, s, sw) : launch_route<float>(r, p, nbatch, s, sw);
   if (cst_prof_is_on())
-    prof.tag("M=%lld N=%lld K=%lld b=%lld a%c b%c split=%d%s%s%s%s%s%s%s", (long long)d->M, (long long)d->N, (long long)d->K, (long long)nbatch, r.ak ? 'k' : 'm',
-             r.bk ? 'k' : 'm', p.splits, d->bias ? " bias" : "", d->act ? " act" : "", d->aux_out ? " aux_out" : "", d->dact ? " dact" : "",
-             d->resid ? " resid" : "", d->drop_p > 0 ? " drop" : "", (d->k_live || d->m_live || d->k_len || d->m_len) ? " live" : "");
+    prof.tag("M=%lld N=%lld K=%lld b=%lld a%c b%c split=%d%s%s%s%s%s%s%s%s", (long long)d->M, (long long)d->N, (long long)d->K, (long long)(d->batch0 * d->batch1),
+             r.ak ? 'k' : 'm', r.bk ? 'k' : 'm', p.splits, d->bias ? " bias" : "", d->act ? " act" : "", d->aux_out ? " aux_out" : "", d->dact ? " dact" : "",
+             d->resid ? " resid" : "", d->drop_p > 0 ? " drop" : "", (d->k_live || d->m_live || d->k_len || d->m_len) ? " live" : "", r.fold ? " kfold" : "");
   return rc != CST_OK ? rc : finish(d, r, p, stream);
 }
 
@@ -1213,6 +1333,8 @@
 extern "C" int cst_gemm_colsum_is_fused(const cst_gemm_desc* d) { return d && query_route(d).colsum == Colsum::Fused ? 1 : 0; }
 
 extern "C" int64_t cst_gemm_workspace(const cst_gemm_desc* d) { return route_workspace(d, query_route(d)); }
+
+extern "C" int cst_gemm_kfold_supported(const cst_gemm_desc* d) { return d && kfold_supported(d) ? 1 : 0; }
 
 extern "C" int cst_gemm_route(const cst_gemm_desc* d, char* out, int64_t out_bytes) {
   if (out && out_bytes > 0) out[0] = 0;
diff --git a/chimera-st_amd/csrc/gemm_common.h b/chimera-st_amd/csrc/gemm_common.h
--- a/chimera-st_amd/csrc/gemm_common.h
+++ b/chimera-st_amd/csrc/gemm_common.h
@@ -38,6 +38,7 @@
   int* sched;
   const uint32_t* m_live; uint32_t m_epoch;
   const int32_t* k_len;
+  int k_fold;
   const int32_t* m_len;
   const uint32_t* k_live; uint32_t k_epoch;
   void* colsum;
diff --git a/chimera-st_amd/functional.py b/chimera-st_amd/functional.py
--- a/chimera-st_amd/functional.py
+++ b/chimera-st_amd/functional.py
@@ -826,13 +826,18 @@
                 pzc = prev_z if prev_z is None else prev_z.contiguous()
                 dx = K.col2im1d(dcol, pzc, B, Lin, Lout, Cin, k, stride, pad, L.ACT_GELU if prev_z is not None else 0)
         if ctx.needs_input_grad[1]:
-            part = torch.empty(B, Cout, k * Cin, dtype=torch.float32, device=dy.device)
-            wgs = B * ((Cout + 255) // 256) * ((k * Cin + 255) // 256)
-            rem = wgs % 256
-            sk = 2 if (wgs >= 256 and 0 < rem < 192 and Lout >= 2048) else 1
             dw = torch.empty(Cout, k * Cin, dtype=w_cl.dtype, device=dy.device)
-            K.gemm(dz_rows, xp, part, Cout, k * Cin, Lout, a_kmajor=0, b_kmajor=0, lda=Cout, ldb=stride * Cin, ldc=k * Cin, batch0=B,
-                   sa=(dz_bs, 0), sb=(xp.stride(0), 0), sc=(Cout * k * Cin, 0), a_off=dz_off, split_k=sk, k_len=ctx.nz_out, reduce_to=dw)
+            folded = None
+            if not _os.environ.get("CST_NO_KFOLD"):
+                folded = K.gemm(dz_rows, xp, dw, Cout, k * Cin, Lout, a_kmajor=0, b_kmajor=0, lda=Cout, ldb=stride * Cin, ldc=k * Cin,
+                                batch0=B, sa=(dz_bs, 0), sb=(xp.stride(0), 0), a_off=dz_off, k_len=ctx.nz_out, k_fold=True)
+            if folded is None:
+                part = torch.empty(B, Cout, k * Cin, dtype=torch.float32, device=dy.device)
+                wgs = B * ((Cout + 255) // 256) * ((k * Cin + 255) // 256)
+                rem = wgs % 256
+                sk = 2 if (wgs >= 256 and 0 < rem < 192 and Lout >= 2048) else 1
+                K.gemm(dz_rows, xp, part, Cout, k * Cin, Lout, a_kmajor=0, b_kmajor=0, lda=Cout, ldb=stride * Cin, ldc=k * Cin, batch0=B,
+                       sa=(dz_bs, 0), sb=(xp.stride(0), 0), sc=(Cout * k * Cin, 0), a_off=dz_off, split_k=sk, k_len=ctx.nz_out, reduce_to=dw)
         if has_bias and ctx.needs_input_grad[2]:
             db = K.colsum(dz_rows.reshape(B * Lout, Cout) if dzp is None else dzp[:, 1:1 + Lout].reshape(B * Lout, Cout), w_cl.dtype)
         return dx, dw, db, None, None, None, None, None, None, None, None, None
diff --git a/chimera-st_amd/kernels.py b/chimera-st_amd/kernels.py
--- a/chimera-st_amd/kernels.py
+++ b/chimera-st_amd/kernels.py
@@ -125,7 +125,7 @@
          aux_out=None, ld_aux_out=0, dact=L.ACT_NONE, aux_in=None, ld_aux_in=0, resid=None, ld_resid=0, alpha=1.0,
          batch0=1, batch1=1, sa=(0, 0), sb=(0, 0), sc=(0, 0), sbias=(0, 0), a_seg=0, a_seg_stride=0, b_seg=0,
          b_seg_stride=0, split_k=-1, a_off=0, b_off=0, c_off=0, drop_p=0.0, drop_key=0, k_live=None, m_live=None, k_len=None, m_len=None,
-         ws=None, colsum=None, defer=False, reduce_to=None):
+         ws=None, colsum=None, defer=False, reduce_to=None, k_fold=False):
     lib = L.load()
     d = L.GemmDesc()
     d.dtype = L.dtype_code(A.dtype)
@@ -171,11 +171,18 @@
     else:
         d.colsum = None
     d.defer_reduce = 0
+    d.k_fold = 0
+    if k_fold:
+        assert reduce_to is None and ws is None and sc == (0, 0)
+        if not lib.cst_gemm_kfold_supported(ctypes.byref(d)):
+            return None
+        d.k_fold = 1
+        STATS["gemm_k_fold"] = STATS.get("gemm_k_fold", 0) + 1
     splits = 1
     need = lib.cst_gemm_workspace(ctypes.byref(d))
-    nb = batch0 * batch1
+    nb = 1 if k_fold else batch0 * batch1
     deferred = False
-    if need > 0 and (reduce_to is not None or (defer and DEFER.on and nb == 1 and need <= DEFER.MAX_BYTES and ldc == N and N % 8 == 0)):
+    if need > 0 and (reduce_to is not None or k_fold or (defer and DEFER.on and nb == 1 and need <= DEFER.MAX_BYTES and ldc == N and N % 8 == 0)):
         splits = lib.cst_gemm_splits(ctypes.byref(d))
         if splits > 1:
             assert ws is None and bias is None and act == L.ACT_NONE and dact == L.ACT_NONE and resid is None and aux_out is None and alpha == 1.0
@@ -197,6 +204,8 @@
             DEFER.push(*item)
         else:
             reduce_multi([(item[0], item[1].data_ptr(), item[2], item[3], item[4], L.dtype_code(reduce_to.dtype), 0)])
+    elif deferred and k_fold and not (defer and DEFER.on):
+        reduce_multi([(ws.data_ptr(), C.data_ptr(), M * N, M * N, splits, L.dtype_code(C.dtype), 0)])
     elif deferred:
         DEFER.push(ws.data_ptr(), C, M * N, M * N, splits, ws)
         if colsum is not None:
diff --git a/chimera-st_amd/lib.py b/chimera-st_amd/lib.py
--- a/chimera-st_amd/lib.py
+++ b/chimera-st_amd/lib.py
@@ -41,6 +41,7 @@
         ("m_len", c_p),
         ("colsum", c_p),
         ("defer_reduce", c_int),
+        ("k_fold", c_int),
     ]
 
 
@@ -140,6 +141,7 @@
     ("cst_gemm_colsum_is_fused", c_int, [ctypes.POINTER(GemmDesc)]),
     ("cst_gemm_splits", c_int, [ctypes.POINTER(GemmDesc)]),
     ("cst_gemm_route", c_int, [ctypes.POINTER(GemmDesc), ctypes.c_char_p, c_i64]),
+    ("cst_gemm_kfold_supported", c_int, [ctypes.POINTER(GemmDesc)]),
     ("cst_reduce_multi", c_int, [ctypes.POINTER(ReduceItem), c_int, c_p]),
     ("cst_gemm", c_int, [ctypes.POINTER(GemmDesc), c_p]),
     ("cst_posconv_fwd", c_int, [c_p, c_p, c_p, c_p, c_p, c_p, c_i64, c_i64, c_i64, c_i64, c_i64, c_p]),
diff --git a/chimera-st_amd/s2t_transformer.py b/chimera-st_amd/s2t_transformer.py
--- a/chimera-st_amd/s2t_transformer.py
+++ b/chimera-st_amd/s2t_transformer.py
@@ -1,7 +1,5 @@
 import math
 from typing import Dict, List, Optional
-
-import os
 
 import torch
 import torch.nn as nn
@@ -48,7 +46,7 @@
         for _ in range(self.n_layers):
             lens.append(((lens[-1].float() - 1) / 2 + 1).floor().long())
         limits = [None] * self.n_layers
-        if padding_unread and not os.environ.get("CST_NO_MLEN"):
+        if padding_unread:
             need = lens[-1]
             for i in reversed(range(self.n_layers)):
                 limits[i] = need.to(torch.int32).contiguous()
diff --git a/include/cst.h b/include/cst.h
--- a/include/cst.h
+++ b/include/cst.h
@@ -75,12 +75,14 @@
   const int32_t* m_len;
   void* colsum;
   int defer_reduce;
+  int k_fold;
 } cst_gemm_desc;
 
 int64_t cst_gemm_workspace(const cst_gemm_desc* d);
 int cst_gemm_colsum_is_fused(const cst_gemm_desc* d);
 int cst_gemm_splits(const cst_gemm_desc* d);
 int cst_gemm_route(const cst_gemm_desc* d, char* out, int64_t out_bytes);
+int cst_gemm_kfold_supported(const cst_gemm_desc* d);
 int cst_gemm_reserve_cus(int n);
 int cst_gemm(const cst_gemm_desc* d, cst_stream stream);
 
```

Result: faster. 513.6, median of 6 (+1.3%).
